# sebhaan/geobo

Measured on AMD Instinct MI355X. Metric: voxels/sec posterior (mean+var) for 64^3 x 2-prop joint inversion; fp64 roofline %, higher is better.
Workload: dtype f64

## Files before the change

geobo_amd/_lib.py:

```python
import ctypes as C
import os

LIB_PATH = os.environ.get("GEOBO_HIP_LIB") or os.path.join(os.path.dirname(os.path.abspath(__file__)), "lib", "libgeobo_hip.so")

_dp = C.c_void_p
_i64 = C.c_int64
_f64 = C.c_double
_int = C.c_int
_sz = C.c_size_t

SIGNATURES = {
    "geobo_version": (_int, []),
    "geobo_pad_m": (_i64, [_i64]),
    "geobo_pad_n": (_i64, [_i64]),
    "geobo_k_block": (_int, [_int, _dp, _dp, _dp, _i64, _dp, _dp, _dp, _i64, _f64, _f64, _f64, _f64, _dp, _i64, _dp]),
    "geobo_k_block_f32": (_int, [_int, _dp, _dp, _dp, _i64, _dp, _dp, _dp, _i64, _f64, _f64, _f64, _f64, _dp, _i64, _dp]),
    "geobo_k_block_grid": (_int, [_int, _int, _int, _dp, _dp, _i64, _i64, _i64, _i64, _int, _dp, _i64, _dp]),
    "geobo_lattice_wbuild": (_int, [_i64, _int, _int, _int, _dp, _dp, _dp, _dp]),
    "geobo_lattice_wplanes": (_int, [_i64, _int, _int, _int, _dp, _dp, _dp, _dp]),
    "geobo_xz2d_fold_inv_strided": (_int, [_int, _i64, _int, _dp, _i64, _i64, _dp, _dp, _dp, _i64, _i64, _i64, _dp]),
    "geobo_xz2d_fold_inv_mul": (_int, [_int, _i64, _int, _dp, _i64, _dp, _i64, _dp, _dp, _dp, _i64, _i64, _i64, _dp]),
    "geobo_sumsq_accum": (_int, [_i64, _i64, _dp, _i64, _dp, _i64, _int, _dp, _i64, _dp]),
    "geobo_lamdot_z": (_int, [_i64, _int, _int, _int, _dp, _dp, _dp, _dp]),
    "geobo_centro_fill": (_int, [_dp, _i64, _i64, _i64, _dp]),
    "geobo_mirror_rows": (_int, [_dp, _i64, _i64, _i64, _i64, _int, _dp]),
    "geobo_mirror_dev_ws_bytes": (_sz, []),
    "geobo_mirror_dev": (_int, [_dp, _i64, _dp, _i64, _i64, _int, _int, _dp, _dp, _sz, _dp]),
    "geobo_colgemv_ws_bytes": (_sz, [_i64, _i64]),
    "geobo_colgemv": (_int, [_i64, _i64, _dp, _i64, _dp, _dp, _dp, _sz, _dp]),
    "geobo_rowgemv": (_int, [_i64, _i64, _dp, _i64, _dp, _dp, _dp]),
    "geobo_convert": (_int, [_int, _dp, _i64, _dp, _i64, _i64, _i64, _dp]),
    "geobo_round_f32": (_int, [_dp, _i64, _dp]),
    "geobo_k_eval": (_int, [_int, _dp, _i64, _f64, _f64, _f64, _f64, _dp, _dp]),
    "geobo_a_sens": (_int, [_int, C.POINTER(_f64), _dp, _i64, _int, _int, _int, _dp, _dp, _dp, _f64, _f64, _dp, _i64, _dp]),
    "geobo_a_sens_slab": (_int, [_int, C.POINTER(_f64), _dp, _i64, _int, _int, _int, _dp, _dp, _dp, _f64, _f64, _int, _int, _dp, _i64, _i64, _dp]),
    "geobo_potential": (_int, [_int, C.POINTER(_f64), _dp, _dp, _dp, _i64, _dp, _dp]),
    "geobo_ak_fused": (_int, [_int, _dp, _i64, _i64, _i64, _dp, _dp, _dp, _i64, _i64, _f64, _f64, _f64, _f64, _dp, _i64, _dp]),
    "geobo_ak_points": (_int, [_int, _dp, _i64, _i64, _i64, _dp, _dp, _dp, _dp, _dp, _dp, _i64, _f64, _f64, _f64, _f64, _dp, _i64, _dp]),
    "geobo_cov_table": (_int, [_int, _int, _int, _int, _f64, _f64, _f64, _f64, _f64, _f64, _f64, _dp, _dp]),
    "geobo_ak_fused_grid": (_int, [_dp, _i64, _i64, _i64, _int, _int, _int, _dp, _i64, _i64, _dp, _i64, _dp]),
    "geobo_gemm_nt": (_int, [_i64, _i64, _i64, _f64, _dp, _i64, _dp, _i64, _f64, _dp, _i64, _int, _i64, _dp]),
    "geobo_tile_order": (_i64, [_int, _int, _int, _int, _int, _int, _int, C.POINTER(_int), _i64]),
    "geobo_gemm_nt_splitk": (_int, [_i64, _i64, _i64, _int, _dp, _i64, _dp, _i64, _dp, _i64, _int, _i64, _dp, _sz, _dp]),
    "geobo_gemm_nn": (_int, [_i64, _i64, _i64, _f64, _dp, _i64, _dp, _i64, _f64, _dp, _i64, _int, _int, _dp]),
    "geobo_gemm_batched": (_int, [_int, _i64, _i64, _i64, _f64, _dp, _i64, _i64, _dp, _i64, _i64, _f64, _dp, _i64, _i64, _i64, _i64, _int, _dp]),
    "geobo_gemm_fold_lamdot": (_int, [_i64, _i64, _i64, _dp, _i64, _dp, _i64, _i64, _dp, _int, _i64, _dp, _i64, _dp]),
    "geobo_gemm_fold": (_int, [_int, _int, _i64, _i64, _i64, _dp, _i64, _i64, _dp, _i64, _i64, _dp, _i64, _i64, _i64, _i64, _i64, _dp]),
    "geobo_scale_broadcast": (_int, [_dp, _dp, _i64, _i64, _dp, _dp]),
    "geobo_scale_broadcast2": (_int, [_dp, _dp, _dp, _i64, _i64, _dp, _dp, _dp]),
    "geobo_a_sens_lattice_ws_bytes": (_sz, [_int, _int, _int]),
    "geobo_a_sens_lattice": (_int, [_int, C.POINTER(_f64), _i64, _int, _int, _int, _dp, _dp, _dp, _dp, _dp, _f64, _f64, _int, _int, _dp, _i64,
                                    _i64, _dp, _sz, _dp]),
    "geobo_xz2d": (_int, [_int, _int, _int, _i64, _int, _dp, _i64, _i64, _dp, _i64, _dp, _i64, _dp, _i64, _i64, _dp]),
    "geobo_xz2d_fold": (_int, [_int, _int, _i64, _int, _dp, _i64, _i64, _dp, _dp, _dp, _i64, _i64, _dp]),
    "geobo_xz2d_fold_quad": (_int, [_int, _int, _i64, _int, _dp, _i64, _i64, _dp, _dp, _dp, _i64, _i64, _dp]),
    "geobo_xcorr_reduce_fold": (_int, [_int, _i64, _int, _dp, _i64, _i64, _dp, _dp, _dp, _i64, _i64, _dp]),
    "geobo_xz2d_fold_lattice": (_int, [_int, _i64, _int, _dp, _dp, _i64, _dp, _i64, _dp, _dp, _dp, _i64, _i64, _dp]),
    "geobo_xz2d_fold_inv_ss_slots": (_int, [_int, _i64, _int]),
    "geobo_xz2d_fold_inv_ss": (_int, [_int, _i64, _int, _dp, _i64, _i64, _dp, _i64, _i64, _dp, _dp, _dp, _dp]),
    "geobo_ymul": (_int, [_int, _int, _i64, _i64, _dp, _i64, _dp, _i64, _dp, _i64, _dp]),
    "geobo_ymul_fold": (_int, [_int, _int, _i64, _i64, _dp, _i64, _dp, _i64, _dp, _i64, _dp]),
    "geobo_xcorr_reduce": (_int, [_int, _int, _i64, _int, _dp, _i64, _i64, _dp, _i64, _dp, _dp, _i64, _i64, _dp]),
    "geobo_toeplitz_y": (_int, [_int, _i64, _i64, _i64, _int, _dp, _dp, _dp, _dp, _dp, _int, _int, _dp]),
    "geobo_toeplitz_y2t": (_int, [_int, _i64, _i64, _i64, _dp, _dp, _dp, _dp, _dp, _dp, _dp, _dp, _dp]),
    "geobo_toeplitz_y2s": (_int, [_int, _i64, _i64, _i64, _dp, _dp, _dp, _dp, _dp, _dp, _dp, _dp]),
    "geobo_toeplitz_y3": (_int, [_int, _i64, _i64, _i64, _int, _dp, C.POINTER(_dp), C.POINTER(_dp), _int, _int, _dp]),
    "geobo_toeplitz_y3_add": (_int, [_int, _i64, _i64, _i64, _int, _dp, C.POINTER(_dp), C.POINTER(_dp), _int, _int, _dp]),
    "geobo_spectral_y_basis_doubles": (_i64, [_int]),
    "geobo_spectral_y_basis": (_int, [_int, _dp, _dp]),
    "geobo_spectral_y": (_int, [_int, _i64, _i64, _i64, _int, _dp, _dp, _dp, _dp, _dp, _int, _int, _dp, _dp]),
    "geobo_spectral_y_lattice": (_int, [_int, _i64, _i64, _i64, _int, _dp, _dp, _dp, _i64, _dp, _dp, _dp, _dp, _dp, _int, _int, _dp, _dp]),
    "geobo_spectral_y2s": (_int, [_int, _i64, _i64, _i64, _dp, _dp, _dp, _dp, _dp, _dp, _dp, _dp, _dp]),
    "geobo_spectral_y3": (_int, [_int, _i64, _i64, _i64, _int, _dp, C.POINTER(_dp), C.POINTER(_dp), _int, _int, _int, _dp, _dp]),
    "geobo_spectral_y3t": (_int, [_int, _i64, _i64, _i64, _int, _dp, _dp, C.POINTER(_dp), C.POINTER(_dp), C.POINTER(_dp), _dp, _dp]),
    "geobo_spectral_axis": (_int, [_int, _int, _i64, _i64, _i64, _i64, _i64, _i64, _dp, _dp, _dp, _int, _dp]),
    "geobo_potrf_ws_bytes": (_sz, [_i64]),
    "geobo_potrf_ctx_create": (_int, [C.POINTER(C.c_void_p)]),
    "geobo_potrf_ctx_destroy": (_int, [_dp]),
    "geobo_potrf_inv": (_int, [_i64, _dp, _i64, _dp, _i64, _dp, _dp, _sz, _dp, _dp]),
    "geobo_posterior_ws_bytes": (_sz, [_i64, _i64]),
    "geobo_posterior_reduce": (_int, [_i64, _i64, _dp, _i64, _dp, _i64, _dp, _f64, _dp, _dp, _i64, _dp, _sz, _dp]),
    "geobo_kinv_dot_ws_bytes": (_sz, [_i64, _int]),
    "geobo_kinv_dot": (_int, [_i64, _dp, _i64, _dp, _int, C.POINTER(_dp), _i64, C.POINTER(_i64), _dp, _dp, _sz, _dp]),
    "geobo_philox_fill": (_int, [_int, C.c_uint64, C.c_uint64, _i64, _i64, _i64, _i64, C.c_uint64, _dp, _dp]),
    "geobo_torus_table": (_int, [_int, _int, _int, _int, _f64, _f64, _f64, _f64, _f64, _f64, _f64, _dp, _dp]),
    "geobo_fft_lines": (_int, [_int, _i64]),
    "geobo_fft_axis": (_int, [_int, _i64, _int, _i64, _int, _int, _dp, _dp, _int, _i64, _i64, _dp]),
    "geobo_sample_factor_ws_bytes": (_sz, []),
    "geobo_sample_factor": (_int, [_int, _int, _int, _int, _dp, _dp, _dp, _dp, _sz, _dp, _dp]),
    "geobo_sample_zpass": (_int, [_int, _i64, _i64, _int, _int, _int, _int, _dp, _dp, C.c_uint64, _dp, _dp]),
    "geobo_spectral_mix": (_int, [_int, _i64, _int, _int, _int, _dp, _f64, _dp, _dp, _dp]),
    "geobo_set_gram": (_int, [_i64, _int, _dp, _i64, _dp, _i64, _i64, _int, _dp, _dp]),
    "geobo_set_logdet": (_int, [_i64, _int, _dp, _dp, _i64, _f64, _dp, _dp, _i64, _dp, _dp, _dp]),
    "geobo_kinv_diag_ws_bytes": (_sz, [_i64]),
    "geobo_kinv_diag": (_int, [_i64, _dp, _i64, _dp, _dp, _dp, _dp, _sz, _dp]),
    "geobo_set_loo": (_int, [_i64, _int, _dp, _dp, _dp, _i64, _dp, _dp, _dp, _dp, _dp, _dp]),
    "geobo_block_cov_ws_bytes": (_sz, [_i64, _int, _int, _int, _int, _int, _int]),
    "geobo_block_cov": (_int, [_i64, _dp, _dp, _dp, _i64, _int, _int, _int, _int, _int, _int, _int, _dp, _dp, _sz, _dp]),
    "geobo_box_means": (_int, [_i64, _dp, _i64, _i64, _int, _int, _int, _int, _int, _int, _dp, _dp, _dp]),
    "geobo_cutoff_stats_ws_bytes": (_sz, [_i64, _i64, _int]),
    "geobo_cutoff_stats": (_int, [_i64, _dp, _i64, _i64, _i64, _int, _int, C.POINTER(_f64), C.POINTER(_f64), _dp, _dp, _dp, _dp, _dp, _dp, _sz, _dp]),
    "geobo_bodies_ws_bytes": (_sz, [_i64, _int, _int, _int, _int]),
    "geobo_bodies": (_int, [_i64, _dp, _i64, _i64, _int, _int, _int, _int, _int, C.POINTER(_f64), C.POINTER(_f64), _dp, _dp, _int, _i64, _i64,
                            C.POINTER(C.c_int32), _dp, _dp, _dp, _dp, _dp, _dp, _int, _dp, _sz, _dp]),
    "geobo_trace_stats_ws_bytes": (_sz, [_i64, _i64, _int]),
    "geobo_trace_stats": (_int, [_i64, _dp, _i64, _i64, _int, _int, _int, _int, _int, C.POINTER(_f64), C.POINTER(_f64), _dp, _i64, _dp, _dp, _int,
                                 _int, _int, _dp, _dp, _dp, _dp, _dp, _dp, _dp, _dp, _dp, _dp, _dp, _sz, _dp]),
    "geobo_trmv_stats": (_int, [_i64, _dp, _i64, _dp, _dp, _i64, _dp, _dp, _dp]),
    "geobo_mfma_f64_peak": (_int, [_int, _int, _dp, _dp]),
    "geobo_mfma_mix": (_int, [_int, _int, _int, _int, _dp, _dp]),
}


class GeoboHipUnavailable(RuntimeError):
    pass


_lib = None


def load():
    global _lib
    if _lib is not None:
        return _lib
    if not os.path.exists(LIB_PATH):
        raise GeoboHipUnavailable(
            "%s not found. Build the HIP extension first: `python -m geobo_amd.build` "
            "(hipcc --offload-arch=gfx950). There is no CPU fallback for the inversion hot path." % LIB_PATH)
    import torch
    try:
        lib = C.CDLL(LIB_PATH)
    except OSError as e:
        raise GeoboHipUnavailable("cannot load %s: %s" % (LIB_PATH, e)) from e
    for name, (res, args) in SIGNATURES.items():
        try:
            fn = getattr(lib, name)
        except AttributeError as e:
            raise GeoboHipUnavailable("libgeobo_hip.so lacks symbol %s (stale build?)" % name) from e
        fn.restype = res
        fn.argtypes = args
    _lib = lib
    return lib


ERRORS = {-1: "GEOBO_E_ARG", -2: "GEOBO_E_ALIGN", -3: "GEOBO_E_LAUNCH", -4: "GEOBO_E_UNSUPPORTED"}


def check(rc, what):
    if rc != 0:
        raise RuntimeError("%s failed: %s (%d)" % (what, ERRORS.get(rc, "?"), rc))
```

geobo_amd/csrc/gemm_f64.hip:

```cpp
#include <hip/hip_runtime.h>
#include <atomic>
#include <type_traits>
#include <stdint.h>
#include "covfun.h"
#include "geobo_hip.h"

typedef double v4d __attribute__((ext_vector_type(4)));
typedef double v2d __attribute__((ext_vector_type(2)));

namespace {

constexpr int BK = 16;
constexpr int XS = 16;
constexpr int NST = 3;

__device__ __forceinline__ int swz(int row) {
  const int p = (row >> 1) & 7;
  return (p & 1) | (((p >> 2) & 1) * 6);
}

enum { Y_GEN = 0, Y_NT = 1, Y_NN = 2, Y_TAB = 3 };
enum { EPI_STORE = 0, EPI_REDUCE = 1 };
enum { TRI_LOWER_ONLY = 1, TRI_X_LOWER = 2, TRI_Y_LOWER = 4 };

struct GemmArgs {
  const double* X; int64_t ldx;
  const double* Y; int64_t ldy;
  double* C; int64_t ldc;
  int64_t k;
  double alpha, beta;
  int nbi, nbj, tri, xcd_map;
  int ntiles;
  int64_t sXb, sYb, sCb, m_valid, n_valid; int batch;
  const double *px, *py, *pz; int64_t gcol0;
  const double *qx, *qy, *qz;
  CovParams cov;
  const double* table; int gnx, gny, gnz; int64_t gN;
  const double* u; double* part_mu; double* part_ss; int64_t ncols;
  int64_t row_shift;
};

__host__ __device__ inline int lower_cols(int bi, int nbj, int tm, int tn) {
  const int64_t c = ((int64_t)(bi + 1) * tm + tn - 1) / tn;
  return c < nbj ? (int)c : nbj;
}
__host__ __device__ inline int64_t tile_items(int nbi, int nbj, int tm, int tn, int tri) {
  if (!(tri & TRI_LOWER_ONLY)) return (int64_t)nbi * nbj;
  int64_t n = 0;
  for (int bi = 0; bi < nbi; ++bi) n += lower_cols(bi, nbj, tm, tn);
  return n;
}
__host__ __device__ __forceinline__ void tile_of_item(int t, int nbi, int nbj, int tm, int tn, int tri, int& bi, int& bj) {
  if (tri & TRI_X_LOWER) { bi = nbi - 1 - t / nbj; bj = t % nbj; return; }
  if (tri & TRI_Y_LOWER) { bj = t / nbi; bi = t % nbi; return; }
  if (!(tri & TRI_LOWER_ONLY)) {
    const int band = t / (4 * nbj), r0 = 4 * band;
    const int rows = nbi - r0 < 4 ? nbi - r0 : 4;
    t -= band * 4 * nbj;
    bj = t / rows; bi = r0 + t % rows;
    return;
  }
  int r0 = 0;
  for (;; r0 += 4) {
    int cnt = 0;
    for (int i = r0; i < r0 + 4 && i < nbi; ++i) cnt += lower_cols(i, nbj, tm, tn);
    if (t < cnt || r0 + 4 >= nbi) break;
    t -= cnt;
  }
  const int r1 = r0 + 4 < nbi ? r0 + 4 : nbi;
  for (bj = 0; bj < nbj; ++bj) {
    const int first = (int)(((int64_t)bj * tn) / tm);
    const int lo = first > r0 ? first : r0;
    const int c = r1 - lo;
    if (c <= 0) continue;
    if (t < c) { bi = lo + t; return; }
    t -= c;
  }
  bi = nbi; bj = 0;
}

template <int WM, int WN>
constexpr int ring_depth() { return (WM * WN >= 8) ? NST : 2; }

template <int WM, int WN, int YMODE>
constexpr int lds_doubles() {
  constexpr int TM = 64 * WM, TN = 64 * WN;
  constexpr int ybuf = (YMODE == Y_NN) ? BK * (TN + 4) : TN * XS;
  return ring_depth<WM, WN>() * (TM * XS + ybuf);
}

template <int WM, int WN, int YMODE, int EPI, int KID>
__global__ void __launch_bounds__(64 * WM * WN, 2) gemm_f64_kernel(const GemmArgs a) {
  constexpr int TM = 64 * WM, TN = 64 * WN, NT = 64 * WM * WN;
  constexpr int YS_NN = TN + 4;
  constexpr int XBUF = TM * XS;
  constexpr int YBUF = (YMODE == Y_NN) ? BK * YS_NN : TN * XS;
  constexpr int XU = TM * 8 / NT;
  constexpr int YU = (YMODE == Y_NN) ? (8 * TN / NT) : (TN * 8 / NT);
  constexpr int EPT = BK * TN / NT;
  static_assert(NT % TN == 0 && EPT >= 2 && EPT % 2 == 0, "generator mapping");

  extern __shared__ __attribute__((aligned(16))) double smem[];
  double* const Xs = smem;
  constexpr int NSTG = ring_depth<WM, WN>();
  double* const Ys = smem + NSTG * XBUF;

  const int tid = threadIdx.x, lane = tid & 63;
  const int wave = __builtin_amdgcn_readfirstlane(tid >> 6);
  const int wrow = wave / WN, wn = wave % WN;
  const int wm = (WM == 4) ? (wrow < 2 ? wrow : 5 - wrow) : wrow;
  const int lr = lane & 15, lg = lane >> 4;

  int bi, bj;
  int batch_idx = blockIdx.y;
  {
    const int b = blockIdx.x;
    if (a.xcd_map == 1) {
      const int xcd = b & 7, s = b >> 3;
      bj = s % a.nbj;
      bi = xcd + 8 * (s / a.nbj);
    } else if (a.xcd_map == 2) {
      const int xcd = b & 7, s = b >> 3;
      const int within = s & 31, g = (s >> 5) * 8 + xcd;
      const int nsi = (a.nbi + 3) >> 2;
      if (a.tri & TRI_X_LOWER) {
        const int nsj = (a.nbj + 31) >> 5;
        bi = g / nsj;
        bj = 32 * (g % nsj) + within;
      } else {
        bi = 4 * (g % nsi) + (within & 3);
        bj = 8 * (g / nsi) + (within >> 2);
      }
      if (bj >= a.nbj) return;
    } else if (a.xcd_map == 3) {
      const int xcd = b & 7, s = b >> 3;
      const int64_t item = ((int64_t)((s >> 5) * 8 + xcd) << 5) + (s & 31);
      if (item >= (int64_t)a.ntiles * a.batch) return;
      batch_idx = (int)(item / a.ntiles);
      tile_of_item((int)(item - (int64_t)batch_idx * a.ntiles), a.nbi, a.nbj, TM, TN, a.tri, bi, bj);
    } else {
      bi = b % a.nbi;
      bj = b / a.nbi;
    }
  }
  if (bi >= a.nbi) return;
  const double* const Xp = a.X + (int64_t)batch_idx * a.sXb;
  const double* const Yp = a.Y + (int64_t)batch_idx * a.sYb;
  double* const Cp = a.C + (int64_t)batch_idx * a.sCb;
  if ((a.tri & TRI_X_LOWER) && a.xcd_map != 3) bi = a.nbi - 1 - bi;
  const int64_t row0 = (int64_t)bi * TM - a.row_shift, col0 = (int64_t)bj * TN;
  if ((a.tri & TRI_LOWER_ONLY) && col0 >= row0 + TM) return;
  int64_t kb = (a.tri & TRI_Y_LOWER) ? col0 : 0;
  int64_t ke = a.k;
  if ((a.tri & TRI_X_LOWER) && ke > row0 + TM) ke = row0 + TM;

  v4d acc[4][4];
#pragma unroll
  for (int m = 0; m < 4; ++m)
#pragma unroll
    for (int n = 0; n < 4; ++n) acc[m][n] = (v4d){0., 0., 0., 0.};
  bool c_in_acc = false;
  if constexpr (EPI == EPI_STORE && (YMODE == Y_NT || YMODE == Y_NN)) {
    c_in_acc = a.beta != 0.0 && (a.beta == a.alpha || a.beta == -a.alpha);
    if (c_in_acc) {
      const double sgn = (a.beta == a.alpha) ? 1.0 : -1.0;
#pragma unroll
      for (int m = 0; m < 4; ++m)
#pragma unroll
        for (int n = 0; n < 4; ++n)
#pragma unroll
          for (int r = 0; r < 4; ++r) {
            const int64_t row = row0 + wm * 64 + m * 16 + lg + 4 * r;
            const int64_t col = col0 + wn * 64 + n * 16 + lr;
            const bool ok = row < a.m_valid && col < a.n_valid;
            const double c = Cp[(row < a.m_valid ? row : a.m_valid - 1) * a.ldc + (col < a.n_valid ? col : a.n_valid - 1)];
            acc[m][n][r] = ok ? sgn * c : 0.0;
          }
    }
  }

  typedef __attribute__((address_space(3))) void* lds_ptr_t;
  typedef const __attribute__((address_space(1))) void* glb_ptr_t;
  auto dma16 = [&](const void* src, double* dst_wave_uniform) {
    __builtin_amdgcn_global_load_lds((glb_ptr_t)src, (lds_ptr_t)dst_wave_uniform, 16, 0, 0);
  };
  constexpr int RPI = NT / 8;
  const int srow = tid >> 3;
  const char* const Xgb = reinterpret_cast<const char*>(Xp);
  int64_t xsrc[XU];
#pragma unroll
  for (int i = 0; i < XU; ++i) {
    const int row = i * RPI + srow;
    const int64_t grow = row0 + row < 0 ? 0 : row0 + row;
    xsrc[i] = (grow * a.ldx + 2 * ((tid & 7) ^ swz(row))) * 8;
  }
  auto stage_x = [&](int64_t k0, int st) {
#pragma unroll
    for (int i = 0; i < XU; ++i) dma16(Xgb + xsrc[i] + k0 * 8, Xs + st * XBUF + (i * RPI + wave * 8) * XS);
  };

  int64_t ysrc[(YMODE == Y_NT) ? YU : 1];
  const char* const Ygb = (YMODE == Y_NT) ? reinterpret_cast<const char*>(Yp + col0 * a.ldy) : nullptr;
  if constexpr (YMODE == Y_NT) {
#pragma unroll
    for (int i = 0; i < YU; ++i) {
      const int row = i * RPI + srow;
      ysrc[i] = ((int64_t)row * a.ldy + 2 * ((tid & 7) ^ swz(row))) * 8;
    }
  }

  double qx = 0., qy = 0., qz = 0.;
  const int gq = tid % TN;
  const int gsub = __builtin_amdgcn_readfirstlane(tid / TN);
  v2d yr[EPT / 2];
  if constexpr (YMODE == Y_GEN) {
    const int64_t q = col0 + gq;
    qx = a.qx[q]; qy = a.qy[q]; qz = a.qz[q];
  }

  int tqy[YU], tqx[YU], tqz[YU], tsl[YU];
  int piy = 0, pix = 0, piz = 0;
  int64_t pk = kb;
  if constexpr (YMODE == Y_TAB) {
#pragma unroll
    for (int i = 0; i < YU; ++i) {
      const int row = i * RPI + srow;
      int64_t q = a.gcol0 + col0 + row;
      if (q >= a.gN) q = a.gN - 1;
      tqz[i] = (int)(q % a.gnz);
      const int64_t t = q / a.gnz;
      tqx[i] = (int)(t % a.gnx);
      tqy[i] = (int)(t / a.gnx);
      tsl[i] = (tid & 7) ^ swz(row);
    }
    piz = (int)(kb % a.gnz);
    const int64_t tp = kb / a.gnz;
    pix = (int)(tp % a.gnx);
    piy = (int)(tp / a.gnx);
  }

  auto stage_y = [&](int64_t k0, int st) {
    if constexpr (YMODE == Y_NT) {
#pragma unroll
      for (int i = 0; i < YU; ++i) dma16(Ygb + ysrc[i] + k0 * 8, Ys + st * YBUF + (i * RPI + wave * 8) * XS);
    } else if constexpr (YMODE == Y_NN) {
#pragma unroll
      for (int i = 0; i < YU; ++i) {
        const int kr = i * (NT / 64) + wave;
        dma16(Yp + (k0 + kr) * a.ldy + col0 + 2 * lane, Ys + st * YBUF + kr * YS_NN);
      }
    } else if constexpr (YMODE == Y_TAB) {
      const int adv = (int)(k0 - pk);
      pk = k0;
      piz += adv;
      int c = piz >= a.gnz ? 1 : 0;
      piz -= c ? a.gnz : 0;
      pix += c;
      c = pix >= a.gnx ? 1 : 0;
      pix -= c ? a.gnx : 0;
      piy += c;
      int bx = pix + 1, by = piy;
      if (bx >= a.gnx) { bx = 0; by += 1; }
      const int ay = piy < a.gny ? piy : a.gny - 1;
      by = by < a.gny ? by : a.gny - 1;
      const char* const tb = reinterpret_cast<const char*>(a.table);
      const unsigned nz2 = 2u * (unsigned)a.gnz;
#pragma unroll
      for (int i = 0; i < YU; ++i) {
        int pz = piz + 2 * tsl[i];
        const bool carry = pz >= a.gnz;
        pz -= carry ? a.gnz : 0;
        const unsigned cy = carry ? by : ay, cx = carry ? bx : pix;
        const unsigned rowb = __umul24(__usad((unsigned)tqx[i], cx, __umul24(__usad((unsigned)tqy[i], cy, 0u), (unsigned)a.gnx)), nz2);
        const unsigned idx = rowb + (unsigned)(pz - tqz[i] + a.gnz - 1);
        dma16(tb + (idx << 3), Ys + st * YBUF + (i * RPI + wave * 8) * XS);
      }
    }
  };
  auto gen_y = [&](int64_t k0) {
    const int64_t p0 = k0 + gsub * EPT;
#pragma unroll
    for (int e = 0; e < EPT; ++e) {
      const double d2 = sqdist3(a.px[p0 + e], a.py[p0 + e], a.pz[p0 + e], qx, qy, qz);
      yr[e >> 1][e & 1] = a.cov.scale * cov_eval<KID>(a.cov, d2);
    }
  };
  auto store_gen = [&](int st) {
    double* buf = Ys + st * YBUF;
#pragma unroll
    for (int e = 0; e < EPT / 2; ++e)
      *reinterpret_cast<v2d*>(buf + gq * XS + 2 * ((gsub * (EPT / 2) + e) ^ swz(gq))) = yr[e];
  };

  if (kb < ke) {
    const int xoff0 = 2 * ((2 * lg + 0) ^ swz(lr)), xoff1 = 2 * ((2 * lg + 1) ^ swz(lr));
    const double* const xfrag = Xs + (wm * 64 + lr) * XS;
    const double* const yfrag = (YMODE == Y_NN) ? (Ys + wn * 64 + lr) : (Ys + (wn * 64 + lr) * XS);
    auto read_half = [&](int stage, int h, v2d (&av)[4], v2d (&bv)[4]) {
      const double* xb = xfrag + stage * XBUF + (h ? xoff1 : xoff0);
#pragma unroll
      for (int m = 0; m < 4; ++m) av[m] = *reinterpret_cast<const v2d*>(xb + m * 16 * XS);
      if constexpr (YMODE == Y_NN) {
        const double* yb = yfrag + stage * YBUF + (4 * lg + 2 * h) * YS_NN;
#pragma unroll
        for (int n = 0; n < 4; ++n) { bv[n][0] = yb[n * 16]; bv[n][1] = yb[YS_NN + n * 16]; }
      } else {
        const double* yb = yfrag + stage * YBUF + (h ? xoff1 : xoff0);
#pragma unroll
        for (int n = 0; n < 4; ++n) bv[n] = *reinterpret_cast<const v2d*>(yb + n * 16 * XS);
      }
    };
    if constexpr (NSTG == 2) {
      stage_x(kb, 0);
      if constexpr (YMODE == Y_GEN) { gen_y(kb); store_gen(0); } else { stage_y(kb, 0); }
      __syncthreads();
      int cur = 0;
      for (int64_t k0 = kb; k0 < ke; k0 += BK) {
        int64_t kn = k0 + BK;
        if (kn >= ke) kn = ke - BK;
        stage_x(kn, cur ^ 1);
        if constexpr (YMODE != Y_GEN) stage_y(kn, cur ^ 1);
        v2d a0[4], b0[4], a1[4], b1[4];
        read_half(cur, 0, a0, b0);
        read_half(cur, 1, a1, b1);
        if constexpr (YMODE == Y_GEN) gen_y(kn);
#pragma unroll
        for (int t = 0; t < 4; ++t)
#pragma unroll
          for (int m = 0; m < 4; ++m)
#pragma unroll
            for (int n = 0; n < 4; ++n)
              acc[m][n] = __builtin_amdgcn_mfma_f64_16x16x4f64(t < 2 ? a0[m][t & 1] : a1[m][t & 1],
                                                               t < 2 ? b0[n][t & 1] : b1[n][t & 1], acc[m][n], 0, 0, 0);
        if constexpr (YMODE == Y_GEN) store_gen(cur ^ 1);
        __syncthreads();
        cur ^= 1;
      }
    } else {
    {
        const int64_t k1 = (kb + BK < ke) ? kb + BK : kb;
        stage_x(kb, 0);
        stage_x(k1, 1);
        if constexpr (YMODE == Y_GEN) {
          gen_y(kb); store_gen(0);
          gen_y(k1); store_gen(1);
        } else {
          stage_y(kb, 0);
          stage_y(k1, 1);
        }
      }
      __syncthreads();
      int s0 = 0, s1 = 1, s2 = 2;
      int64_t kw = ke;
      if constexpr (YMODE != Y_GEN) {
        if ((a.tri & TRI_X_LOWER) && kw > row0 + 64 * (wm + 1)) kw = row0 + 64 * (wm + 1);
        if (row0 + wm * 64 >= a.m_valid || row0 + wm * 64 < 0 || kw < kb) kw = kb;
      }
      int64_t kd = kw;
      if constexpr (YMODE != Y_GEN) {
        if ((a.tri & TRI_X_LOWER) && kw == row0 + 64 * (wm + 1) && kw - 64 >= kb) kd = kw - 64;
      }
      if (kw > kb) {
      v2d a0[4], b0[4], a1[4], b1[4];
      read_half(0, 0, a0, b0);
      for (int64_t k0 = kb; k0 < kd; k0 += BK) {
        int64_t kn = k0 + 2 * BK;
        if (kn >= ke) kn = ke - BK;
        stage_x(kn, s2);
        if constexpr (YMODE != Y_GEN) stage_y(kn, s2);
        const int64_t p0 = kn + gsub * EPT;
        read_half(s0, 1, a1, b1);
  #pragma unroll
        for (int t = 0; t < 4; ++t) {
          if (t == 2) read_half(s1, 0, a0, b0);
  #pragma unroll
          for (int m = 0; m < 4; ++m)
  #pragma unroll
            for (int n = 0; n < 4; ++n)
              acc[m][n] = __builtin_amdgcn_mfma_f64_16x16x4f64(t < 2 ? a0[m][t & 1] : a1[m][t & 1],
                                                               t < 2 ? b0[n][t & 1] : b1[n][t & 1], acc[m][n], 0, 0, 0);
          if constexpr (YMODE == Y_GEN) {
  #pragma unroll
            for (int e = t * (EPT / 4); e < (t + 1) * (EPT / 4); ++e) {
              const double d2 = sqdist3(a.px[p0 + e], a.py[p0 + e], a.pz[p0 + e], qx, qy, qz);
              yr[e >> 1][e & 1] = a.cov.scale * cov_eval<KID>(a.cov, d2);
            }
          }
        }
        if constexpr (YMODE != Y_GEN) {
  #pragma unroll
          for (int i = 0; i < 64; ++i) {
            __builtin_amdgcn_sched_group_barrier(0x008, 1, 0);
            __builtin_amdgcn_sched_group_barrier(0x126, 4, 0);
          }
        }
        if constexpr (YMODE == Y_GEN && (KID <= COV_MATERN32_X)) {
          constexpr int GEN_VALU = (KID == COV_MATERN32_X) ? 7 : ((KID == COV_D2) ? 1 : 5);
  #pragma unroll
          for (int i = 0; i < 64; ++i) {
            __builtin_amdgcn_sched_group_barrier(0x008, 1, 0);
            __builtin_amdgcn_sched_group_barrier(0x002, GEN_VALU * (EPT / 4), 0);
          }
        }
        if constexpr (YMODE == Y_GEN) store_gen(s2);
        __syncthreads();
        const int ts = s0; s0 = s1; s1 = s2; s2 = ts;
      }
      if constexpr (YMODE != Y_GEN) {
        if (kd < kw) {
          auto diag_chunk = [&](auto mlo, int64_t k0) {
            constexpr int MLO = decltype(mlo)::value;
            int64_t kn = k0 + 2 * BK;
            if (kn >= ke) kn = ke - BK;
            stage_x(kn, s2);
            stage_y(kn, s2);
            read_half(s0, 1, a1, b1);
  #pragma unroll
            for (int t = 0; t < 4; ++t) {
              if (t == 2) read_half(s1, 0, a0, b0);
  #pragma unroll
              for (int m = MLO; m < 4; ++m)
  #pragma unroll
                for (int n = 0; n < 4; ++n)
                  acc[m][n] = __builtin_amdgcn_mfma_f64_16x16x4f64(t < 2 ? a0[m][t & 1] : a1[m][t & 1],
                                                                   t < 2 ? b0[n][t & 1] : b1[n][t & 1], acc[m][n], 0, 0, 0);
            }
  #pragma unroll
            for (int i = 0; i < 16 * (4 - MLO); ++i) {
              __builtin_amdgcn_sched_group_barrier(0x008, 1, 0);
              __builtin_amdgcn_sched_group_barrier(0x126, 6, 0);
            }
            __syncthreads();
            const int ts = s0; s0 = s1; s1 = s2; s2 = ts;
          };
          diag_chunk(std::integral_constant<int, 0>{}, kd);
          diag_chunk(std::integral_constant<int, 1>{}, kd + BK);
          diag_chunk(std::integral_constant<int, 2>{}, kd + 2 * BK);
          diag_chunk(std::integral_constant<int, 3>{}, kd + 3 * BK);
        }
      }
      }
      if constexpr (YMODE != Y_GEN) {
        for (int64_t k0 = kw; k0 < ke; k0 += BK) {
          int64_t kn = k0 + 2 * BK;
          if (kn >= ke) kn = ke - BK;
          stage_x(kn, s2);
          stage_y(kn, s2);
          __syncthreads();
          const int ts = s0; s0 = s1; s1 = s2; s2 = ts;
        }
      }
    }
  }

  if constexpr (EPI == EPI_STORE) {
    if (row0 + TM <= a.m_valid && col0 + TN <= a.n_valid && (a.beta == 0.0 || c_in_acc)) {
      double* const cw = Cp + (row0 + wm * 64 + lg) * a.ldc + col0 + wn * 64 + lr;
#pragma unroll
      for (int m = 0; m < 4; ++m)
#pragma unroll
        for (int n = 0; n < 4; ++n)
#pragma unroll
          for (int r = 0; r < 4; ++r) cw[(int64_t)(m * 16 + 4 * r) * a.ldc + n * 16] = a.alpha * acc[m][n][r];
      return;
    }
#pragma unroll
    for (int m = 0; m < 4; ++m)
#pragma unroll
      for (int n = 0; n < 4; ++n)
#pragma unroll
        for (int r = 0; r < 4; ++r) {
          const int64_t row = row0 + wm * 64 + m * 16 + lg + 4 * r;
          const int64_t col = col0 + wn * 64 + n * 16 + lr;
          if (row < a.m_valid && col < a.n_valid) {
            double v = a.alpha * acc[m][n][r];
            double* dst = Cp + row * a.ldc + col;
            if (a.beta != 0.0 && !c_in_acc) v += a.beta * (*dst);
            *dst = v;
          }
        }
  } else {
    double smu[4], sss[4];
#pragma unroll
    for (int n = 0; n < 4; ++n) { smu[n] = 0.; sss[n] = 0.; }
#pragma unroll
    for (int m = 0; m < 4; ++m)
#pragma unroll
      for (int r = 0; r < 4; ++r) {
        const int64_t ri = row0 + wm * 64 + m * 16 + lg + 4 * r;
        const double ur = a.u[ri < 0 ? 0 : ri];
#pragma unroll
        for (int n = 0; n < 4; ++n) {
          const double v = acc[m][n][r];
          smu[n] = __builtin_fma(v, ur, smu[n]);
          sss[n] = __builtin_fma(v, v, sss[n]);
        }
      }
#pragma unroll
    for (int n = 0; n < 4; ++n) {
      smu[n] += __shfl_xor(smu[n], 16); smu[n] += __shfl_xor(smu[n], 32);
      sss[n] += __shfl_xor(sss[n], 16); sss[n] += __shfl_xor(sss[n], 32);
    }
    double* red = smem;
    if (lg == 0) {
#pragma unroll
      for (int n = 0; n < 4; ++n) {
        red[(0 * WM + wm) * TN + wn * 64 + n * 16 + lr] = smu[n];
        red[(1 * WM + wm) * TN + wn * 64 + n * 16 + lr] = sss[n];
      }
    }
    __syncthreads();
    if (tid < TN) {
      double m_ = 0., s_ = 0.;
#pragma unroll
      for (int w = 0; w < WM; ++w) { m_ += red[(0 * WM + w) * TN + tid]; s_ += red[(1 * WM + w) * TN + tid]; }
      a.part_mu[(int64_t)bi * a.ncols + col0 + tid] = m_;
      a.part_ss[(int64_t)bi * a.ncols + col0 + tid] = s_;
    }
  }
}

__global__ void __launch_bounds__(256) sum_slices_kernel(const double* __restrict__ part, int splits, int64_t m, int64_t n,
                                                         double* __restrict__ out, int64_t ldo) {
  const int64_t n2 = n >> 1, total = m * n2;
  for (int64_t i = (int64_t)blockIdx.x * 256 + threadIdx.x; i < total; i += (int64_t)gridDim.x * 256) {
    const int64_t r = i / n2, c = (i - r * n2) * 2;
    v2d acc = *reinterpret_cast<const v2d*>(part + r * n + c);
    for (int s = 1; s < splits; ++s) acc += *reinterpret_cast<const v2d*>(part + (int64_t)s * m * n + r * n + c);
    *reinterpret_cast<v2d*>(out + r * ldo + c) = acc;
  }
}

__global__ void posterior_finish_kernel(const double* part_mu, const double* part_ss, int nbi, int64_t ncols,
                                        double prior_var, double* mu, double* var) {
  const int64_t c = (int64_t)blockIdx.x * blockDim.x + threadIdx.x;
  if (c >= ncols) return;
  double m = 0., s = 0.;
  for (int b = 0; b < nbi; ++b) { m += part_mu[(int64_t)b * ncols + c]; s += part_ss[(int64_t)b * ncols + c]; }
  mu[c] = m;
  var[c] = prior_var - s;
}

template <int WM, int WN, int YMODE, int EPI, int KID>
int launch(GemmArgs& a, hipStream_t st) {
  constexpr int NT = 64 * WM * WN;
  constexpr size_t lds = sizeof(double) * lds_doubles<WM, WN, YMODE>();
  auto kern = gemm_f64_kernel<WM, WN, YMODE, EPI, KID>;
  static std::atomic<uint64_t> attr_done{0};
  int dev = 0;
  if (hipGetDevice(&dev) != hipSuccess || dev < 0 || dev >= 64) return GEOBO_E_LAUNCH;
  if (!((attr_done.load(std::memory_order_acquire) >> dev) & 1)) {
    if (hipFuncSetAttribute(reinterpret_cast<const void*>(kern), hipFuncAttributeMaxDynamicSharedMemorySize, (int)lds) != hipSuccess)
      return GEOBO_E_LAUNCH;
    attr_done.fetch_or((uint64_t)1 << dev, std::memory_order_release);
  }
  if (a.m_valid <= 0) a.m_valid = (int64_t)1 << 62;
  if (a.n_valid <= 0) a.n_valid = (int64_t)1 << 62;
  a.xcd_map = (a.nbi >= 8) ? 1 : 0;
  if ((YMODE == Y_NT || YMODE == Y_NN) && !(a.tri & TRI_LOWER_ONLY) && a.nbi >= 4 && a.nbj >= 8) a.xcd_map = 2;
  a.ntiles = 0;
  if (a.batch <= 0) a.batch = 1;
  const int64_t items = (int64_t)a.nbi * a.nbj * a.batch;
  if ((YMODE == Y_NT || YMODE == Y_NN) && EPI == EPI_STORE && a.batch <= 64 &&
      a.nbi * a.nbj >= ((a.tri & (TRI_X_LOWER | TRI_Y_LOWER)) ? 16 : 64) && items <= 65536 && a.nbi <= 4096 &&
      (a.tri & (TRI_X_LOWER | TRI_Y_LOWER)) != (TRI_X_LOWER | TRI_Y_LOWER)) {
    a.ntiles = (int)tile_items(a.nbi, a.nbj, 64 * WM, 64 * WN, a.tri);
    if (a.ntiles > 0) a.xcd_map = 3;
  }
  int nblocks = a.nbi * a.nbj;
  if (a.xcd_map == 3) {
    const int64_t groups = ((int64_t)a.ntiles * a.batch + 31) / 32;
    nblocks = (int)(8 * 32 * ((groups + 7) / 8));
    hipLaunchKernelGGL(kern, dim3(nblocks), dim3(NT), lds, st, a);
    return hipGetLastError() == hipSuccess ? GEOBO_OK : GEOBO_E_LAUNCH;
  }
  if (a.xcd_map == 1) nblocks = 8 * ((a.nbi + 7) / 8) * a.nbj;
  if (a.xcd_map == 2) {
    int nst = ((a.nbi + 3) / 4) * ((a.nbj + 7) / 8);
    if (a.tri & TRI_X_LOWER) nst = a.nbi * ((a.nbj + 31) / 32);
    nblocks = 8 * 32 * ((nst + 7) / 8);
  }
  hipLaunchKernelGGL(kern, dim3(nblocks, a.batch), dim3(NT), lds, st, a);
  return hipGetLastError() == hipSuccess ? GEOBO_OK : GEOBO_E_LAUNCH;
}

template <int YMODE, int EPI, int KID>
int launch_by_rows(GemmArgs& a, int64_t m, int64_t n, hipStream_t st, bool small_tiles = false) {
  if (n % 128) return GEOBO_E_ALIGN;
  a.nbj = (int)(n / 128);
  if (m % 256 == 0 && !small_tiles) { a.nbi = (int)(m / 256); return launch<4, 2, YMODE, EPI, KID>(a, st); }
  if (m % 128 == 0) { a.nbi = (int)(m / 128); return launch<2, 2, YMODE, EPI, KID>(a, st); }
  return GEOBO_E_ALIGN;
}

}

extern "C" int64_t geobo_tile_order(int nbi, int nbj, int tm, int tn, int lower_only, int x_lower, int y_lower, int* out_host,
                                    int64_t capacity) {
  if (nbi <= 0 || nbj <= 0 || tm <= 0 || tn <= 0 || (x_lower && y_lower)) return GEOBO_E_ARG;
  const int tri = (lower_only ? TRI_LOWER_ONLY : 0) | (x_lower ? TRI_X_LOWER : 0) | (y_lower ? TRI_Y_LOWER : 0);
  const int64_t n = tile_items(nbi, nbj, tm, tn, tri);
  if (out_host)
    for (int64_t t = 0; t < n && t < capacity; ++t) {
      int bi, bj;
      tile_of_item((int)t, nbi, nbj, tm, tn, tri, bi, bj);
      out_host[t] = bi << 16 | bj;
    }
  return n;
}

extern "C" int geobo_ak_fused(int kernel_id, const double* A, int64_t Ms_pad, int64_t N_pad, int64_t lda,
                              const double* x, const double* y, const double* z, int64_t col0, int64_t ncols,
                              double l1, double l2, double w, double amp, double* AK, int64_t ldak, void* stream) {
  if (!A || !x || !y || !z || !AK) return GEOBO_E_ARG;
  if (Ms_pad % 128 || N_pad % BK || ncols % 128 || (lda & 1) || col0 < 0 || col0 + ncols > N_pad) return GEOBO_E_ALIGN;
  GemmArgs a{};
  a.X = A; a.ldx = lda; a.Y = nullptr; a.ldy = 0; a.C = AK; a.ldc = ldak; a.k = N_pad;
  a.alpha = 1.0; a.beta = 0.0; a.tri = 0;
  a.px = x; a.py = y; a.pz = z; a.gcol0 = col0;
  a.qx = x + col0; a.qy = y + col0; a.qz = z + col0;
  a.cov = make_cov(kernel_id, l1, l2, w, amp);
  hipStream_t st = (hipStream_t)stream;
#define GEOBO_FUSED(ID) return launch_by_rows<Y_GEN, EPI_STORE, ID>(a, Ms_pad, ncols, st)
  COV_DISPATCH_ALL(kernel_id, GEOBO_FUSED);
#undef GEOBO_FUSED
  return GEOBO_E_ARG;
}

extern "C" int geobo_ak_points(int kernel_id, const double* A, int64_t R_pad, int64_t N_pad, int64_t lda,
                               const double* px, const double* py, const double* pz,
                               const double* qx, const double* qy, const double* qz, int64_t nq_pad,
                               double l1, double l2, double w, double amp, double* out, int64_t ldo, void* stream) {
  if (!A || !px || !py || !pz || !qx || !qy || !qz || !out) return GEOBO_E_ARG;
  if (R_pad <= 0 || N_pad <= 0 || nq_pad <= 0 || R_pad % 128 || N_pad % BK || nq_pad % 128 || (lda & 1) || lda < N_pad || ldo < nq_pad)
    return GEOBO_E_ALIGN;
  GemmArgs a{};
  a.X = A; a.ldx = lda; a.Y = nullptr; a.ldy = 0; a.C = out; a.ldc = ldo; a.k = N_pad;
  a.alpha = 1.0; a.beta = 0.0; a.tri = 0;
  a.px = px; a.py = py; a.pz = pz; a.gcol0 = 0;
  a.qx = qx; a.qy = qy; a.qz = qz;
  a.cov = make_cov(kernel_id, l1, l2, w, amp);
  hipStream_t st = (hipStream_t)stream;
#define GEOBO_POINTS(ID) return launch_by_rows<Y_GEN, EPI_STORE, ID>(a, R_pad, nq_pad, st)
  COV_DISPATCH_ALL(kernel_id, GEOBO_POINTS);
#undef GEOBO_POINTS
  return GEOBO_E_ARG;
}

extern "C" int geobo_ak_fused_grid(const double* A, int64_t Ms_pad, int64_t N_pad, int64_t lda, int nx, int ny, int nz,
                                   const double* table, int64_t col0, int64_t ncols, double* AK, int64_t ldak,
                                   void* stream) {
  if (!A || !table || !AK) return GEOBO_E_ARG;
  if (nx <= 0 || ny <= 0 || nz < BK || (nz & 1)) return GEOBO_E_UNSUPPORTED;
  if ((int64_t)nx * ny * nz * 16 >= (int64_t)1 << 32) return GEOBO_E_UNSUPPORTED;
  const int64_t N = (int64_t)nx * ny * nz;
  if (Ms_pad % 128 || N_pad % BK || ncols % 128 || (lda & 1) || col0 < 0 || col0 + ncols > N_pad || N_pad < N) return GEOBO_E_ALIGN;
  GemmArgs a{};
  a.X = A; a.ldx = lda; a.Y = nullptr; a.ldy = 0; a.C = AK; a.ldc = ldak; a.k = N_pad;
  a.alpha = 1.0; a.beta = 0.0; a.tri = 0;
  a.gcol0 = col0; a.table = table; a.gnx = nx; a.gny = ny; a.gnz = nz; a.gN = N;
  return launch_by_rows<Y_TAB, EPI_STORE, COV_D2>(a, Ms_pad, ncols, (hipStream_t)stream);
}

extern "C" int geobo_gemm_nt(int64_t m, int64_t n, int64_t k, double alpha, const double* X, int64_t ldx,
                             const double* Y, int64_t ldy, double beta, double* C, int64_t ldc, int lower_only,
                             int64_t m_valid, void* stream) {
  if (!X || !Y || !C) return GEOBO_E_ARG;
  if (k % BK || (ldx & 1) || (ldy & 1)) return GEOBO_E_ALIGN;
  GemmArgs a{};
  a.X = X; a.ldx = ldx; a.Y = Y; a.ldy = ldy; a.C = C; a.ldc = ldc; a.k = k;
  a.alpha = alpha; a.beta = beta; a.tri = (lower_only & GEOBO_GEMM_LOWER_ONLY) ? TRI_LOWER_ONLY : 0;
  a.m_valid = m_valid;
  return launch_by_rows<Y_NT, EPI_STORE, COV_D2>(a, m, n, (hipStream_t)stream, (lower_only & GEOBO_GEMM_SMALL_TILES) != 0);
}

extern "C" int geobo_gemm_nt_splitk(int64_t m, int64_t n, int64_t k, int splits, const double* X, int64_t ldx, const double* Y,
                                    int64_t ldy, double* C, int64_t ldc, int lower_only, int64_t m_valid, void* ws,
                                    size_t ws_bytes, void* stream) {
  if (!X || !Y || !C || !ws || splits < 1 || splits > 64) return GEOBO_E_ARG;
  if (k % (BK * splits) || (ldx & 1) || (ldy & 1) || (ldc & 1) || (n & 1)) return GEOBO_E_ALIGN;
  if (ws_bytes < (size_t)splits * m * n * sizeof(double)) return GEOBO_E_ARG;
  hipStream_t st = (hipStream_t)stream;
  if (hipMemsetAsync(ws, 0, (size_t)splits * m * n * sizeof(double), st) != hipSuccess) return GEOBO_E_LAUNCH;
  GemmArgs a{};
  a.X = X; a.ldx = ldx; a.Y = Y; a.ldy = ldy; a.C = (double*)ws; a.ldc = n; a.k = k / splits;
  a.alpha = 1.0; a.beta = 0.0; a.tri = lower_only ? TRI_LOWER_ONLY : 0;
  a.sXb = k / splits; a.sYb = k / splits; a.sCb = m * n; a.batch = splits;
  a.m_valid = m_valid;
  int rc = launch_by_rows<Y_NT, EPI_STORE, COV_D2>(a, m, n, st);
  if (rc) return rc;
  int64_t nblk = (m * (n / 2) + 255) / 256;
  if (nblk > 256 * 16) nblk = 256 * 16;
  hipLaunchKernelGGL(sum_slices_kernel, dim3((unsigned)nblk), dim3(256), 0, st, (const double*)ws, splits, m, n, C, ldc);
  return hipGetLastError() == hipSuccess ? GEOBO_OK : GEOBO_E_LAUNCH;
}

extern "C" int geobo_gemm_nn(int64_t m, int64_t n, int64_t k, double alpha, const double* X, int64_t ldx,
                             const double* Y, int64_t ldy, double beta, double* C, int64_t ldc, int x_lower,
                             int y_lower, void* stream) {
  if (!X || !Y || !C) return GEOBO_E_ARG;
  if (k % BK || (ldx & 1) || (ldy & 1)) return GEOBO_E_ALIGN;
  GemmArgs a{};
  a.X = X; a.ldx = ldx; a.Y = Y; a.ldy = ldy; a.C = C; a.ldc = ldc; a.k = k;
  a.alpha = alpha; a.beta = beta; a.tri = ((x_lower & 1) ? TRI_X_LOWER : 0) | ((y_lower & 1) ? TRI_Y_LOWER : 0);
  return launch_by_rows<Y_NN, EPI_STORE, COV_D2>(a, m, n, (hipStream_t)stream, ((x_lower | y_lower) & GEOBO_GEMM_SMALL_TILES) != 0);
}

extern "C" int geobo_gemm_batched(int y_is_kn, int64_t m, int64_t n, int64_t k, double alpha, const double* X, int64_t ldx,
                                  int64_t strideX, const double* Y, int64_t ldy, int64_t strideY, double beta, double* C,
                                  int64_t ldc, int64_t strideC, int64_t m_valid, int64_t n_valid, int batch, void* stream) {
  if (!X || !Y || !C || batch <= 0 || batch > 65535) return GEOBO_E_ARG;
  if (k % BK || (ldx & 1) || (ldy & 1) || (strideX & 1) || (strideY & 1)) return GEOBO_E_ALIGN;
  GemmArgs a{};
  a.X = X; a.ldx = ldx; a.Y = Y; a.ldy = ldy; a.C = C; a.ldc = ldc; a.k = k;
  a.alpha = alpha; a.beta = beta; a.tri = 0;
  a.sXb = strideX; a.sYb = strideY; a.sCb = strideC; a.m_valid = m_valid; a.n_valid = n_valid; a.batch = batch;
  if (y_is_kn) return launch_by_rows<Y_NN, EPI_STORE, COV_D2>(a, m, n, (hipStream_t)stream);
  return launch_by_rows<Y_NT, EPI_STORE, COV_D2>(a, m, n, (hipStream_t)stream);
}

extern "C" size_t geobo_posterior_ws_bytes(int64_t m, int64_t ncols) {
  return (size_t)2 * (size_t)((m + 127) / 128) * (size_t)ncols * sizeof(double);
}

extern "C" int geobo_posterior_reduce(int64_t m, int64_t ncols, const double* Linv, int64_t ldi, const double* AK,
                                      int64_t ldak, const double* u, double prior_var, double* mu, double* var,
                                      int64_t m_valid, void* ws, size_t ws_bytes, void* stream) {
  if (!Linv || !AK || !u || !mu || !var || !ws) return GEOBO_E_ARG;
  if (m % 128 || ncols % 128 || (ldi & 1) || (ldak & 1)) return GEOBO_E_ALIGN;
  if (ws_bytes < geobo_posterior_ws_bytes(m, ncols)) return GEOBO_E_ARG;
  hipStream_t st = (hipStream_t)stream;
  GemmArgs a{};
  a.X = Linv; a.ldx = ldi; a.Y = AK; a.ldy = ldak; a.C = nullptr; a.ldc = 0; a.k = m;
  a.alpha = 1.0; a.beta = 0.0; a.tri = TRI_X_LOWER;
  a.u = u; a.ncols = ncols;
  a.m_valid = (m_valid > 0 && m_valid < m) ? m_valid : m;
  const int nbi_max = (int)((m + 127) / 128);
  a.part_mu = (double*)ws;
  a.part_ss = (double*)ws + (size_t)nbi_max * ncols;
  const int64_t groups = (a.m_valid + 63) / 64;
  a.row_shift = 64 * ((4 - groups % 4) % 4);
  a.nbi = (int)((groups * 64 + a.row_shift) / 256);
  a.nbj = (int)(ncols / 128);
  int rc = launch<4, 2, Y_NN, EPI_REDUCE, COV_D2>(a, st);
  if (rc) return rc;
  hipLaunchKernelGGL(posterior_finish_kernel, dim3((unsigned)((ncols + 255) / 256)), dim3(256), 0, st, a.part_mu,
                     a.part_ss, a.nbi, ncols, prior_var, mu, var);
  return hipGetLastError() == hipSuccess ? GEOBO_OK : GEOBO_E_LAUNCH;
}
```

geobo_amd/csrc/reduce.hip:

```cpp
#include <hip/hip_runtime.h>
#include <stdint.h>
#include "geobo_hip.h"

namespace {

typedef double v2d __attribute__((ext_vector_type(2)));

__global__ void __launch_bounds__(256) sumsq_accum_kernel(int64_t rows, int64_t n2, const double* __restrict__ a, int64_t lda,
                                                          const double* __restrict__ b, int64_t ldb, int slots, double* __restrict__ ss,
                                                          int64_t ld_ss) {
  const int64_t c2 = (int64_t)blockIdx.x * 256 + threadIdx.x;
  if (c2 >= n2) return;
  const int slot = blockIdx.y;
  v2d acc = *reinterpret_cast<const v2d*>(ss + slot * ld_ss + 2 * c2);
  if (b) {
    for (int64_t r = slot; r < rows; r += slots) {
      const v2d x = *reinterpret_cast<const v2d*>(a + r * lda + 2 * c2) + *reinterpret_cast<const v2d*>(b + r * ldb + 2 * c2);
      acc.x = __builtin_fma(x.x, x.x, acc.x);
      acc.y = __builtin_fma(x.y, x.y, acc.y);
    }
  } else {
    for (int64_t r = slot; r < rows; r += slots) {
      const v2d x = *reinterpret_cast<const v2d*>(a + r * lda + 2 * c2);
      acc.x = __builtin_fma(x.x, x.x, acc.x);
      acc.y = __builtin_fma(x.y, x.y, acc.y);
    }
  }
  *reinterpret_cast<v2d*>(ss + slot * ld_ss + 2 * c2) = acc;
}

__global__ void __launch_bounds__(256) lamdot_z_kernel(int64_t nrows, int planes, int px, int nz, const double* __restrict__ D,
                                                       const double* __restrict__ lam, double* __restrict__ out) {
  const int sub = threadIdx.x & 7;
  for (int64_t row = (int64_t)blockIdx.x * 32 + (threadIdx.x >> 3); row < nrows; row += (int64_t)gridDim.x * 32) {
    const int64_t bp = row / px;
    const int o = (int)(row - bp * px);
    const double* d = D + row * nz;
    const double* l = lam + ((int64_t)(bp % planes) * px + o) * nz;
    double acc = 0.0;
    for (int z = 2 * sub; z < nz; z += 16) {
      const v2d x = *reinterpret_cast<const v2d*>(d + z), y = *reinterpret_cast<const v2d*>(l + z);
      acc = __builtin_fma(x.x, y.x, acc);
      acc = __builtin_fma(x.y, y.y, acc);
    }
    acc += __shfl_xor(acc, 1);
    acc += __shfl_xor(acc, 2);
    acc += __shfl_xor(acc, 4);
    if (sub == 0) out[row] = acc;
  }
}

__global__ void __launch_bounds__(256) rowgemv_kernel(int64_t m, int64_t n2, const double* __restrict__ X, int64_t ld,
                                                      const double* __restrict__ v, double* __restrict__ out) {
  __shared__ double part[4];
  for (int64_t r = blockIdx.x; r < m; r += gridDim.x) {
    const v2d* x = reinterpret_cast<const v2d*>(X + r * ld);
    const v2d* w = reinterpret_cast<const v2d*>(v);
    double acc = 0.0;
    for (int64_t c = threadIdx.x; c < n2; c += 256) {
      const v2d a = x[c], b = w[c];
      acc = __builtin_fma(a.x, b.x, acc);
      acc = __builtin_fma(a.y, b.y, acc);
    }
    for (int o = 32; o > 0; o >>= 1) acc += __shfl_xor(acc, o);
    if ((threadIdx.x & 63) == 0) part[threadIdx.x >> 6] = acc;
    __syncthreads();
    if (threadIdx.x == 0) out[r] = (part[0] + part[1]) + (part[2] + part[3]);
    __syncthreads();
  }
}

__global__ void __launch_bounds__(256) centro_fill_kernel(double* __restrict__ B, int64_t ld, int64_t n, int64_t r0) {
  const int64_t p = (int64_t)blockIdx.x * 256 + threadIdx.x;
  const int64_t c = 2 * p;
  if (c >= n) return;
  for (int64_t r = r0 + blockIdx.y; r < n; r += gridDim.y) {
    const double* src = B + (n - 1 - r) * ld;
    double* dst = B + r * ld;
    if (c + 1 < n) {
      const v2d v = *reinterpret_cast<const v2d*>(src + c);
      if ((n & 1) == 0) {
        v2d w;
        w.x = v.y;
        w.y = v.x;
        *reinterpret_cast<v2d*>(dst + (n - 2 - c)) = w;
      } else {
        dst[n - 2 - c] = v.y;
        dst[n - 1 - c] = v.x;
      }
    } else {
      dst[0] = src[c];
    }
  }
}

__global__ void __launch_bounds__(256) mirror_rows_kernel(double* __restrict__ X, int64_t ld, int64_t m, int64_t r0, int64_t nb, int nz2) {
  const int64_t e = (int64_t)blockIdx.x * 256 + threadIdx.x;
  if (e >= nb * nz2) return;
  const int64_t b = e / nz2;
  const int64_t se = (nb - 1 - b) * nz2 + (e - b * nz2);
  for (int64_t r = r0 + blockIdx.y; r < m; r += gridDim.y)
    reinterpret_cast<v2d*>(X + r * ld)[e] = reinterpret_cast<const v2d*>(X + (m - 1 - r) * ld)[se];
}

__device__ __forceinline__ double max_keep_nan(double m, double v) { return (v > m || v != v) ? v : m; }

constexpr int MIRROR_SLOTS_X = 4, MIRROR_SLOTS_Y = 256;

__global__ void __launch_bounds__(256) mirror_dev_kernel(const double* __restrict__ a, int64_t lda, const double* __restrict__ b, int64_t ldb,
                                                         int64_t rows, int nx, int nz2, double* __restrict__ part) {
  __shared__ double sh[2][4];
  double dev = 0.0, mx = 0.0;
  const int pairs = nx * nz2;
  for (int64_t r = blockIdx.y; r < rows; r += gridDim.y) {
    const v2d* pa = reinterpret_cast<const v2d*>(a + r * lda);
    const v2d* pb = reinterpret_cast<const v2d*>(b + (rows - 1 - r) * ldb);
    for (int e = blockIdx.x * 256 + threadIdx.x; e < pairs; e += gridDim.x * 256) {
      const int x = e / nz2;
      const v2d u = pa[e], w = pb[(nx - 1 - x) * nz2 + (e - x * nz2)];
      dev = max_keep_nan(max_keep_nan(dev, __builtin_fabs(u.x - w.x)), __builtin_fabs(u.y - w.y));
      mx = max_keep_nan(max_keep_nan(mx, __builtin_fabs(u.x)), __builtin_fabs(u.y));
      mx = max_keep_nan(max_keep_nan(mx, __builtin_fabs(w.x)), __builtin_fabs(w.y));
    }
  }
  for (int o = 32; o > 0; o >>= 1) {
    dev = max_keep_nan(dev, __shfl_xor(dev, o));
    mx = max_keep_nan(mx, __shfl_xor(mx, o));
  }
  if ((threadIdx.x & 63) == 0) {
    sh[0][threadIdx.x >> 6] = dev;
    sh[1][threadIdx.x >> 6] = mx;
  }
  __syncthreads();
  if (threadIdx.x < 2) {
    const double* s = sh[threadIdx.x];
    part[2 * ((int64_t)blockIdx.y * gridDim.x + blockIdx.x) + threadIdx.x] = max_keep_nan(max_keep_nan(s[0], s[1]), max_keep_nan(s[2], s[3]));
  }
}

__global__ void __launch_bounds__(256) mirror_dev_finish_kernel(const double* __restrict__ part, int slots, double* __restrict__ out) {
  __shared__ double sh[2][4];
  double dev = 0.0, mx = 0.0;
  for (int s = threadIdx.x; s < slots; s += 256) {
    dev = max_keep_nan(dev, part[2 * s]);
    mx = max_keep_nan(mx, part[2 * s + 1]);
  }
  for (int o = 32; o > 0; o >>= 1) {
    dev = max_keep_nan(dev, __shfl_xor(dev, o));
    mx = max_keep_nan(mx, __shfl_xor(mx, o));
  }
  if ((threadIdx.x & 63) == 0) {
    sh[0][threadIdx.x >> 6] = dev;
    sh[1][threadIdx.x >> 6] = mx;
  }
  __syncthreads();
  if (threadIdx.x < 2) {
    const double* s = sh[threadIdx.x];
    out[threadIdx.x] = max_keep_nan(max_keep_nan(s[0], s[1]), max_keep_nan(s[2], s[3]));
  }
}

}

extern "C" int geobo_centro_fill(double* B, int64_t ld, int64_t n, int64_t r0, void* stream) {
  if (!B || ((uintptr_t)B & 15) || n < 0 || r0 < 0 || r0 > n || 2 * r0 < n || ld < n) return GEOBO_E_ARG;
  if (ld & 1) return GEOBO_E_ALIGN;
  if (r0 == n) return GEOBO_OK;
  const int64_t gy = n - r0 < 65535 ? n - r0 : 65535;
  hipLaunchKernelGGL(centro_fill_kernel, dim3((unsigned)(((n + 1) / 2 + 255) / 256), (unsigned)gy), dim3(256), 0, (hipStream_t)stream, B, ld, n, r0);
  return hipGetLastError() == hipSuccess ? GEOBO_OK : GEOBO_E_LAUNCH;
}

extern "C" int geobo_mirror_rows(double* X, int64_t ld, int64_t m, int64_t r0, int64_t nb, int nz, void* stream) {
  if (!X || m < 0 || r0 < 0 || r0 > m || 2 * r0 < m || nb <= 0 || nz <= 0 || nb * nz > ld) return GEOBO_E_ARG;
  if ((nz & 1) || (ld & 1) || ((uintptr_t)X & 15)) return GEOBO_E_ALIGN;
  if (r0 == m) return GEOBO_OK;
  const int64_t pairs = nb * (nz / 2), gy = m - r0 < 65535 ? m - r0 : 65535;
  hipLaunchKernelGGL(mirror_rows_kernel, dim3((unsigned)((pairs + 255) / 256), (unsigned)gy), dim3(256), 0, (hipStream_t)stream, X, ld, m, r0, nb,
                     nz / 2);
  return hipGetLastError() == hipSuccess ? GEOBO_OK : GEOBO_E_LAUNCH;
}

extern "C" size_t geobo_mirror_dev_ws_bytes(void) { return sizeof(double) * 2 * MIRROR_SLOTS_X * MIRROR_SLOTS_Y; }

extern "C" int geobo_mirror_dev(const double* a, int64_t lda, const double* b, int64_t ldb, int64_t rows, int nx, int nz, double* out2, void* ws,
                                size_t ws_bytes, void* stream) {
  if (!a || !b || !out2 || !ws || rows <= 0 || nx <= 0 || nz <= 0 || ws_bytes < geobo_mirror_dev_ws_bytes()) return GEOBO_E_ARG;
  if ((int64_t)nx * nz > lda || (int64_t)nx * nz > ldb || (int64_t)nx * nz >= (1LL << 31)) return GEOBO_E_ARG;
  if ((nz & 1) || (lda & 1) || (ldb & 1) || ((uintptr_t)a & 15) || ((uintptr_t)b & 15) || ((uintptr_t)ws & 15)) return GEOBO_E_ALIGN;
  const int pairs = nx * (nz / 2);
  const int gx = (pairs + 255) / 256 < MIRROR_SLOTS_X ? (pairs + 255) / 256 : MIRROR_SLOTS_X;
  const int gy = rows < MIRROR_SLOTS_Y ? (int)rows : MIRROR_SLOTS_Y;
  hipLaunchKernelGGL(mirror_dev_kernel, dim3(gx, gy), dim3(256), 0, (hipStream_t)stream, a, lda, b, ldb, rows, nx, nz / 2, (double*)ws);
  hipLaunchKernelGGL(mirror_dev_finish_kernel, dim3(1), dim3(256), 0, (hipStream_t)stream, (const double*)ws, gx * gy, out2);
  return hipGetLastError() == hipSuccess ? GEOBO_OK : GEOBO_E_LAUNCH;
}

extern "C" int geobo_rowgemv(int64_t m, int64_t n, const double* X, int64_t ld, const double* v, double* out, void* stream) {
  if (!X || !v || !out) return GEOBO_E_ARG;
  if (m <= 0 || n <= 0) return GEOBO_OK;
  if ((n & 1) || (ld & 1) || ld < n || ((uintptr_t)X & 15) || ((uintptr_t)v & 15)) return GEOBO_E_ALIGN;
  const int64_t nb = m < 256 * 16 ? m : 256 * 16;
  hipLaunchKernelGGL(rowgemv_kernel, dim3((unsigned)nb), dim3(256), 0, (hipStream_t)stream, m, n / 2, X, ld, v, out);
  return hipGetLastError() == hipSuccess ? GEOBO_OK : GEOBO_E_LAUNCH;
}

extern "C" int geobo_sumsq_accum(int64_t rows, int64_t n, const double* a, int64_t lda, const double* b, int64_t ldb, int slots,
                                 double* ss, int64_t ld_ss, void* stream) {
  if (!a || !ss) return GEOBO_E_ARG;
  if (rows <= 0 || n <= 0) return GEOBO_OK;
  if (slots < 1 || slots > 65535) return GEOBO_E_ARG;
  if ((n & 1) || (lda & 1) || (ldb & 1) || (ld_ss & 1) || lda < n || (b && ldb < n) || ld_ss < n || ((uintptr_t)a & 15) || ((uintptr_t)b & 15) ||
      ((uintptr_t)ss & 15))
    return GEOBO_E_ALIGN;
  const int64_t n2 = n / 2;
  hipLaunchKernelGGL(sumsq_accum_kernel, dim3((unsigned)((n2 + 255) / 256), (unsigned)slots), dim3(256), 0, (hipStream_t)stream, rows, n2, a,
                     lda, b, ldb, slots, ss, ld_ss);
  return hipGetLastError() == hipSuccess ? GEOBO_OK : GEOBO_E_LAUNCH;
}

extern "C" int geobo_lamdot_z(int64_t batch, int planes, int px, int nz, const double* D, const double* lam, double* out, void* stream) {
  if (!D || !lam || !out) return GEOBO_E_ARG;
  if (batch <= 0) return GEOBO_OK;
  if (planes <= 0 || px <= 0 || nz <= 0) return GEOBO_E_ARG;
  if ((nz & 15) || ((uintptr_t)D & 15) || ((uintptr_t)lam & 15)) return GEOBO_E_ALIGN;
  const int64_t nrows = batch * px;
  int64_t nb = (nrows + 31) / 32;
  if (nb > 256 * 64) nb = 256 * 64;
  hipLaunchKernelGGL(lamdot_z_kernel, dim3((unsigned)nb), dim3(256), 0, (hipStream_t)stream, nrows, planes, px, nz, D, lam, out);
  return hipGetLastError() == hipSuccess ? GEOBO_OK : GEOBO_E_LAUNCH;
}
```

geobo_amd/hip.py:

```python
import ctypes as C

import numpy as np
import torch

from . import _lib

F64 = torch.float64

KERNEL_IDS = {"d2": 0, "exp": 1, "exp_x": 2, "matern32": 3, "matern32_x": 4, "sparse": 5, "sparse_x": 6,
              "exp_dl": 7, "exp_x_dl1": 8, "exp_x_dl2": 9, "matern32_dl": 10, "matern32_x_dl1": 11, "matern32_x_dl2": 12,
              "sparse_dl": 13, "sparse_x_dl1": 14, "sparse_x_dl2": 15}
FUNC_IDS = {"grav": 0, "magn": 1}
from .plan import (PAD_M, PAD_N, SPECTRAL_AXIS_N, SPECTRAL_Y3T_NY, SPECTRAL_Y_NY, TOEPLITZ_ADD_NY, TOEPLITZ_NY, TOEPLITZ_Y2T_NY,
                   XZ2D_FOLD_N, XZ2D_SHAPES, YMUL_SHAPES)


def kernel_id(name, cross, deriv=None):
    if name not in ("exp", "matern32", "sparse"):
        raise ValueError("unknown kernelfunc %r (expected 'sparse', 'exp' or 'matern32')" % (name,))
    if deriv is None:
        return KERNEL_IDS[name + ("_x" if cross else "")]
    if isinstance(deriv, bool) or deriv not in (1, 2):
        raise ValueError("deriv must be None, 1 or 2, got %r" % (deriv,))
    if not cross:
        if deriv != 1:
            raise ValueError("the self family %r has one length: deriv must be 1" % (name,))
        return KERNEL_IDS[name + "_dl"]
    return KERNEL_IDS["%s_x_dl%d" % (name, deriv)]


def pad_m(m):
    return (int(m) + PAD_M - 1) // PAD_M * PAD_M


def pad_n(n):
    return (int(n) + PAD_N - 1) // PAD_N * PAD_N


def require_gpu():
    if not torch.cuda.is_available():
        raise _lib.GeoboHipUnavailable("no MI355X / ROCm device visible: the GeoBO hot path has no CPU fallback")
    return _lib.load()


def _stream():
    return C.c_void_p(torch.cuda.current_stream().cuda_stream)


def _p(t):
    return C.c_void_p(t.data_ptr())


def _chk(t, name, dtype=F64):
    if not (isinstance(t, torch.Tensor) and t.is_cuda and t.dtype == dtype):
        raise TypeError("%s must be a CUDA %s tensor" % (name, dtype))
    return t


def _rowmajor(t, name):
    _chk(t, name)
    if t.dim() != 2 or t.stride(1) != 1:
        raise ValueError("%s must be 2-D with unit column stride" % name)
    return t.stride(0)


def version():
    return _lib.load().geobo_version()


F32 = torch.float32


def k_block(kid, rows_xyz, cols_xyz, l1, l2, w, amp, out):
    lib = require_gpu()
    rx, ry, rz = (_chk(t, "rows") for t in rows_xyz)
    cx, cy, cz = (_chk(t, "cols") for t in cols_xyz)
    if not (isinstance(out, torch.Tensor) and out.is_cuda and out.dtype in (F64, F32) and out.dim() == 2 and out.stride(1) == 1):
        raise TypeError("out must be a 2-D CUDA float64 / float32 tensor with unit column stride")
    ld = out.stride(0)
    nr, nc = rx.numel(), cx.numel()
    assert out.shape[0] >= nr and out.shape[1] >= nc
    fn, name = (lib.geobo_k_block, "geobo_k_block") if out.dtype == F64 else (lib.geobo_k_block_f32, "geobo_k_block_f32")
    _lib.check(fn(kid, _p(rx), _p(ry), _p(rz), nr, _p(cx), _p(cy), _p(cz), nc, float(l1), float(l2), float(w), float(amp),
                  _p(out), ld, _stream()), name)
    return out


def k_block_grid(table, nx, ny, nz, rows, col0, out, row0=0, nr=None):
    lib = require_gpu()
    if not (isinstance(out, torch.Tensor) and out.is_cuda and out.dtype in (F64, F32) and out.dim() == 2 and out.stride(1) == 1):
        raise TypeError("out must be a 2-D CUDA float64 / float32 tensor with unit column stride")
    if rows is not None:
        assert rows.dtype == torch.int64 and rows.is_cuda and rows.is_contiguous()
        nr = rows.numel()
    nr = out.shape[0] if nr is None else int(nr)
    assert out.shape[0] >= nr and _chk(table, "table").numel() >= 2 * nx * ny * nz
    _lib.check(lib.geobo_k_block_grid(int(nx), int(ny), int(nz), _p(table), C.c_void_p(rows.data_ptr()) if rows is not None else None,
                                      int(row0), nr, int(col0), out.shape[1], 1 if out.dtype == F32 else 0, _p(out), out.stride(0),
                                      _stream()), "geobo_k_block_grid")
    return out


def lattice_wbuild(rows, Py, Px, nz, lamW, lhat, W):
    lib = require_gpu()
    done = 0
    while done < rows:
        nb = min(rows - done, 65535)
        _lib.check(lib.geobo_lattice_wbuild(nb, int(Py), int(Px), int(nz), _p(_chk(lamW, "lamW")),
                                            C.c_void_p(_chk(lhat, "lhat").data_ptr() + done * Py * Px * 8),
                                            C.c_void_p(_chk(W, "W").data_ptr() + done * Px * nz * Py * 8), _stream()), "geobo_lattice_wbuild")
        done += nb


def lattice_wplanes(rows, Py, Px, nz, lam3, lhat, W):
    lib = require_gpu()
    done = 0
    while done < rows:
        nb = min(rows - done, 65535)
        _lib.check(lib.geobo_lattice_wplanes(nb, int(Py), int(Px), int(nz), _p(_chk(lam3, "lam3")),
                                             C.c_void_p(_chk(lhat, "lhat").data_ptr() + done * Py * Px * 8),
                                             C.c_void_p(_chk(W, "W").data_ptr() + done * nz * Py * Px * 8), _stream()), "geobo_lattice_wplanes")
        done += nb


def xz2d_fold_inv_strided(n, rows, ppr, src, in_row, in_plane, Fx, Fz, out, out_row, out_plane, out_rowstride):
    lib = require_gpu()
    _lib.check(lib.geobo_xz2d_fold_inv_strided(int(n), int(rows), int(ppr), _p(_chk(src, "src")), int(in_row), int(in_plane), _p(_chk(Fx, "Fx")),
                                               _p(_chk(Fz, "Fz")), _p(_chk(out, "out")), int(out_row), int(out_plane), int(out_rowstride),
                                               _stream()), "geobo_xz2d_fold_inv_strided")


def xz2d_fold_inv_mul(n, rows, ppr, a, a_plane, b, b_row, Fx, Fz, out, out_row, out_plane, out_rowstride):
    lib = require_gpu()
    _lib.check(lib.geobo_xz2d_fold_inv_mul(int(n), int(rows), int(ppr), _p(_chk(a, "a")), int(a_plane), _p(_chk(b, "b")), int(b_row),
                                           _p(_chk(Fx, "Fx")), _p(_chk(Fz, "Fz")), _p(_chk(out, "out")), int(out_row), int(out_plane),
                                           int(out_rowstride), _stream()), "geobo_xz2d_fold_inv_mul")


def colgemv(X, v, out=None, ws=None):
    lib = require_gpu()
    ld = _rowmajor(X, "X")
    m, n = X.shape
    assert _chk(v, "v").numel() >= m
    if out is None:
        out = torch.empty(n, dtype=F64, device=X.device)
    nbytes = lib.geobo_colgemv_ws_bytes(m, n)
    if ws is None or ws.numel() * 8 < nbytes:
        ws = torch.empty(max(nbytes // 8, 1), dtype=F64, device=X.device)
    _lib.check(lib.geobo_colgemv(m, n, _p(X), ld, _p(v), _p(_chk(out, "out")), _p(ws), ws.numel() * 8, _stream()), "geobo_colgemv")
    return out


def rowgemv(X, v, out=None):
    lib = require_gpu()
    ld = _rowmajor(X, "X")
    m, n = X.shape
    assert v.numel() >= n and v.dtype == F64 and v.is_cuda
    if out is None:
        out = torch.empty(m, dtype=F64, device=X.device)
    _lib.check(lib.geobo_rowgemv(int(m), int(n), _p(X), int(ld), _p(v), _p(out), _stream()), "geobo_rowgemv")
    return out


def sumsq_accum(a, b, rows, ss):
    lib = require_gpu()
    lda = _rowmajor(a, "a")
    n = ss.shape[1]
    assert a.shape[1] >= n and a.shape[0] >= rows and _rowmajor(ss, "ss") >= n
    _lib.check(lib.geobo_sumsq_accum(int(rows), int(n), _p(a), lda, _p(b) if b is not None else None,
                                     _rowmajor(b, "b") if b is not None else 0, ss.shape[0], _p(ss), ss.stride(0), _stream()),
               "geobo_sumsq_accum")
    return ss


def lamdot_z(batch, planes, px, nz, D, lam, out):
    lib = require_gpu()
    _lib.check(lib.geobo_lamdot_z(int(batch), int(planes), int(px), int(nz), _p(_chk(D, "D")), _p(_chk(lam, "lam")), _p(_chk(out, "out")),
                                  _stream()), "geobo_lamdot_z")
    return out


def centro_fill(B, n, r0):
    lib = require_gpu()
    ld = _rowmajor(B, "B")
    assert B.shape[0] >= n and B.shape[1] >= n
    _lib.check(lib.geobo_centro_fill(_p(B), int(ld), int(n), int(r0), _stream()), "geobo_centro_fill")
    return B


def mirror_rows(X, m, r0, nb, nz):
    lib = require_gpu()
    ld = _rowmajor(X, "X")
    assert X.shape[0] >= m and X.shape[1] >= nb * nz
    _lib.check(lib.geobo_mirror_rows(_p(X), int(ld), int(m), int(r0), int(nb), int(nz), _stream()), "geobo_mirror_rows")
    return X


def mirror_dev_ws_doubles():
    return require_gpu().geobo_mirror_dev_ws_bytes() // 8


def mirror_dev(a, b, rows, nx, nz, out=None, ws=None):
    lib = require_gpu()
    lda, ldb = _rowmajor(a, "a"), _rowmajor(b, "b")
    assert a.shape[0] >= rows and b.shape[0] >= rows
    nws = lib.geobo_mirror_dev_ws_bytes() // 8
    if ws is None:
        ws = torch.empty(nws, dtype=F64, device=a.device)
    if out is None:
        out = torch.empty(2, dtype=F64, device=a.device)
    _lib.check(lib.geobo_mirror_dev(_p(a), int(lda), _p(b), int(ldb), int(rows), int(nx), int(nz), _p(_chk(out, "out")), _p(_chk(ws, "ws")),
                                    ws.numel() * 8, _stream()), "geobo_mirror_dev")
    return out


def convert(src, dst):
    lib = require_gpu()
    assert src.shape == dst.shape and src.dim() == 2 and src.stride(1) == 1 and dst.stride(1) == 1
    assert {src.dtype, dst.dtype} == {F64, F32}, "one side float64, the other float32"
    _lib.check(lib.geobo_convert(1 if dst.dtype == F32 else 0, _p(src), src.stride(0), _p(dst), dst.stride(0), src.shape[0],
                                 src.shape[1], _stream()), "geobo_convert")
    return dst


def round_f32_(x):
    lib = require_gpu()
    assert _chk(x, "x").is_contiguous()
    _lib.check(lib.geobo_round_f32(_p(x), x.numel(), _stream()), "geobo_round_f32")
    return x


def k_eval(kid, d2, l1, l2, w=1.0, amp=1.0):
    lib = require_gpu()
    d2 = _chk(d2, "d2").contiguous()
    out = torch.empty_like(d2)
    _lib.check(lib.geobo_k_eval(kid, _p(d2), d2.numel(), float(l1), float(l2), float(w), float(amp), _p(out), _stream()),
               "geobo_k_eval")
    return out


def lattice_plan(loc, xe, ye, ze, nx, ny, nz, device="cuda"):
    loc = np.asarray(loc, dtype=np.float64)
    xe, ye, ze = (np.asarray(v, dtype=np.float64) for v in (xe, ye, ze))
    if ny < 3 or nz % 2 or loc.shape != (nx * ny, 3) or np.unique(loc[:, 2]).size != 1:
        return None
    ux, uy = np.unique(loc[:, 0]), np.unique(loc[:, 1])
    if ux.size != nx or uy.size != ny:
        return None
    jx, jy = np.searchsorted(ux, loc[:, 0]), np.searchsorted(uy, loc[:, 1])
    if np.unique(jy * nx + jx).size != nx * ny:
        return None
    X = xe[:, None] - ux[None, :]
    Y = ye[1:ny, None] - uy[None, :]
    dix = np.arange(nx + 1)[:, None] - np.arange(nx)[None, :] + nx - 1
    diy = np.arange(1, ny)[:, None] - np.arange(ny)[None, :] + ny - 2
    dxv, dyv = np.empty(2 * nx), np.empty(2 * ny - 2)
    dxv[dix.ravel()] = X.ravel()
    dyv[diy.ravel()] = Y.ravel()
    if not ((dxv[dix] == X).all() and (dyv[diy] == Y).all()):
        return None
    dev = lambda a, dt: torch.as_tensor(np.ascontiguousarray(a, dtype=dt)).to(device)
    return dict(dxv=dev(dxv, np.float64), dyv=dev(dyv, np.float64), dzv=dev(ze - loc[0, 2], np.float64),
                jx=dev(jx, np.int32), jy=dev(jy, np.int32), rowmajor=bool((jy * nx + jx == np.arange(nx * ny)).all()))


def a_sens(func, B, loc, nx, ny, nz, xe, ye, ze, scale_mul, scale_div, out, iy0=0, iy1=None, plan=None, rows=None, ws=None,
           col_origin=0):
    lib = require_gpu()
    ld = _rowmajor(out, "A")
    col_origin = int(col_origin)
    base = _p(out)
    loc = _chk(loc, "loc").contiguous()
    Bh = (C.c_double * 3)(*[float(b) for b in B])
    iy1 = int(ny if iy1 is None else iy1)

    def direct(a, b):
        _lib.check(lib.geobo_a_sens_slab(FUNC_IDS[func], Bh, _p(loc), loc.shape[0], int(nx), int(ny), int(nz), _p(_chk(xe, "xe")),
                                         _p(_chk(ye, "ye")), _p(_chk(ze, "ze")), float(scale_mul), float(scale_div), int(a),
                                         int(b), base, ld, col_origin, _stream()), "geobo_a_sens_slab")
    if plan is None:
        direct(iy0, iy1)
        return out
    rows = slice(0, loc.shape[0]) if rows is None else rows
    jx, jy = plan["jx"][rows].contiguous(), plan["jy"][rows].contiguous()
    assert jx.numel() == loc.shape[0]
    nbytes = lib.geobo_a_sens_lattice_ws_bytes(int(nx), int(ny), int(nz))
    if ws is None or ws.numel() * 8 < nbytes:
        ws = torch.empty(nbytes // 8, dtype=F64, device=out.device)
    _lib.check(lib.geobo_a_sens_lattice(FUNC_IDS[func], Bh, loc.shape[0], int(nx), int(ny), int(nz), _p(plan["dxv"]), _p(plan["dyv"]),
                                        _p(plan["dzv"]), C.c_void_p(jx.data_ptr()), C.c_void_p(jy.data_ptr()), float(scale_mul),
                                        float(scale_div), int(iy0), iy1, base, ld, col_origin, _p(ws), nbytes, _stream()),
               "geobo_a_sens_lattice")
    if iy0 == 0:
        direct(0, 1)
    if iy1 == ny:
        direct(ny - 1, ny)
    return out


def potential(func, B, x, y, z):
    lib = require_gpu()
    x, y, z = (_chk(t, "xyz").contiguous() for t in (x, y, z))
    out = torch.empty_like(x)
    Bh = (C.c_double * 3)(*[float(b) for b in B])
    _lib.check(lib.geobo_potential(FUNC_IDS[func], Bh, _p(x), _p(y), _p(z), x.numel(), _p(out), _stream()), "geobo_potential")
    return out


def ak_fused(kid, A, xyz, col0, ncols, l1, l2, w, amp, out):
    lib = require_gpu()
    lda = _rowmajor(A, "A")
    ldo = _rowmajor(out, "AK")
    x, y, z = (_chk(t, "xyz") for t in xyz)
    Ms_pad, N_pad = A.shape
    assert x.numel() >= N_pad and out.shape[0] >= Ms_pad and out.shape[1] >= ncols
    _lib.check(lib.geobo_ak_fused(kid, _p(A), Ms_pad, N_pad, lda, _p(x), _p(y), _p(z), int(col0), int(ncols), float(l1),
                                  float(l2), float(w), float(amp), _p(out), ldo, _stream()), "geobo_ak_fused")
    return out


def ak_points(kid, A, grid_xyz, q_xyz, l1, l2, w, amp, out):
    lib = require_gpu()
    lda = _rowmajor(A, "A")
    ldo = _rowmajor(out, "out")
    x, y, z = (_chk(t, "grid_xyz") for t in grid_xyz)
    qx, qy, qz = (_chk(t, "q_xyz") for t in q_xyz)
    R_pad, N_pad = A.shape
    nq = qx.numel()
    assert min(x.numel(), y.numel(), z.numel()) >= N_pad and qy.numel() == nq and qz.numel() == nq
    assert all(t.is_contiguous() for t in (x, y, z, qx, qy, qz)) and out.shape[0] >= R_pad and out.shape[1] >= nq
    _lib.check(lib.geobo_ak_points(kid, _p(A), R_pad, N_pad, lda, _p(x), _p(y), _p(z), _p(qx), _p(qy), _p(qz), nq, float(l1),
                                   float(l2), float(w), float(amp), _p(out), ldo, _stream()), "geobo_ak_points")
    return out


def cov_table(kid, nx, ny, nz, sx, sy, sz, l1, l2, w, amp, device="cuda"):
    lib = require_gpu()
    tab = torch.empty(2 * int(nx) * int(ny) * int(nz), dtype=F64, device=device)
    _lib.check(lib.geobo_cov_table(kid, int(nx), int(ny), int(nz), float(sx), float(sy), float(sz), float(l1), float(l2),
                                   float(w), float(amp), _p(tab), _stream()), "geobo_cov_table")
    return tab


def ak_fused_grid(A, nx, ny, nz, table, col0, ncols, out):
    lib = require_gpu()
    lda = _rowmajor(A, "A")
    ldo = _rowmajor(out, "AK")
    Ms_pad, N_pad = A.shape
    assert out.shape[0] >= Ms_pad and out.shape[1] >= ncols and _chk(table, "table").numel() >= 2 * nx * ny * nz
    _lib.check(lib.geobo_ak_fused_grid(_p(A), Ms_pad, N_pad, lda, int(nx), int(ny), int(nz), _p(table), int(col0), int(ncols),
                                       _p(out), ldo, _stream()), "geobo_ak_fused_grid")
    return out


def gemm_nt(X, Y, C_, alpha=1.0, beta=0.0, lower_only=False, m_valid=0, small_tiles=False):
    lib = require_gpu()
    ldx, ldy, ldc = _rowmajor(X, "X"), _rowmajor(Y, "Y"), _rowmajor(C_, "C")
    m, k = X.shape
    n = Y.shape[0]
    assert Y.shape[1] == k and C_.shape[0] >= m and C_.shape[1] >= n
    _lib.check(lib.geobo_gemm_nt(m, n, k, float(alpha), _p(X), ldx, _p(Y), ldy, float(beta), _p(C_), ldc,
                                 (1 if lower_only else 0) | (2 if small_tiles else 0), int(m_valid), _stream()), "geobo_gemm_nt")
    return C_


def gemm_nt_splitk(X, Y, C_, splits, ws, lower_only=False, m_valid=0):
    lib = require_gpu()
    ldx, ldy, ldc = _rowmajor(X, "X"), _rowmajor(Y, "Y"), _rowmajor(C_, "C")
    m, k = X.shape
    n = Y.shape[0]
    assert Y.shape[1] == k and C_.shape[0] >= m and C_.shape[1] >= n and ws.numel() >= splits * m * n
    _lib.check(lib.geobo_gemm_nt_splitk(m, n, k, int(splits), _p(X), ldx, _p(Y), ldy, _p(C_), ldc, 1 if lower_only else 0,
                                        int(m_valid), _p(ws), ws.numel() * 8, _stream()), "geobo_gemm_nt_splitk")
    return C_


def gemm_nn(X, Y, C_, alpha=1.0, beta=0.0, x_lower=False, y_lower=False):
    lib = require_gpu()
    ldx, ldy, ldc = _rowmajor(X, "X"), _rowmajor(Y, "Y"), _rowmajor(C_, "C")
    m, k = X.shape
    n = Y.shape[1]
    assert Y.shape[0] == k and C_.shape[0] >= m and C_.shape[1] >= n
    _lib.check(lib.geobo_gemm_nn(m, n, k, float(alpha), _p(X), ldx, _p(Y), ldy, float(beta), _p(C_), ldc,
                                 1 if x_lower else 0, 1 if y_lower else 0, _stream()), "geobo_gemm_nn")
    return C_


def _check_extents(fn, ops, batch):
    for T, lead, stride, rows, cols, what in ops:
        last = (batch - 1) * int(stride) + (int(rows) - 1) * int(lead) + int(cols)
        room = T.untyped_storage().nbytes() // T.element_size() - T.storage_offset()
        if last > room:
            raise ValueError("%s: operand %s (%d x %d, ld %d, batch %d x stride %d) reads %d elements past its allocation"
                             % (fn, what, rows, cols, lead, batch, stride, last - room))


def axis_pass(fold, y_is_kn, inverse, *args):
    even = (4, 5, 7, 8) + ((10, 11) if not (y_is_kn or inverse) else ())
    if fold and all(int(args[i]) % 2 == 0 for i in even):
        return gemm_fold(y_is_kn, inverse, *args)
    return gemm_batched(y_is_kn, *args)


def gemm_fold_lamdot(px, nz, k, G, ldg, Y, ldy, strideY, lam, planes, out, batch):
    lib = require_gpu()
    _check_extents("geobo_gemm_fold_lamdot", ((G, ldg, 0, pad_n(px), k, "G"), (Y, ldy, strideY, k, pad_n(nz), "Y")), batch)
    done = 0
    while done < batch:
        nb = min(batch - done, 65535)
        _lib.check(lib.geobo_gemm_fold_lamdot(int(px), int(nz), int(k), _p(G), int(ldg), C.c_void_p(Y.data_ptr() + done * strideY * 8),
                                              int(ldy), int(strideY), _p(_chk(lam, "lam")), int(planes), int(done),
                                              C.c_void_p(out.data_ptr() + done * px * 8), int(nb), _stream()), "geobo_gemm_fold_lamdot")
        done += nb
    return out


def gemm_fold(y_is_kn, inverse, m, n, k, X, ldx, strideX, Y, ldy, strideY, C_, ldc, strideC, m_valid, n_valid, batch):
    lib = require_gpu()
    _check_extents("geobo_gemm_fold", ((X, ldx, strideX, m, k, "X"), (Y, ldy, strideY, k if y_is_kn else n, n if y_is_kn else k, "Y")), batch)
    done = 0
    while done < batch:
        nb = min(batch - done, 65535)
        _lib.check(lib.geobo_gemm_fold(1 if y_is_kn else 0, int(inverse), int(m), int(n), int(k),
                                       C.c_void_p(X.data_ptr() + done * strideX * 8), int(ldx), int(strideX),
                                       C.c_void_p(Y.data_ptr() + done * strideY * 8), int(ldy), int(strideY),
                                       C.c_void_p(C_.data_ptr() + done * strideC * 8), int(ldc), int(strideC), int(m_valid), int(n_valid),
                                       int(nb), _stream()), "geobo_gemm_fold")
        done += nb
    return C_


def gemm_batched(y_is_kn, m, n, k, X, ldx, strideX, Y, ldy, strideY, C_, ldc, strideC, m_valid, n_valid, batch, alpha=1.0,
                 beta=0.0):
    lib = require_gpu()
    done = 0
    esz = 8
    _check_extents("geobo_gemm_batched", ((X, ldx, strideX, m, k, "X"), (Y, ldy, strideY, k if y_is_kn else n, n if y_is_kn else k, "Y")), batch)
    while done < batch:
        nb = min(batch - done, 65535)
        _lib.check(lib.geobo_gemm_batched(1 if y_is_kn else 0, int(m), int(n), int(k), float(alpha),
                                          C.c_void_p(X.data_ptr() + done * strideX * esz), int(ldx), int(strideX),
                                          C.c_void_p(Y.data_ptr() + done * strideY * esz), int(ldy), int(strideY), float(beta),
                                          C.c_void_p(C_.data_ptr() + done * strideC * esz), int(ldc), int(strideC),
                                          int(m_valid), int(n_valid), int(nb), _stream()), "geobo_gemm_batched")
        done += nb
    return C_


def scale_broadcast(a, b, out):
    lib = require_gpu()
    _lib.check(lib.geobo_scale_broadcast(_p(_chk(a, "a")), _p(_chk(b, "b")), a.numel(), b.numel(), _p(out), _stream()),
               "geobo_scale_broadcast")
    return out


def scale_broadcast2(a, b0, b1, out0, out1):
    lib = require_gpu()
    _lib.check(lib.geobo_scale_broadcast2(_p(_chk(a, "a")), _p(_chk(b0, "b0")), _p(_chk(b1, "b1")), a.numel(), b0.numel(),
                                          _p(out0), _p(out1), _stream()), "geobo_scale_broadcast2")




def xz2d(inverse, nx, nz, rows, ppr, src, in_row, in_plane, Mx, Mz, out, out_row, out_plane):
    lib = require_gpu()
    _lib.check(lib.geobo_xz2d(1 if inverse else 0, int(nx), int(nz), int(rows), int(ppr), _p(_chk(src, "src")), int(in_row),
                              int(in_plane), _p(_chk(Mx, "Mx")), int(Mx.stride(0)), _p(_chk(Mz, "Mz")), int(Mz.stride(0)),
                              _p(_chk(out, "out")), int(out_row), int(out_plane), _stream()), "geobo_xz2d")




def xz2d_fold(inverse, n, rows, ppr, src, in_row, in_plane, Fx, Fz, out, out_row, out_plane):
    lib = require_gpu()
    _lib.check(lib.geobo_xz2d_fold(1 if inverse else 0, int(n), int(rows), int(ppr), _p(_chk(src, "src")), int(in_row), int(in_plane),
                                   _p(_chk(Fx, "Fx")), _p(_chk(Fz, "Fz")), _p(_chk(out, "out")), int(out_row), int(out_plane), _stream()),
               "geobo_xz2d_fold")


def xz2d_fold_quad(inverse, n, rows, groups, src, in_row, in_plane, Fx, Fz, out, out_row, out_plane):
    lib = require_gpu()
    _lib.check(lib.geobo_xz2d_fold_quad(1 if inverse else 0, int(n), int(rows), int(groups), _p(_chk(src, "src")), int(in_row), int(in_plane),
                                        _p(_chk(Fx, "Fx")), _p(_chk(Fz, "Fz")), _p(_chk(out, "out")), int(out_row), int(out_plane), _stream()),
               "geobo_xz2d_fold_quad")


def xz2d_fold_inv_ss_slots(n, rows, ppr):
    return _lib.load().geobo_xz2d_fold_inv_ss_slots(int(n), int(rows), int(ppr))


def xz2d_fold_inv_ss(n, rows, ppr, src, in_row, in_plane, Fx, Fz, ss, src2=None, in2_row=0, r2_first=0):
    lib = require_gpu()
    assert _chk(ss, "ss").numel() >= xz2d_fold_inv_ss_slots(n, rows, ppr) * ppr * n * n
    _lib.check(lib.geobo_xz2d_fold_inv_ss(int(n), int(rows), int(ppr), _p(_chk(src, "src")), int(in_row), int(in_plane),
                                          _p(_chk(src2, "src2")) if src2 is not None else None, int(in2_row), int(r2_first),
                                          _p(_chk(Fx, "Fx")), _p(_chk(Fz, "Fz")), _p(ss), _stream()), "geobo_xz2d_fold_inv_ss")


def tile_rows(m, m_valid, tile=256, group=64):
    m_valid = m if not m_valid or m_valid > m else m_valid
    out = []
    for r0 in range(0, m, tile):
        v = min(max(m_valid - r0, 0), tile)
        out.append((v + group - 1) // group * group)
    return out


def xz2d_fold_lattice(n, rows, ppr, Q, row_off, q_plane, edge, edge_row, Fx, Fz, out, out_row, out_plane):
    lib = require_gpu()
    assert row_off.dtype == torch.int64 and row_off.is_contiguous() and row_off.numel() >= rows
    _lib.check(lib.geobo_xz2d_fold_lattice(int(n), int(rows), int(ppr), _p(_chk(Q, "Q")), row_off.data_ptr(), int(q_plane),
                                           _p(_chk(edge, "edge")), int(edge_row), _p(_chk(Fx, "Fx")), _p(_chk(Fz, "Fz")),
                                           _p(_chk(out, "out")), int(out_row), int(out_plane), _stream()), "geobo_xz2d_fold_lattice")




def ymul(m, k, C, rows, G, src, in_row, out, out_row, fold=False):
    lib = require_gpu()
    fn, name = (lib.geobo_ymul_fold, "geobo_ymul_fold") if fold else (lib.geobo_ymul, "geobo_ymul")
    _lib.check(fn(int(m), int(k), int(C), int(rows), _p(_chk(G, "G")), int(G.stride(0)), _p(_chk(src, "src")), int(in_row),
                  _p(_chk(out, "out")), int(out_row), _stream()), name)


def xcorr_reduce(nx, nz, rows, planes, src, in_row, in_plane, Mx, lam, out, out_row, out_plane):
    lib = require_gpu()
    _lib.check(lib.geobo_xcorr_reduce(int(nx), int(nz), int(rows), int(planes), _p(_chk(src, "src")), int(in_row), int(in_plane),
                                      _p(_chk(Mx, "Mx")), int(Mx.stride(0)), _p(_chk(lam, "lam")), _p(_chk(out, "out")),
                                      int(out_row), int(out_plane), _stream()), "geobo_xcorr_reduce")


def xcorr_reduce_fold(n, rows, planes, src, in_row, in_plane, F, lam, out, out_row, out_plane):
    lib = require_gpu()
    _lib.check(lib.geobo_xcorr_reduce_fold(int(n), int(rows), int(planes), _p(_chk(src, "src")), int(in_row), int(in_plane),
                                           _p(_chk(F, "F")), _p(_chk(lam, "lam")), _p(_chk(out, "out")), int(out_row), int(out_plane),
                                           _stream()), "geobo_xcorr_reduce_fold")


def a_sens_lattice_stencil(ws, nx, ny, nz):
    np_ = (2 * ny - 2) * (2 * nx) * (nz + 1)
    return ws[np_:np_ + (2 * ny - 3) * (2 * nx - 1) * nz].view(2 * ny - 3, 2 * nx - 1, nz)






def toeplitz_y(ny, C, R, src, tabs, outs, y0=0, y1=None, plane=None, accumulate=False):
    lib = require_gpu()
    y1 = ny if y1 is None else y1
    n = len(tabs)
    assert 1 <= n <= 3 and len(outs) == n
    import ctypes
    tp = (ctypes.c_void_p * n)(*[t.data_ptr() for t in (_chk(t, "tab") for t in tabs)])
    op = (ctypes.c_void_p * n)(*[o.data_ptr() for o in (_chk(o, "out") for o in outs)])
    fn, name = (lib.geobo_toeplitz_y3_add, "geobo_toeplitz_y3_add") if accumulate else (lib.geobo_toeplitz_y3, "geobo_toeplitz_y3")
    _lib.check(fn(int(ny), int(C), int(C if plane is None else plane), int(R), n, _p(_chk(src, "src")), tp, op, int(y0), int(y1), _stream()), name)




def toeplitz_y2t(ny, C, R, src_g, src_m, tabs_g, tabs_m, outs, plane=None):
    lib = require_gpu()
    assert len(tabs_g) == 2 and len(tabs_m) == 2 and len(outs) == 2
    _lib.check(lib.geobo_toeplitz_y2t(int(ny), int(C), int(C if plane is None else plane), int(R), _p(_chk(src_g, "src_g")), _p(_chk(src_m, "src_m")),
                                      _p(_chk(tabs_g[0], "tab")), _p(_chk(tabs_g[1], "tab")), _p(_chk(tabs_m[0], "tab")), _p(_chk(tabs_m[1], "tab")),
                                      _p(_chk(outs[0], "out")), _p(_chk(outs[1], "out")), _stream()), "geobo_toeplitz_y2t")


def toeplitz_y2s(ny, C, R, src_g, src_m, tab_d0, tab_x, tab_d1, outs, plane=None):
    lib = require_gpu()
    assert len(outs) == 2
    _lib.check(lib.geobo_toeplitz_y2s(int(ny), int(C), int(C if plane is None else plane), int(R), _p(_chk(src_g, "src_g")), _p(_chk(src_m, "src_m")),
                                      _p(_chk(tab_d0, "tab")), _p(_chk(tab_x, "tab")), _p(_chk(tab_d1, "tab")),
                                      _p(_chk(outs[0], "out")), _p(_chk(outs[1], "out")), _stream()), "geobo_toeplitz_y2s")


_spectral_y_basis = {}


def spectral_y_basis(ny, device=None):
    lib = require_gpu()
    dev = torch.cuda.current_device() if device is None else torch.device(device).index
    b = _spectral_y_basis.get((ny, dev))
    if b is None:
        n = int(lib.geobo_spectral_y_basis_doubles(int(ny)))
        if n <= 0:
            raise RuntimeError("geobo_spectral_y: ny = %d is not instantiated" % ny)
        b = torch.empty(n, dtype=F64, device="cuda:%d" % dev)
        _lib.check(lib.geobo_spectral_y_basis(int(ny), _p(b), _stream()), "geobo_spectral_y_basis")
        _spectral_y_basis[(ny, dev)] = b
    return b


def spectral_y(ny, C, R, src, tabs, outs, y0=0, y1=None, plane=None, accumulate=False):
    lib = require_gpu()
    y1 = ny if y1 is None else y1
    n = len(tabs)
    assert 1 <= n <= 3 and len(outs) == n
    import ctypes
    tp = (ctypes.c_void_p * n)(*[t.data_ptr() for t in (_chk(t, "tab") for t in tabs)])
    op = (ctypes.c_void_p * n)(*[o.data_ptr() for o in (_chk(o, "out") for o in outs)])
    _lib.check(lib.geobo_spectral_y3(int(ny), int(C), int(C if plane is None else plane), int(R), n, _p(_chk(src, "src")), tp, op, int(y0), int(y1),
                                     1 if accumulate else 0, _p(spectral_y_basis(ny, src.device)), _stream()), "geobo_spectral_y3")


def spectral_y_lattice(ny, C, R, pool, row_off, edge, edge_row, order, tabs, outs, y0=0, y1=None, plane=None):
    lib = require_gpu()
    y1 = ny if y1 is None else y1
    n = len(tabs)
    assert 1 <= n <= 3 and len(outs) == n
    assert row_off.is_cuda and row_off.dtype == torch.int64 and row_off.is_contiguous() and row_off.numel() >= R
    assert order is None or (order.is_cuda and order.dtype == torch.int32 and order.is_contiguous() and order.numel() == R)
    basis = spectral_y_basis(ny, pool.device)
    for j in range(0, n, 2):
        two = j + 1 < n
        _lib.check(lib.geobo_spectral_y_lattice(int(ny), int(C), int(C if plane is None else plane), int(R), 2 if two else 1, _p(_chk(pool, "pool")),
                                                row_off.data_ptr(), _p(_chk(edge, "edge")), int(edge_row), order.data_ptr() if order is not None else None,
                                                _p(_chk(tabs[j], "tab")), _p(_chk(tabs[j + 1], "tab")) if two else None,
                                                _p(_chk(outs[j], "out")), _p(_chk(outs[j + 1], "out")) if two else None,
                                                int(y0), int(y1), _p(basis), _stream()), "geobo_spectral_y_lattice")




def spectral_y3t(ny, C, R, src_g, src_m, tabs_g, tabs_m, outs, plane=None):
    lib = require_gpu()
    n = len(outs)
    assert 1 <= n <= 3 and len(tabs_g) == n and len(tabs_m) == n
    import ctypes
    arr = lambda ts, what: (ctypes.c_void_p * n)(*[t.data_ptr() for t in (_chk(t, what) for t in ts)])
    _lib.check(lib.geobo_spectral_y3t(int(ny), int(C), int(C if plane is None else plane), int(R), n, _p(_chk(src_g, "src_g")), _p(_chk(src_m, "src_m")),
                                      arr(tabs_g, "tab"), arr(tabs_m, "tab"), arr(outs, "out"), _p(spectral_y_basis(ny, src_g.device)), _stream()),
               "geobo_spectral_y3t")




def spectral_axis(inverse, n, C, plane_in, plane_out, item_in, item_out, items, src, dst, mask_ends=False):
    lib = require_gpu()
    _lib.check(lib.geobo_spectral_axis(1 if inverse else 0, int(n), int(C), int(plane_in), int(plane_out), int(item_in), int(item_out), int(items),
                                       _p(_chk(src, "src")), _p(_chk(dst, "dst")), _p(spectral_y_basis(n, src.device)), 1 if mask_ends else 0, _stream()),
               "geobo_spectral_axis")
    return dst


def spectral_y2s(ny, C, R, src_g, src_m, tab_d0, tab_x, tab_d1, outs, plane=None):
    lib = require_gpu()
    assert len(outs) == 2
    _lib.check(lib.geobo_spectral_y2s(int(ny), int(C), int(C if plane is None else plane), int(R), _p(_chk(src_g, "src_g")), _p(_chk(src_m, "src_m")),
                                      _p(_chk(tab_d0, "tab")), _p(_chk(tab_x, "tab")), _p(_chk(tab_d1, "tab")),
                                      _p(_chk(outs[0], "out")), _p(_chk(outs[1], "out")), _p(spectral_y_basis(ny, src_g.device)), _stream()),
               "geobo_spectral_y2s")


class PotrfContext:

    def __init__(self):
        lib = require_gpu()
        self._h = C.c_void_p()
        _lib.check(lib.geobo_potrf_ctx_create(C.byref(self._h)), "geobo_potrf_ctx_create")

    @property
    def handle(self):
        return self._h

    def close(self):
        if getattr(self, "_h", None) is not None and self._h.value:
            _lib.load().geobo_potrf_ctx_destroy(self._h)
            self._h = C.c_void_p()

    def __del__(self):
        try:
            self.close()
        except Exception:
            pass


def potrf_inv(A, Linv=None, ws=None, ctx=None):
    lib = require_gpu()
    ld = _rowmajor(A, "A")
    m = A.shape[0]
    if Linv is None:
        Linv = torch.empty((m, m), dtype=F64, device=A.device)
    info = torch.zeros(1, dtype=torch.int32, device=A.device)
    nbytes = lib.geobo_potrf_ws_bytes(m)
    if ws is None or ws.numel() * 8 < nbytes:
        ws = torch.empty(max(nbytes // 8, 1), dtype=F64, device=A.device)
    _lib.check(lib.geobo_potrf_inv(m, _p(A), ld, _p(Linv), Linv.stride(0), _p(info), _p(ws), nbytes,
                                   ctx.handle if ctx is not None else None, _stream()), "geobo_potrf_inv")
    return Linv, info


def trmv_stats(Linv, y, L):
    lib = require_gpu()
    m = Linv.shape[0]
    u = torch.empty(m, dtype=F64, device=Linv.device)
    stats = torch.empty(2, dtype=F64, device=Linv.device)
    _lib.check(lib.geobo_trmv_stats(m, _p(Linv), _rowmajor(Linv, "Linv"), _p(_chk(y, "y")), _p(L), _rowmajor(L, "L"),
                                    _p(u), _p(stats), _stream()), "geobo_trmv_stats")
    return u, stats


def a_sens_lattice_ws_doubles(nx, ny, nz):
    return max(_lib.load().geobo_a_sens_lattice_ws_bytes(int(nx), int(ny), int(nz)) // 8, 1)


def potrf_ws_doubles(m):
    return max(_lib.load().geobo_potrf_ws_bytes(int(m)) // 8, 1)


def colgemv_ws_doubles(m, n):
    return max(_lib.load().geobo_colgemv_ws_bytes(int(m), int(n)) // 8, 1)


def posterior_ws_doubles(m, ncols):
    return max(_lib.load().geobo_posterior_ws_bytes(int(m), int(ncols)) // 8, 1)


def posterior_reduce(Linv, AK, u, prior_var, ws=None, m_valid=0):
    lib = require_gpu()
    m, ncols = AK.shape
    mu = torch.empty(ncols, dtype=F64, device=AK.device)
    var = torch.empty(ncols, dtype=F64, device=AK.device)
    nbytes = lib.geobo_posterior_ws_bytes(m, ncols)
    if ws is None or ws.numel() * 8 < nbytes:
        ws = torch.empty(max(nbytes // 8, 1), dtype=F64, device=AK.device)
    _lib.check(lib.geobo_posterior_reduce(m, ncols, _p(Linv), _rowmajor(Linv, "Linv"), _p(AK), _rowmajor(AK, "AK"),
                                          _p(_chk(u, "u")), float(prior_var), _p(mu), _p(var), int(m_valid), _p(ws), nbytes,
                                          _stream()),
               "geobo_posterior_reduce")
    return mu, var


def kinv_dot_ws_doubles(m, T):
    return max(_lib.load().geobo_kinv_dot_ws_bytes(int(m), int(T)) // 8, 1)


def kinv_dot(Linv, alpha, Gs, segs, ws=None, out=None):
    lib = require_gpu()
    m = Linv.shape[0]
    ldl = _rowmajor(Linv, "Linv")
    T = len(Gs)
# ... 457 lines not shown
```

geobo_amd/lattice_gram.py:

```python
import numpy as np

import torch

from . import hip

F64 = hip.F64


class LatticeGram:
    def __init__(self, sp, device):
        self.sp, self.device = sp, device
        self.nx, self.ny, self.nz = sp.nx, sp.ny, sp.nz
        self.Px, self.Py = sp.Px, sp.Py
        gy0 = sp.G["y"].clone()
        gy0[:, 0] = 0.0
        gy0[:, self.ny - 1] = 0.0
        self.Gy0 = gy0
        per_row = self.Py * self.Px * self.nz * 8
        self.R = self.Rz = 256 if self.fast(self.nx, self.ny, self.nz) else max(8, min(256, (2 << 30) // per_row))
        self.J = (self.ny + 63) // 64 * 64
        self._lam_oz = {}

    EDGE_ROWS = 1024

    def _edge_consts(self):
        if getattr(self, "_edge_c", None) is None:
            nx = self.nx
            P = 2 * nx
            i = np.arange(nx)
            F2 = np.zeros((hip.pad_n(2 * nx) // 2, 2, nx))
            F2[0, 0], F2[0, 1] = 1.0, (-1.0) ** i
            Fi = np.zeros((hip.pad_n(nx), nx, 2))
            Fi[:nx, 0, 0], Fi[:nx, 0, 1] = 1.0 / P, ((-1.0) ** i) / P
            for w in range(1, nx):
                ang = 2.0 * np.pi * ((w * i) % P) / P
                F2[w, 0], F2[w, 1] = np.cos(ang), np.sin(ang)
                Fi[:nx, w, 0], Fi[:nx, w, 1] = 2.0 / P * np.cos(ang), 2.0 / P * np.sin(ang)
            self._edge_c = (hip.to_dev(F2.reshape(-1, nx), self.device), hip.to_dev(Fi.reshape(-1, 2 * nx), self.device))
        return self._edge_c

    def edge_supported(self):
        return True

    def edge_eigen(self, E):
        nx, ny, nz, J = self.nx, self.ny, self.nz, self.J
        Kc_s, Ks_s, K64 = self._edge_spectra(E)
        V = torch.zeros((nx, 2, J, 2, nz), dtype=F64, device=self.device)
        V[1:, 0, :ny, 0], V[1:, 0, :ny, 1] = Kc_s[1:], Ks_s[1:]
        V[1:, 1, :ny, 0], V[1:, 1, :ny, 1] = -Ks_s[1:], Kc_s[1:]
        V[0, 0, :ny, 0] = Kc_s[0]
        V[0, 1, :ny, 1] = K64
        return V.view(nx, 2 * J, 2 * nz)

    def _edge_spectra(self, E):
        nx, ny, nz = self.nx, self.ny, self.nz
        F2, _ = self._edge_consts()
        Ev = E[:ny * nx]
        nzp = hip.pad_n(nz)
        kap = torch.zeros((2, ny, nx, nzp), dtype=F64, device=self.device)
        kap[0, :, :, :nz] = Ev[0::nx].reshape(ny, nx, nz)
        kap[1, :, 1:, :nz] = Ev[:, :nz].reshape(ny, nx, nz)[:, 1:]
        T = torch.empty((2 * ny * 2 * nx * nz + 4096,), dtype=F64, device=self.device)[:2 * ny * 2 * nx * nz].view(2, ny, 2 * nx, nz)
        hip.gemm_batched(True, hip.pad_n(2 * nx), nzp, nx, F2, nx, 0, kap, nzp, nx * nzp, T, nz, 2 * nx * nz, 2 * nx, nz, 2 * ny)
        T = T.view(2, ny, nx, 2, nz)
        even = T[0] + T[1]
        Ks = (T[0] - T[1])[:, :, 1]
        Kc = even[:, :, 0]
        return Kc.permute(1, 0, 2).contiguous(), Ks.permute(1, 0, 2).contiguous(), even[:, 0, 1].contiguous()

    def edge_rows(self, X, nrows, V, out):
        nx, ny, nz, sp, J = self.nx, self.ny, self.nz, self.sp, self.J
        pl, RB = nx * nz, self.EDGE_ROWS
        F2, FiT = self._edge_consts()
        assert X.stride(1) == 1 and X.stride(0) % 2 == 0 and out.stride(1) == 1
        nzp, nxp = hip.pad_n(nz), hip.pad_n(nx)
        end = X.storage_offset() + (nrows - 1) * X.stride(0) + pl + nzp
        if end > X.untyped_storage().nbytes() // 8:
            Xc = sp.buf("LG_EX", nrows * pl + nzp)[:nrows * pl].view(nrows, pl)
            Xc.copy_(X[:nrows, :pl])
            X = Xc
        for r0 in range(0, nrows, RB):
            R = min(RB, nrows - r0)
            Rp = (R + 127) // 128 * 128
            Xh = sp.buf("LG_EXh", RB * 2 * nx * max(nz, J))
            hip.gemm_batched(True, hip.pad_n(2 * nx), nzp, nx, F2, nx, 0, X[r0:], nz, X.stride(0), Xh, nz, 2 * nx * nz, 2 * nx, nz, R)
            o2 = sp.buf("LG_EO2", nx * 2 * max(J, nz) * RB)
            hip.gemm_batched(False, 2 * J, Rp, 2 * nz, V, 2 * nz, 2 * J * 2 * nz, Xh, 2 * nx * nz, 2 * nz, o2, Rp, 2 * J * Rp, 2 * J, R, nx)
            oT = sp.buf("LG_EOT", max(J, nz) * nx * RB)
            hip.gemm_batched(True, nxp, Rp, 2 * nx, FiT, 2 * nx, 0, o2, J * Rp, Rp, oT, Rp, nx * Rp, nx, R, ny)
            out[r0:r0 + R, :ny * nx] += oT[:ny * nx * Rp].view(ny * nx, Rp)[:, :R].t()

    def transpose_tables(self, lam):
        return lam.view(self.Py, self.nz, self.Px).permute(2, 1, 0).contiguous().view(-1)

    def _plane_yx(self, inverse, R, src, ld_src, dst, ld_dst):
        nx, ny, Px, Py, sp = self.nx, self.ny, self.Px, self.Py, self.sp
        form, fold = sp.forms.plane_yx, sp.forms.fold
        p_src, p_dst = (Py * Px, ny * nx) if inverse else (ny * nx, Py * Px)
        if form == "fold":
            hip.xz2d_fold(inverse, ny, R, 1, src, ld_src, p_src, sp.F["y"], sp.F["x"], dst, ld_dst, p_dst)
        elif form == "fused":
            M = sp.GT if inverse else sp.G
            hip.xz2d(inverse, ny, nx, R, 1, src, ld_src, p_src, M["y"], M["x"], dst, ld_dst, p_dst)
        elif inverse:
            t1 = sp.buf("LG_Bt", R * ny * Px + hip.pad_n(ny) * Px)
            hip.axis_pass(fold, True, True, hip.pad_n(ny), hip.pad_n(Px), Py, sp.GT["y"], Py, 0, src, Px, ld_src, t1, Px, ny * Px, ny, Px, R)
            hip.gemm_batched(True, hip.pad_n(ny), hip.pad_n(nx), Px, t1, Px, ny * Px, sp.G["x"], nx, 0, dst, nx, ld_dst, ny, nx, R)
        else:
            nyp = hip.pad_n(ny)
            end = src.storage_offset() + (R - 1) * ld_src + nyp * nx
            if end > src.untyped_storage().nbytes() // 8:
                Lc = sp.buf("LG_LX", R * ny * nx + nyp * nx)[:R * ny * nx].view(R, ny * nx)
                Lc.copy_(src[:R, :ny * nx])
                src, ld_src = Lc, ny * nx
            t1 = sp.buf("LG_Lt", R * ny * Px + nyp * Px)
            hip.axis_pass(fold, False, False, nyp, hip.pad_n(Px), nx, src, nx, ld_src, sp.G["x"], nx, 0, t1, Px, ny * Px, ny, Px, R)
            hip.axis_pass(fold, True, False, hip.pad_n(Py), hip.pad_n(Px), ny, sp.G["y"], ny, 0, t1, Px, ny * Px, dst, Px, ld_dst, Py, Px, R)

    def apply_transpose(self, Lrows, nrows, lamW, out):
        nx, ny, nz, Px, Py, sp = self.nx, self.ny, self.nz, self.Px, self.Py, self.sp
        assert Lrows.stride(1) == 1 and Lrows.stride(0) % 2 == 0 and out.stride(1) == 1
        if getattr(self, "_GyT0", None) is None:
            g = sp.GT["y"].clone()
            g[0] = 0.0
            g[ny - 1] = 0.0
            self._GyT0 = g
        R = self.Rz
        for r0 in range(0, nrows, R):
            Rb = min(R, nrows - r0)
            lh = sp.buf("LG_Lh", R * Py * Px)
            self._plane_yx(False, Rb, Lrows[r0:], Lrows.stride(0), lh, Py * Px)
            W = sp.buf("LG_W", R * Px * nz * Py)
            hip.lattice_wbuild(Rb, Py, Px, nz, lamW, lh, W)
            U = sp.buf("LG_U", R * nx * nz * Py)
            if sp.forms.x_axis4 and (nz * Py) % 16 == 0 and 2 * nx * nz * Py * 8 < (1 << 31):
                hip.spectral_axis(True, nx, nz * Py, nz * Py, nz * Py, Px * nz * Py, nx * nz * Py, Rb, W, U)
            else:
                hip.axis_pass(sp.forms.fold, True, True, hip.pad_n(nx), nz * Py, Px, sp.GT["x"], Px, 0, W, nz * Py, Px * nz * Py, U, nz * Py, nx * nz * Py, nx, nz * Py, Rb)
            hip.axis_pass(sp.forms.fold and 2, False, 2, hip.pad_n(ny), nx * nz, Py, self._GyT0, Py, 0, U, Py, nx * nz * Py, out[r0:], nx * nz, out.stride(0), ny, nx * nz, Rb)

    def transpose_tables3(self, lam):
        return lam.view(self.Py, self.nz, self.Px).permute(1, 0, 2).contiguous().view(-1)

    def zx_supported(self):
        return self.sp.forms.zx

    def apply_transpose_zx(self, Lrows, nrows, lam3, out):
        nx, ny, nz, Px, Py, sp = self.nx, self.ny, self.nz, self.Px, self.Py, self.sp
        assert self.zx_supported() and Lrows.stride(1) == 1 and Lrows.stride(0) % 2 == 0 and out.stride(1) == 1
        R = self.R
        for r0 in range(0, nrows, R):
            Rb = min(R, nrows - r0)
            lh = sp.buf("LG_Lh", R * Py * Px)
            self._plane_yx(False, Rb, Lrows[r0:], Lrows.stride(0), lh, Py * Px)
            if sp.forms.z_mul:
                hip.xz2d_fold_inv_mul(ny, Rb, nz, lam3, Py * Px, lh, Py * Px, sp.F["y"], sp.F["x"], out[r0:], out.stride(0), nx, nz * nx)
                continue
            W = sp.buf("LG_W", R * nz * Py * Px)
            hip.lattice_wplanes(Rb, Py, Px, nz, lam3, lh, W)
            hip.xz2d_fold_inv_strided(ny, Rb, nz, W, nz * Py * Px, Py * Px, sp.F["y"], sp.F["x"], out[r0:], out.stride(0), nx, nz * nx)

    def edge_eigen_t(self, E):
        nx, ny, nz, J = self.nx, self.ny, self.nz, self.J
        Kc_s, Ks_s, K64 = self._edge_spectra(E)
        spare = (hip.pad_n(2 * nz) - 2 * nz + 2 * nz - 1) // (2 * nz)
        Vt = torch.zeros((nx + max(spare, 1), 2, nz, 2, J), dtype=F64, device=self.device)
        Kc_t, Ks_t = Kc_s.transpose(1, 2), Ks_s.transpose(1, 2)
        Vt[1:nx, 0, :, 0, :ny], Vt[1:nx, 0, :, 1, :ny] = Kc_t[1:], -Ks_t[1:]
        Vt[1:nx, 1, :, 0, :ny], Vt[1:nx, 1, :, 1, :ny] = Ks_t[1:], Kc_t[1:]
        Vt[0, 0, :, 0, :ny] = Kc_t[0]
        Vt[0, 1, :, 1, :ny] = K64.t()
        return Vt.view(-1, 2 * nz, 2 * J)

    def edge_apply_transpose(self, Lrows, nrows, Vt, out, zx=False):
        nx, ny, nz, sp, J = self.nx, self.ny, self.nz, self.sp, self.J
        RB = self.EDGE_ROWS
        F2, FiT = self._edge_consts()
        nyp, nxp = hip.pad_n(ny), hip.pad_n(nx)
        end = Lrows.storage_offset() + (nrows - 1) * Lrows.stride(0) + nyp * nx
        if end > Lrows.untyped_storage().nbytes() // 8:
            Lc = sp.buf("LG_EX", nrows * ny * nx + nyp * nx)[:nrows * ny * nx].view(nrows, ny * nx)
            Lc.copy_(Lrows[:nrows, :ny * nx])
            Lrows = Lc
        for r0 in range(0, nrows, RB):
            R = min(RB, nrows - r0)
            Rp = (R + 127) // 128 * 128
            Lh = sp.buf("LG_EXh", RB * 2 * nx * max(nz, J))
            if ny < J:
                Lh.zero_()
            hip.gemm_batched(False, hip.pad_n(2 * nx), nyp, nx, F2, nx, 0, Lrows[r0:], nx, Lrows.stride(0), Lh, J, 2 * nx * J, 2 * nx, ny, R)
            o2 = sp.buf("LG_EO2", nx * 2 * max(J, nz) * RB)
            hip.gemm_batched(False, hip.pad_n(2 * nz), Rp, 2 * J, Vt, 2 * J, 2 * nz * 2 * J, Lh, 2 * nx * J, 2 * J, o2, Rp, 2 * nz * Rp, 2 * nz, R, nx)
            oT = sp.buf("LG_EOT", max(J, nz) * nx * RB)
            hip.gemm_batched(True, nxp, Rp, 2 * nx, FiT, 2 * nx, 0, o2, nz * Rp, Rp, oT, Rp, nx * Rp, nx, R, nz)
            res = oT[:nz * nx * Rp].view(nz, nx, Rp)[:, :, :R]
            if zx:
                out[r0:r0 + R, :nx * nz].view(R, nz, nx).copy_(res.permute(2, 0, 1))
            else:
                out[r0:r0 + R, :nx * nz].view(R, nx, nz).copy_(res.permute(2, 1, 0))

    @staticmethod
    def fast(nx, ny, nz):
        from .plan import lattice_gram_fast
        return lattice_gram_fast(nx, ny, nz)

    @staticmethod
    def supported(nx, ny, nz):
        from .plan import lattice_gram_supported
        return lattice_gram_supported(nx, ny, nz)

    def eigen(self, Q, tol=1e-11, extra=None):
        nx, ny, nz, Px, Py = self.nx, self.ny, self.nz, self.Px, self.Py
        cy, cx = ny - 2, nx - 1
        sp = self.sp
        Qh = sp.buf("LG_Qh", ny * nx * nz)[:ny * nx * nz].view(ny, nx, nz)
        Qh.zero_()
        Qh[:ny - 1] = Q[cy:cy + ny - 1, cx:cx + nx]
        dev = [Q.abs().max()]
        for sy, sx in ((-1, 1), (1, -1), (-1, -1)):
            ys = torch.arange(0, ny - 1, device=self.device) * sy + cy
            xs = torch.arange(0, nx, device=self.device) * sx + cx
            dev.append((Q[ys][:, xs] - Qh[:ny - 1]).abs().max())
        dev = torch.stack(dev)
        dev = (dev if extra is None else torch.cat([dev, extra.reshape(-1)])).tolist()
        dev, self.extra_host = dev[:4], dev[4:]
        if max(dev[1:]) > tol * dev[0]:
            return None
        T = sp.buf("LG_T", ny * Px * nz)
        hip.gemm_batched(True, hip.pad_n(Px), hip.pad_n(nz), nx, sp.E["x"], nx, 0, Qh, nz, nx * nz, T, nz, Px * nz, Px, nz, ny)
        lam = torch.empty(Py * Px * nz + 4096, dtype=F64, device=self.device)
        hip.gemm_batched(True, hip.pad_n(Py), hip.pad_n(Px * nz), ny, sp.E["y"], ny, 0, T, Px * nz, 0, lam, Px * nz, 0, Py, Px * nz, 1)
        lam[:Py * Px * nz].mul_(1.0 / float(Py * Px))
        return lam[:Py * Px * nz].view(Py, Px, nz).transpose(1, 2).contiguous().view(-1)

    def flops(self, rows, Ly=None):
        nx, ny, nz, Px, Py = self.nx, self.ny, self.nz, self.Px, self.Py
        Ly = ny if Ly is None else Ly
        f = self.sp.forms.gram_x == "fold"
        h = hb = 0.25 if f else 1.0
        zsum = 0.0 if self.fast(nx, ny, nz) else 2.0 * Py * Px * nz
        hy = 0.5 if (f and Ly in self.sp.forms.ymul_slabs) else 1.0
        return rows * (2.0 * (hy * hip.pad_n(Py) * nx * nz * Ly + h * Py * Px * nx * nz + hb * (ny * Py * Px + ny * nx * Px)) + zsum)

    def gram_rows(self, X, nrows, lam, out, y0=0, y1=None):
        nx, ny, nz, Px, Py = self.nx, self.ny, self.nz, self.Px, self.Py
        y1 = ny if y1 is None else y1
        Ly = y1 - y0
        assert Ly % 16 == 0
        sp, f = self.sp, self.sp.forms
        plane = nx * nz
        assert X.stride(1) == 1 and out.stride(1) == 1 and X.stride(0) % 2 == 0 and out.stride(0) % 2 == 0
        gy = self.Gy0[:, y0:]
        for r0 in range(0, nrows, self.R):
            R = min(self.R, nrows - r0)
            y1b = sp.buf("LG_Y1", R * Py * plane)
            if Ly in f.ymul_slabs and plane % 64 == 0:
                hip.ymul(Py, Ly, plane, R, gy, X[r0:], X.stride(0), y1b, Py * plane, fold=f.fold and y0 % 2 == 0)
            elif f.gram_y_axis4 and y0 == 0 and Ly == ny and plane % 16 == 0 and 2 * ny * plane * 8 < (1 << 31) and X.stride(0) >= ny * plane:
                hip.spectral_axis(False, ny, plane, plane, plane, X.stride(0), Py * plane, R, X[r0:], y1b, mask_ends=True)
            else:
                hip.axis_pass(f.fold and y0 % 2 == 0, True, False, hip.pad_n(Py), hip.pad_n(plane), Ly, gy, ny, 0, X[r0:], plane, X.stride(0),
                              y1b, plane, Py * plane, Py, plane, R)
            s = sp.buf("LG_S", R * Py * Px)
            if f.gram_x == "fold":
                hip.xcorr_reduce_fold(nx, R, Py, y1b, Py * plane, plane, sp.F["x"], lam, s, Py * Px, Px)
            elif f.gram_x == "plain":
                hip.xcorr_reduce(nx, nz, R, Py, y1b, Py * plane, plane, sp.G["x"], lam, s, Py * Px, Px)
            elif f.gram_x == "fold_lamdot":
                hip.gemm_fold_lamdot(Px, nz, nx, sp.G["x"], nx, y1b, nz, plane, self.lam_oz(lam), Py, s, R * Py)
            else:
                D = sp.buf("LG_D", R * Py * Px * nz)
                hip.axis_pass(f.fold, True, False, hip.pad_n(Px), hip.pad_n(nz), nx, sp.G["x"], nx, 0, y1b, nz, plane, D, nz, Px * nz, Px, nz, R * Py)
                hip.lamdot_z(R * Py, Py, Px, nz, D, self.lam_oz(lam), s)
            self._plane_yx(True, R, s, Py * Px, out[r0:], out.stride(0))

    def lam_oz(self, lam):
        hit = self._lam_oz.get(lam.data_ptr())
        if hit is None or hit[0] is not lam:
            self._lam_oz = {k: v for k, v in self._lam_oz.items() if v[0] is not lam}
            if len(self._lam_oz) > 4:
                self._lam_oz = {}
            hit = self._lam_oz[lam.data_ptr()] = (lam, lam.view(self.Py, self.nz, self.Px).transpose(1, 2).contiguous().view(-1))
        return hit[1]
```

geobo_amd/spectral.py:

```python
import math
import os

import numpy as np
import torch

from . import hip, plan
from .plan import INTEGER_BASIS_N, half_integer

F64 = hip.F64
SLACK = 4096


def base_modes(n):
    assert n % 4 == 0
    q = n // 4
    modes = [("cos", 0), ("mid", n // 2), ("cos", q), ("sin", q)]
    for om in range(1, q):
        modes += [("cos", om), ("sin", om), ("cos", n // 2 - om), ("sin", n // 2 - om)]
    return modes


def half_modes(n):
    assert n % 4 == 0
    modes = []
# ... 115 lines not shown
        return PooledRows(self.pool, self.row_off, self.edge, self.jy, self.jx, self.r0 + r0, self.geo)


class SpectralProduct:

    def __init__(self, nx, ny, nz, device, rows_per_batch=None, plane_pad=0, opts=None, forms=None):
        if nx % 16 or ny % 16 or nz % 16:
            raise ValueError("spectral path needs grid extents that are multiples of 16")
        self.nx, self.ny, self.nz = nx, ny, nz
        self.forms = f = forms or plan.stage_forms(nx, ny, nz, plan.switches(os.environ) if opts is None else opts)
        self.Px, self.Py, self.Pz = 2 * nx, 2 * ny, 2 * nz
        self.N, self.P3 = nx * ny * nz, self.Px * self.Py * self.Pz
        self.device = device
        dev = lambda a: hip.to_dev(a, device)
        axes = {"x": nx, "y": ny, "z": nz}
        self.G = {a: dev(_pad_rows(forward_matrix(n))) for a, n in axes.items()}
        self.GT = {a: dev(_pad_rows(forward_matrix(n).T.copy())) for a, n in axes.items()}
        self.E = {a: dev(_pad_rows(eigen_matrix(n))) for a, n in axes.items()}
        self.F = {a: dev(np.stack(folded_matrices(axes[a]), axis=2)) for a in f.folded_axes()}
        if f.xz == "quad":
            fe, fo = folded_matrices(32)
            fq = np.zeros((64, 32, 2))
            fq[:32, :16, 0], fq[:32, :16, 1] = fe, fo
            fq[32:, 16:, 0], fq[32:, 16:, 1] = fe, fo
            self.Fq = dev(fq)
        self._pairs = {}
        C, pad = self.Px * self.Pz, int(plane_pad)
        self.Cp = C + pad if (self.fused_xz and self.dense_y and C % 2048 == 0 and pad > 0) else C
        if rows_per_batch is None:
            per_row = (ny * self.Cp if self.dense_y else self.P3) * 8
            cap = 3 << 30
            rows_per_batch = max(1, min(256 if self.dense_y else 128, cap // per_row))
        g = 128 // math.gcd(nx * ny, 128)
        self.R = max(g, rows_per_batch // g * g)
        self._bufs = {}
        self._pool_tabs = {}
        self.kernel_timer = None

    pooled_feed = True

    def pool_applies(self):
        return bool(self.pooled_feed and self.forms.lattice_feed and self.forms.y == "mfma" and self.ny in (32, 48, 64))

    def pool_planes(self, Ms):
        return pool_layout(self.nx, self.ny, Ms, self.Cp)[3]

    def plane_pool(self, lattice, Ms, jy, jx):
        assert self.pool_applies()
        nx, ny, nz, Cp = self.nx, self.ny, self.nz, self.Cp
        nd = 2 * ny - 3
        n_int, edge_off, edge_row, planes = pool_layout(nx, ny, Ms, Cp)
        buf = self.buf("Pool", planes * Cp)
        hip.xz2d_fold(False, nx, nx, nd, lattice.Q, nz, lattice.q_plane, self.F["x"], self.F["z"], buf, nd * Cp, Cp)
        e0 = lattice.edge[lattice.r0:]
        edge = buf[edge_off:planes * Cp]
        hip.xz2d_fold(False, nx, Ms, 2, e0, lattice.edge.stride(0), nx * nz, self.F["x"], self.F["z"], edge, edge_row, Cp)
        jy, jx = np.ascontiguousarray(jy, dtype=np.int64)[:Ms], np.ascontiguousarray(jx, dtype=np.int64)[:Ms]
        rows = PooledRows(buf, None, edge, jy, jx)
        key = (rows.geo, Cp)
        row_off = self._pool_tabs.get(key)
        if row_off is None:
            row_off = self._pool_tabs[key] = torch.from_numpy(pool_row_off(nx, ny, Cp, jy, jx)).to(self.device)
        rows.row_off = row_off
        return rows

    def _pool_batch(self, A, r0, R):
        a = A.r0 + r0
        key = (A.geo, a, R)
        hit = self._pool_tabs.get(key)
        if hit is None:
            jy, jx = A.jy[a:a + R], A.jx[a:a + R]
            hit = self._pool_tabs[key] = (torch.from_numpy(pool_order(jy, jx)).to(self.device), pool_distinct_planes(self.ny, jy, jx))
        return hit

    def _ystage_pooled(self, A, r0, R, tabs, outs, y0, y1):
        ny, C, Cp = self.ny, self.Px * self.Pz, self.Cp
        order, distinct = self._pool_batch(A, r0, R)
        a = A.r0 + r0
        fn = lambda: hip.spectral_y_lattice(ny, C, R, A.pool, A.row_off[a:], A.edge[a * 2 * Cp:], 2 * Cp, order, tabs, outs, y0, y1, plane=Cp)
        name = "kernel:toeplitz_y" if len(tabs) >= 2 else "kernel:toeplitz_y_single"
        return self._launch(name, 8.0 * C * (distinct + R * len(tabs) * (y1 - y0)), R, self.y_stage_flop(1, len(tabs), y1 - y0), fn)

    dense_y = property(lambda self: self.forms.y != "spectrum")
    y_mfma = property(lambda self: self.forms.y == "mfma")
    fused_xz = property(lambda self: self.forms.xz in ("fold", "fused"))

    def _ystage(self, ny, C, R, src, tabs, outs, y0, y1, plane, accumulate=False):
        if self.y_mfma and (ny > 64 or not accumulate) and (ny <= 64 or 2 * (y1 - y0) >= ny):
            fn = lambda: hip.spectral_y(ny, C, R, src, tabs, outs, y0, y1, plane=plane, accumulate=accumulate)
        else:
            fn = lambda: hip.toeplitz_y(ny, C, R, src, tabs, outs, y0, y1, plane=plane, accumulate=accumulate)
        name = "kernel:toeplitz_y" if len(tabs) >= 2 or ny > 64 else "kernel:toeplitz_y_single"
        return self._launch(name, 8.0 * R * C * (ny + (2 if accumulate else 1) * len(tabs) * (y1 - y0)), R, self.y_stage_flop(1, len(tabs), y1 - y0), fn)

    def _launch(self, name, nbytes, rows, flop, fn):
        if self.kernel_timer is None:
            return fn()
        return self.kernel_timer(name, nbytes, fn, valu=rows * flop[1], flop=rows * flop[0])

    def buf(self, name, n):
        b = self._bufs.get(name)
        if b is None or b.numel() < n + SLACK:
            b = self._bufs[name] = _buf(n, self.device)
        return b

    def _paired(self, Mx, rows, cols):
        key = (Mx.data_ptr(), rows, cols)
        m2 = self._pairs.get(key)
        if m2 is None:
            m2 = torch.zeros((2 * rows, 2 * cols), dtype=Mx.dtype, device=Mx.device)
            m2[:rows, :cols] = Mx[:rows, :cols]
            m2[rows:, cols:] = Mx[:rows, :cols]
            self._pairs[key] = m2
        return m2

    def forward_zx(self, src, R, M, src_row_stride=None, out_name="T2"):
        nx, ny, nz, Px, Pz, Cp = self.nx, self.ny, self.nz, self.Px, self.Pz, self.Cp
        xz, analysis = self.forms.xz, M is self.G
        lds = self.N if src_row_stride is None else int(src_row_stride)
        t2 = self.buf(out_name, R * ny * Cp)
        if isinstance(src, LatticeRows):
            assert self.forms.lattice_feed and analysis
            hip.xz2d_fold_lattice(nx, R, ny, src.Q, src.row_off[src.r0:], src.q_plane, src.edge[src.r0:], src.edge.stride(0),
                                  self.F["x"], self.F["z"], t2, ny * Cp, Cp)
        elif xz == "fold" and analysis:
            hip.xz2d_fold(False, nx, R, ny, src, lds, nx * nz, self.F["x"], self.F["z"], t2, ny * Cp, Cp)
        elif xz in ("fold", "fused"):
            hip.xz2d(False, nx, nz, R, ny, src, lds, nx * nz, M["x"], M["z"], t2, ny * Cp, Cp)
        elif xz == "quad" and analysis:
            hip.xz2d_fold_quad(False, nx, R, ny // 4, src, lds, nx * nz, self.Fq, self.Fq, t2, ny * Cp, Cp)
        elif xz in ("quad", "pair"):
            hip.xz2d(False, 2 * nx, nz, R, ny // 2, src, lds, 2 * nx * nz, self._paired(M["x"], Px, nx), M["z"], t2, ny * Cp, 2 * Cp)
        else:
            fold = self.forms.fold and analysis
            t1 = self.buf("T1", R * ny * nx * Pz)
            hip.axis_pass(fold, False, False, hip.pad_n(ny * nx), hip.pad_n(Pz), nz, src, nz, lds, M["z"], nz, 0, t1, Pz, ny * nx * Pz, ny * nx, Pz, R)
            if self.forms.x_axis4 and analysis and Pz % 16 == 0:
                hip.spectral_axis(False, nx, Pz, Pz, Pz, nx * Pz, Px * Pz, R * ny, t1, t2)
            else:
                hip.axis_pass(fold, True, False, hip.pad_n(Px), hip.pad_n(Pz), nx, M["x"], nx, 0, t1, Pz, nx * Pz, t2, Pz, Px * Pz, Px, Pz, R * ny)
        return t2

    def forward(self, src, R, M, out_name="T3", src_row_stride=None):
        ny, Px, Py, Pz = self.ny, self.Px, self.Py, self.Pz
        t2 = self.forward_zx(src, R, M, src_row_stride)
        t3 = self.buf(out_name, R * self.P3)
        hip.gemm_batched(True, hip.pad_n(Py), hip.pad_n(Px * Pz), ny, M["y"], ny, 0, t2, Px * Pz, ny * Px * Pz, t3, Px * Pz,
                         self.P3, Py, Px * Pz, R)
        return t3

    def backward(self, spec, R, y0, y1, out, ldo):
        Px, Py, Pz = self.Px, self.Py, self.Pz
        slab = y1 - y0
        gyt = self.GT["y"][y0:]
        u2 = self.buf("U2", R * slab * Px * Pz)
        hip.gemm_batched(True, hip.pad_n(slab), hip.pad_n(Px * Pz), Py, gyt, Py, 0, spec, Px * Pz, self.P3, u2, Px * Pz,
                         slab * Px * Pz, slab, Px * Pz, R)
        self.backward_xz(u2, R, y0, y1, [(y0, y1, out, ldo)])

    def backward_xz(self, u2, R, ylo, yhi, targets):
        nx, nz, Px, Pz, Cp = self.nx, self.nz, self.Px, self.Pz, self.Cp
        Ly, xz = yhi - ylo, self.forms.xz
        whole = lambda k: all((yb - ya) % k == 0 for ya, yb, _, _ in targets)
        if xz == "fold":
            for ya, yb, out, ldo in targets:
                hip.xz2d_fold(True, nx, R, yb - ya, u2[(ya - ylo) * Cp:], Ly * Cp, Cp, self.F["x"], self.F["z"], out, ldo, nx * nz)
        elif xz == "fused":
            for ya, yb, out, ldo in targets:
                hip.xz2d(True, nx, nz, R, yb - ya, u2[(ya - ylo) * Cp:], Ly * Cp, Cp, self.GT["x"], self.GT["z"], out, ldo, nx * nz)
        elif xz == "quad" and whole(4):
            for ya, yb, out, ldo in targets:
                hip.xz2d_fold_quad(True, nx, R, (yb - ya) // 4, u2[(ya - ylo) * Cp:], Ly * Cp, Cp, self.Fq, self.Fq, out, ldo, nx * nz)
        elif xz in ("quad", "pair") and whole(2):
            for ya, yb, out, ldo in targets:
                hip.xz2d(True, 2 * nx, nz, R, (yb - ya) // 2, u2[(ya - ylo) * Cp:], Ly * Cp, 2 * Cp,
                         self._paired(self.GT["x"], nx, Px), self.GT["z"], out, ldo, 2 * nx * nz)
        else:
            fold = self.forms.fold
            u1 = self.buf("U1", R * Ly * nx * Pz)
            if self.forms.x_axis4 and Pz % 16 == 0:
                hip.spectral_axis(True, nx, Pz, Pz, Pz, Px * Pz, nx * Pz, R * Ly, u2, u1)
            else:
                hip.axis_pass(fold, True, True, hip.pad_n(nx), hip.pad_n(Pz), Px, self.GT["x"], Px, 0, u2, Pz, Px * Pz, u1, Pz, nx * Pz, nx, Pz, R * Ly)
            for ya, yb, out, ldo in targets:
                slab = yb - ya
                hip.axis_pass(fold, False, True, hip.pad_n(slab * nx), hip.pad_n(nz), Pz, u1[(ya - ylo) * nx * Pz:], Pz, Ly * nx * Pz,
                              self.GT["z"], Pz, 0, out, nz, ldo, slab * nx, nz, R)

    def flops(self, rows, nblocks, slab, fwd_planes=None):
        nx, ny, nz, Px, Py, Pz = self.nx, self.ny, self.nz, self.Px, self.Py, self.Pz
        pn = hip.pad_n
        fwd = 2.0 * (ny * nx * pn(Pz) * nz + ny * pn(Px) * pn(Pz) * nx)
        bwd = 2.0 * (slab * pn(nx) * pn(Pz) * Px + pn(slab * nx) * pn(nz) * Pz)
        xz = self.forms.xz
        if xz == "gemm" and self.forms.fold:
            fwd, bwd = 0.5 * fwd, 0.5 * bwd
        elif xz == "quad":
            fwd = 0.25 * ny * (64.0 * 64 * 128 + 128.0 * 64 * 128)
            bwd = 0.25 * slab * (128.0 * 128 * 64 + 64.0 * 128 * 64)
        elif xz == "pair":
            fwd += 2.0 * ny * Px * Pz * nx
            bwd += 2.0 * slab * nx * Pz * Px
        elif xz == "fold":
            fwd = 2.0 * ny * (0.5 * nx * pn(Pz) * nz + 0.25 * pn(Px) * pn(Pz) * nx)
            bwd = 0.25 * bwd
        if not self.dense_y:
            fwd += 2.0 * pn(Py) * Px * Pz * ny
            bwd += 2.0 * pn(slab) * Px * Pz * Py
        if fwd_planes is not None:
            fwd *= float(fwd_planes) / (rows * ny)
        return rows * (fwd + nblocks * bwd + (self.y_stage_flop(1, nblocks, slab)[0] if self.dense_y else 0.0))

    def y_stage_flop(self, terms, nblocks, slab=None, shared=False):
        ny, C = self.ny, self.Px * self.Pz
        if self.y_mfma and (ny <= 64 or slab is None or 2 * slab >= ny):
            valu = C * ny * (4.0 * terms + (7.0 * nblocks if terms == 1 else 10.0 * nblocks))
            return C * 1.0 * ny * ny * (terms + nblocks) + valu, valu
        outs = ny if (ny <= 64 or slab is None) else (slab + 15) // 16 * 16
        nprod = terms * nblocks * (0.75 if shared and terms == 2 and nblocks == 2 else 1.0)
        f = 2.0 * ny * outs * C * nprod
        return f, f

    def flops_valu(self, rows, nblocks, slab=None):
        return rows * self.y_stage_flop(1, nblocks, slab)[1] if self.dense_y else 0.0

    def eigenvalues(self, table_mirrored):
        nx, ny, nz = self.nx, self.ny, self.nz
        T = table_mirrored[:ny * nx * 2 * nz].view(ny, nx, 2 * nz)[:, :, nz - 1:2 * nz - 1].contiguous()
        src = self.buf("Tsrc", self.N)
        src[:self.N] = T.reshape(-1)
        if self.dense_y:
            C, Cp = self.Px * self.Pz, self.Cp
            gen = self.forward_zx(src, 1, self.E, out_name="Lam")[:ny * Cp].view(ny, Cp)[:, :C].clone().view(-1)
            gen.mul_(1.0 / float(C))
            return gen
        lam = self.forward(src, 1, self.E, out_name="Lam")[:self.P3].clone()
        lam.mul_(1.0 / float(self.P3))
        return lam

    def product(self, A, Ms, lam_list, outs, y0=0, y1=None, slabs=None):
        y1 = self.ny if y1 is None else y1
        if slabs is None:
            slabs = [(y0, y1, outs)]
        N = self.N
        if isinstance(A, PooledRows):
            assert self.pool_applies() and self.dense_y
        elif isinstance(A, LatticeRows):
            assert self.forms.lattice_feed
        else:
            assert A.stride(1) == 1 and A.stride(0) >= N and A.stride(0) % 2 == 0
        if self.dense_y:
            return self._product_dense_y(A, Ms, lam_list, slabs)
        for r0 in range(0, Ms, self.R):
            R = min(self.R, Ms - r0)
            spec = self.forward(A[r0:], R, self.G, src_row_stride=A.stride(0))
            n = R * self.P3
            j = 0
            while j < len(lam_list):
                if j + 1 < len(lam_list):
                    s0, s1 = self.buf("S", n), self.buf("S1", n)
                    hip.scale_broadcast2(spec[:n], lam_list[j], lam_list[j + 1], s0[:n], s1[:n])
                    for ya, yb, o in slabs:
                        self.backward(s0, R, ya, yb, o[j][r0:], o[j].stride(0))
                        self.backward(s1, R, ya, yb, o[j + 1][r0:], o[j + 1].stride(0))
                    j += 2
                else:
                    s0 = self.buf("S", n)
                    hip.scale_broadcast(spec[:n], lam_list[j], s0[:n])
                    for ya, yb, o in slabs:
                        self.backward(s0, R, ya, yb, o[j][r0:], o[j].stride(0))
                    j += 1

    def _product_dense_y(self, A, Ms, gens, slabs):
        ny, C, Cp = self.ny, self.Px * self.Pz, self.Cp
        ylo, yhi = min(s[0] for s in slabs), max(s[1] for s in slabs)
        n_out = (yhi - ylo) * Cp
        for r0 in range(0, Ms, self.R):
            R = min(self.R, Ms - r0)
            if isinstance(A, PooledRows):
                t2 = None
            elif isinstance(A, LatticeRows):
                t2 = self.forward_zx(A.rows(r0), R, self.G)
            else:
                t2 = self.forward_zx(A[r0:], R, self.G, src_row_stride=A.stride(0))
            for j in range(0, len(gens), 3):
                js = list(range(j, min(j + 3, len(gens))))
                u2 = [self.buf(("S", "S1", "S2")[i], R * n_out) for i in range(len(js))]
                if t2 is None:
                    for i in range(0, len(js), 2):
                        self._ystage_pooled(A, r0, R, [gens[jj] for jj in js[i:i + 2]], u2[i:i + 2], ylo, yhi)
                else:
                    self._ystage(ny, C, R, t2, [gens[jj] for jj in js], u2, ylo, yhi, Cp)
                for i, jj in enumerate(js):
                    self.backward_xz(u2[i], R, ylo, yhi, [(ya, yb, o[jj][r0:], o[jj].stride(0)) for ya, yb, o in slabs])

    def fused_ss(self):
        return self.forms.ss == "fused"

    GENERIC_SS_SLOTS = 8

    def ss_slots(self):
        return hip.xz2d_fold_inv_ss_slots(self.nx, self.R, self.ny) if self.fused_ss() else self.GENERIC_SS_SLOTS

    def y2s_tables(self, gens_g, gens_m, pair=(0, 1)):
        self.sym_residual = None
        a, b = pair
        if not (self.forms.y2s and b == a + 1 and a % 2 == 0 and b < len(gens_g)):
            return None
        x = gens_g[b]
        den = torch.maximum(x.abs().max(), gens_m[a].abs().max())
        self.sym_residual = (x - gens_m[a]).abs().max() / den.clamp_min(torch.finfo(x.dtype).tiny)
        return (a, gens_g[a] - x, x, gens_m[b] - x)

    def reduce_ss(self, Zg, Mg, gens_g, Zm, m_first, gens_m, ss, y2s=None):
        nx, ny, nz, C, Cp, R = self.nx, self.ny, self.nz, self.Px * self.Pz, self.Cp, self.R
        P_c, y2s_tabs, meet = len(gens_g), y2s, self.forms.y_two_term
        if Zm is None:
            m_first = Mg
        starts = list(range(0, min(m_first, Mg), R)) + list(range(m_first, Mg, R))
        if not self.fused_ss():
            N = self.N
            add_y = self.dense_y and meet == "add"
            for r0 in starts:
                two = r0 >= m_first
                Rb = min(R, (Mg if two else min(m_first, Mg)) - r0)
                vg = [self.buf("SSV%d" % jj, R * N)[:R * N].view(R, N) for jj in range(P_c)]
                if two and add_y:
                    t2g = self.forward_zx(Zg[r0:], Rb, self.G, src_row_stride=Zg.stride(0), out_name="T2")
                    t2m = self.forward_zx(Zm[r0 - m_first:], Rb, self.G, src_row_stride=Zm.stride(0), out_name="T2b")
                    for j in range(0, P_c, 3):
                        js = list(range(j, min(j + 3, P_c)))
                        u2 = [self.buf(("S", "S1", "S2")[i], Rb * ny * Cp) for i in range(len(js))]
                        if self.forms.y3t:
                            fn = lambda: hip.spectral_y3t(ny, C, Rb, t2g, t2m, [gens_g[jj] for jj in js], [gens_m[jj] for jj in js], u2, plane=Cp)
                            self._launch("kernel:toeplitz_y", 8.0 * Rb * C * ny * (2 + len(js)), Rb, self.y_stage_flop(2, len(js)), fn)
                        else:
                            self._ystage(ny, C, Rb, t2g, [gens_g[jj] for jj in js], u2, 0, ny, Cp)
                            self._ystage(ny, C, Rb, t2m, [gens_m[jj] for jj in js], u2, 0, ny, Cp, accumulate=True)
                        for i, jj in enumerate(js):
                            self.backward_xz(u2[i], Rb, 0, ny, [(0, ny, vg[jj], vg[jj].stride(0))])
                    for jj in range(P_c):
                        hip.sumsq_accum(vg[jj], None, Rb, ss[jj].view(ss[jj].shape[0], -1))
                    continue
                self.product(Zg[r0:], Rb, gens_g, vg)
                vm = None
                if two:
                    vm = [self.buf("SSW%d" % jj, R * N)[:R * N].view(R, N) for jj in range(P_c)]
                    self.product(Zm[r0 - m_first:], Rb, gens_m, vm)
                for jj in range(P_c):
                    hip.sumsq_accum(vg[jj], vm[jj] if two else None, Rb, ss[jj].view(ss[jj].shape[0], -1))
            return
        for r0 in starts:
            two = r0 >= m_first
            Rb = min(R, (Mg if two else min(m_first, Mg)) - r0)
            t2g = self.forward_zx(Zg[r0:], Rb, self.G, src_row_stride=Zg.stride(0), out_name="T2")
            t2m = self.forward_zx(Zm[r0 - m_first:], Rb, self.G, src_row_stride=Zm.stride(0), out_name="T2b") if two else None
            for j in range(0, P_c, 2):
                js = list(range(j, min(j + 2, P_c)))
                sg = [self.buf(("S", "S1")[i], Rb * ny * Cp) for i in range(len(js))]
                if two and len(js) == 2 and meet == "y2t":
                    if y2s_tabs is not None and y2s_tabs[0] == j:
                        y2s_fn = hip.spectral_y2s if self.y_mfma else hip.toeplitz_y2s
                        fn = lambda: y2s_fn(ny, C, Rb, t2g, t2m, y2s_tabs[1], y2s_tabs[2], y2s_tabs[3], sg, plane=Cp)
                        kname, nprod = "kernel:toeplitz_y2s", 3
                    else:
                        fn = lambda: hip.toeplitz_y2t(ny, C, Rb, t2g, t2m, [gens_g[jj] for jj in js], [gens_m[jj] for jj in js], sg, plane=Cp)
                        kname, nprod = "kernel:toeplitz_y2t", 4
                    self._launch(kname, 8.0 * Rb * C * (2 * ny + 2 * ny), Rb, self.y_stage_flop(2, 2, shared=nprod == 3), fn)
                    for i, jj in enumerate(js):
                        hip.xz2d_fold_inv_ss(nx, Rb, ny, sg[i], ny * Cp, Cp, self.F["x"], self.F["z"], ss[jj])
                    continue
                self._ystage(ny, C, Rb, t2g, [gens_g[jj] for jj in js], sg, 0, ny, Cp)
                sm = None
                if two and meet == "add":
                    self._ystage(ny, C, Rb, t2m, [gens_m[jj] for jj in js], sg, 0, ny, Cp, accumulate=True)
                elif two:
                    sm = [self.buf(("Sb", "S1b")[i], Rb * ny * Cp) for i in range(len(js))]
                    self._ystage(ny, C, Rb, t2m, [gens_m[jj] for jj in js], sm, 0, ny, Cp)
                for i, jj in enumerate(js):
                    hip.xz2d_fold_inv_ss(nx, Rb, ny, sg[i], ny * Cp, Cp, self.F["x"], self.F["z"], ss[jj],
                                         src2=sm[i] if sm is not None else None, in2_row=ny * Cp, r2_first=0)

    def flops_ss(self, rows_one, rows_two, nblocks, shared=False):
        nx, ny, nz, Px, Pz = self.nx, self.ny, self.nz, self.Px, self.Pz
        fwd = 1.0 * ny * (nx * nz * Pz + 0.5 * Px * nx * Pz)
        inv1, inv2 = 0.5 * ny * Px * Pz * nz, 0.5 * ny * nx * Px * nz
        terms = rows_one + 2 * rows_two
        y = rows_one * self.y_stage_flop(1, nblocks)[0] + rows_two * self.y_stage_flop(2, nblocks, shared=shared)[0]
        return terms * (fwd + nblocks * inv1) + (rows_one + rows_two) * nblocks * inv2 + y

    def valu_ss(self, rows_one, rows_two, nblocks, shared=False):
        return rows_one * self.y_stage_flop(1, nblocks)[1] + rows_two * self.y_stage_flop(2, nblocks, shared=shared)[1]
```

geobo_amd/transposed.py:

```python

import torch

from . import hip
from .operators import StreamedOperator

F64 = hip.F64


class TransposedPosteriorMixin:
    def _sym_ok(self, A_g, A_m):
        if not self._zpath_static_ok():
            return False
        return (self._gram is not None and self._gram.edge_supported() and self.Ms_pad == self.nx * self.ny
                and all(self._lam.get(f) is not None and self._lam[f][0] is A for f, A in (("grav", A_g), ("magn", A_m))))

    def _assemble_AkA_sym(self, step, AkA, AK, A_g, A_m):
        gram, pl, ny, Msp, nc = self._gram, self.nx * self.nz, self.ny, self.Ms_pad, self.nc
        Md, off_d, props = step.Md, 2 * self.Ms_pad, step.props
        lam = {0: self._lam["grav"][1], 1: self._lam["magn"][1]}
        ops = {0: A_g, 1: A_m}

        def edge_cols(sp_, k, iy):
            A = ops[sp_]
            if isinstance(A, StreamedOperator):
                return A.edge[:, k * pl:(k + 1) * pl] if A.lattice is not None else A.slab_into(self._workspace2d("op_slab", Msp, pl), iy, iy + 1)
            return A[:, iy * pl:(iy + 1) * pl]

        def rows_times_AT(X, nrows, sp_, out):
            gram.gram_rows(X, nrows, lam[sp_], out, 0, ny)
            for k, iy in enumerate((0, ny - 1)):
                gram.edge_rows(X[:, iy * pl:], nrows, self._edge_spectrum(("grav", "magn")[sp_], k, edge_cols(sp_, k, iy)), out)
        blk = lambda r0, j: AK[r0:, props.index(j) * nc:(props.index(j) + 1) * nc]

        Mm = step.mirror or self.Ms

        def run():
            rows_times_AT(blk(0, 0), self.Ms, 0, AkA[0:, 0:Msp])
            rows_times_AT(blk(0, 1), self.Ms, 1, AkA[0:, Msp:2 * Msp])
            rows_times_AT(blk(Msp, 1), Mm, 1, AkA[Msp:, Msp:2 * Msp])
            AkA[Msp:2 * Msp, :Msp] = AkA[:Msp, Msp:2 * Msp].t()
            if Md:
                rows_times_AT(blk(off_d, 0), Md, 0, AkA[off_d:, 0:Msp])
                rows_times_AT(blk(off_d, 1), Md, 1, AkA[off_d:, Msp:2 * Msp])
        self._timed("aka_lattice", gram.flops(2 * self.Ms + Mm + 2 * Md, ny), run)
        if step.mirror:
            self._timed("aka_centro_fill", 0.0, lambda: hip.centro_fill(AkA[Msp:Msp + self.Ms, Msp:Msp + self.Ms], self.Ms, (self.Ms + 1) // 2))
        return self._finish_AkA(step, AkA)

    def _zpath_static_ok(self):
        if not self.route.single or self.exchange:
            return False
        self._spectral_product()
        return True

    def _zpath_ok(self, step, AK):
        return (self._zpath_static_ok() and AK is not None and AK.dtype == F64
                and all((s_, j) in step.gens for s_ in (0, 1) for j in step.props))

    def _resident_operator(self, A, func):
        if not isinstance(A, StreamedOperator):
            return A
        R = self._workspace2d("A_" + func, self.Ms_pad, self.N_pad)
        xed, yed, zed = A.axes_dev
        hip.a_sens(A.func, A.Bv, A.locd, self.nx, self.ny, self.nz, xed, yed, zed, A.mul, A.div, R, plan=A.plan, ws=A.lws)
        return R

    def _lattice_Z(self, Lview, nrows, func, A, out, zx=False, edge=None):
        gram, pl, ny = self._gram, self.nx * self.nz, self.ny
        lam = self._lam[func][1]
        hit = self._lamW.get((func, zx))
        if hit is None or hit[0] is not lam:
            hit = self._lamW[(func, zx)] = (lam, gram.transpose_tables3(lam) if zx else gram.transpose_tables(lam))
        if zx:
            gram.apply_transpose_zx(Lview, nrows, hit[1], out)
        else:
            gram.apply_transpose(Lview, nrows, hit[1], out)
        for k, iy in enumerate((0, ny - 1)):
            if edge is not None:
                ycols = edge[k]
            elif isinstance(A, StreamedOperator) and A.lattice is not None:
                ycols = A.edge[:, k * pl:(k + 1) * pl]
            elif isinstance(A, StreamedOperator):
                ycols = A.slab_into(self._workspace2d("op_slab", self.Ms_pad, pl), iy, iy + 1)
            else:
                ycols = A[:, iy * pl:(iy + 1) * pl]
            key = (func, k)
            vt = self._edgeVt.get(key)
            if vt is None or vt[0] != ycols.data_ptr():
                vt = self._edgeVt[key] = (ycols.data_ptr(), gram.edge_eigen_t(ycols))
            gram.edge_apply_transpose(Lview, nrows, vt[1], out[:, iy * pl:(iy + 1) * pl], zx=zx)

    def _posterior_zpath(self, step, Linv, AK, u, A_g, A_m):
        props, Md, M_pad, amp = step.props, step.Md, step.M_pad, step.prior.amp
        sp, N, Msp, P_c = self._spectral, self.N, self.Ms_pad, len(props)
        nx, ny, nz = self.nx, self.ny, self.nz
        cws = self._workspace("colgemv_ws", (max(hip.colgemv_ws_doubles(M_pad, M_pad), hip.colgemv_ws_doubles(Msp, self.N_pad)),))
        w = self._timed("posterior_mean", 0.0, lambda: hip.colgemv(Linv, u, ws=cws))
        Zg, Zm = self._workspace2d("Zg", 2 * Msp, N), self._workspace2d("Zm", Msp, N)
        lat = (self._gram is not None and self._gram.edge_supported() and Msp == nx * ny and self.route.opt("z_lattice")
               and all(self._lam.get(f) is not None and self._lam[f][0] is A for f, A in (("grav", A_g), ("magn", A_m))))
        if lat:
            gram = self._gram
            fl = 3 * Msp * (gram.flops(1, ny) + 2 * 3 * 2.0 * 128 * 128 * 64)

            zx = gram.zx_supported()

            def zlattice():
                self._lattice_Z(Linv[:2 * Msp, :Msp], 2 * Msp, "grav", A_g, Zg, zx=zx)
                self._lattice_Z(Linv[Msp:2 * Msp, Msp:2 * Msp], Msp, "magn", A_m, Zm, zx=zx)
            self._timed("posterior_zlattice", fl, zlattice)
            Ag = Am = None
            vec_of = lambda func, wv, out: self._lattice_Z(wv.view(1, -1), 1, func, A_g if func == "grav" else A_m, out)
        else:
            Ag = self._timed("a_sens_grav", 0.0, lambda: self._resident_operator(A_g, "grav"))
            Am = self._timed("a_sens_magn", 0.0, lambda: self._resident_operator(A_m, "magn"))
            tri = sum(min(256 * (bi + 1), Msp) for bi in range(Msp // 256)) * 256.0
            fl = 2.0 * N * (2 * tri + 1.0 * Msp * Msp)
            alg = 2.0 * N * (2 * (Msp * (Msp + 1) / 2.0) + 1.0 * Msp * Msp)

            def zgemm():
                hip.gemm_nn(Linv[:2 * Msp, :Msp], Ag[:Msp, :N], Zg, x_lower=True)
                hip.gemm_nn(Linv[Msp:2 * Msp, Msp:2 * Msp], Am[:Msp, :N], Zm, x_lower=True)
            self._timed("posterior_zgemm", fl, zgemm, alg=alg)
            vec_of = lambda func, wv, out: hip.colgemv((Ag if func == "grav" else Am)[:Msp, :N], wv, out=out[0], ws=cws)
        mu_l = self._timed("posterior_mean", 0.0, lambda: self._mean_rows(step, w, vec_of)).reshape(-1)
        slots = hip.xz2d_fold_inv_ss_slots(nx, sp.R, ny)
        ss = [self._workspace("post_ss_%d" % jj, (slots, ny, nx * nz)) for jj in range(P_c)]
        for t in ss:
            t.zero_()
        gens_g, gens_m = [step.gens[(0, j)] for j in props], [step.gens[(1, j)] for j in props]
        zx = lat and zx
        swap = (lambda g: g.view(ny, sp.Px, sp.Pz).transpose(1, 2).contiguous().view(-1)) if zx else (lambda g: g)
        tg, tm = [swap(g) for g in gens_g], [swap(g) for g in gens_m]
        y2s = sp.y2s_tables(tg, tm) if tuple(props[:2]) == (0, 1) else None
        shared = y2s is not None and P_c == 2
        self._timed("posterior_spectral", sp.flops_ss(Msp, Msp, P_c, shared), lambda: sp.reduce_ss(Zg, 2 * Msp, tg, Zm, Msp, tm, ss, y2s=y2s),
                    valu=sp.valu_ss(Msp, Msp, P_c, shared))
        if zx:
            ssum = torch.stack([t.sum(0).view(ny, nz, nx).transpose(1, 2).reshape(-1) for t in ss])
        else:
            ssum = torch.stack([t.sum(0).reshape(-1) for t in ss])
        if Md:
            ssum = ssum + self._timed("posterior_drill_rows", 0.0, lambda: self._drill_rows_ss(
                step, Linv, 0, Md, (lambda Lv, n, func, out: self._lattice_Z(Lv, n, func, A_g if func == "grav" else A_m, out)) if lat else None, Ag, Am))
        return mu_l, (amp * 1.0 - ssum).reshape(-1)

    def _mean_rows(self, step, w, vec_of):
        props, sel_t, Md = step.props, step.sel_t, step.Md
        sp, N, Msp, P_c = self._spectral, self.N, self.Ms_pad, len(props)
        V = self._workspace2d("mean_rows", 4, N)
        vec_of("grav", w[:Msp], V[0:1])
        vec_of("magn", w[Msp:2 * Msp], V[1:2])
        terms = [(V[0:1], 0), (V[1:2], 1)]
        if Md:
            V[2].zero_()
            V[2][sel_t] = w[2 * Msp:2 * Msp + Md]
            terms.append((V[2:3], 2))
        mu = torch.zeros((P_c, N), dtype=F64, device=self.device)
        tmp = [self._workspace2d("mean_tmp_%d" % jj, 2, N) for jj in range(P_c)]
        for rows, s_ in terms:
            gens = [step.gens[(s_, j)] if s_ < 2 else sp.eigenvalues(step.prior.table(self, s_, j)) for j in props]
            sp.product(rows, 1, gens, tmp)
            for jj in range(P_c):
                mu[jj].add_(tmp[jj][0])
        return mu

    def _drill_rows_ss(self, step, Linv, d0, nd, lattice_Z, Ag, Am):
        props, sel_t, Md = step.props, step.sel_t, step.Md
        sp, N, Msp, P_c, T = self._spectral, self.N, self.Ms_pad, len(props), 128
        Zgd, Zmd, Zdd = (self._workspace2d(nm, T, N) for nm in ("Zg_d", "Zm_d", "Zd_d"))
        Vd = [self._workspace2d("Vd_%d" % jj, T, N) for jj in range(P_c)]
        tmp = [self._workspace2d("Vt_%d" % jj, T, N) for jj in range(P_c)]
        gens_g, gens_m = [step.gens[(0, j)] for j in props], [step.gens[(1, j)] for j in props]
        gens_d = [sp.eigenvalues(step.prior.table(self, 2, j)) for j in props]
        acc = torch.zeros((P_c, N), dtype=F64, device=self.device)
        for c0 in range(d0, d0 + nd, T):
            n = min(T, d0 + nd - c0)
            b0 = 2 * Msp + c0
            if lattice_Z is not None:
                lattice_Z(Linv[b0:b0 + n, :Msp], n, "grav", Zgd)
                lattice_Z(Linv[b0:b0 + n, Msp:2 * Msp], n, "magn", Zmd)
            else:
                nt = min(T, Linv.shape[0] - b0)
                hip.gemm_nn(Linv[b0:b0 + nt, :Msp], Ag[:Msp, :N], Zgd)
                hip.gemm_nn(Linv[b0:b0 + nt, Msp:2 * Msp], Am[:Msp, :N], Zmd)
            Zdd[:n].zero_()
            Zdd[:n, sel_t] = Linv[b0:b0 + n, 2 * Msp:2 * Msp + Md]
            sp.product(Zgd, n, gens_g, Vd)
            for Zx, gx in ((Zmd, gens_m), (Zdd, gens_d)):
                sp.product(Zx, n, gx, tmp)
                for jj in range(P_c):
                    Vd[jj][:n].add_(tmp[jj][:n])
            for jj in range(P_c):
                acc[jj].add_((Vd[jj][:n] ** 2).sum(0))
        return acc
```

include/geobo_hip.h:

```cpp
#ifndef GEOBO_HIP_H
#define GEOBO_HIP_H

#include <stddef.h>
#include <stdint.h>

#ifdef __cplusplus
extern "C" {
#endif

#define GEOBO_VERSION 212


#define GEOBO_PAD_M 256
#define GEOBO_PAD_N 128

enum { GEOBO_OK = 0, GEOBO_E_ARG = -1, GEOBO_E_ALIGN = -2, GEOBO_E_LAUNCH = -3, GEOBO_E_UNSUPPORTED = -4 };

enum {
  GEOBO_K_D2 = 0,
  GEOBO_K_EXP = 1,
  GEOBO_K_EXP_X = 2,
  GEOBO_K_MATERN32 = 3,
  GEOBO_K_MATERN32_X = 4,
  GEOBO_K_SPARSE = 5,
  GEOBO_K_SPARSE_X = 6
};

enum { GEOBO_F_GRAV = 0, GEOBO_F_MAGN = 1 };

int geobo_version(void);
int64_t geobo_pad_m(int64_t m);
int64_t geobo_pad_n(int64_t n);

int geobo_k_block(int kernel_id, const double* rx, const double* ry, const double* rz, int64_t nr,
                  const double* cx, const double* cy, const double* cz, int64_t nc,
                  double l1, double l2, double w, double amp, double* out, int64_t ld, void* stream);

int geobo_k_block_f32(int kernel_id, const double* rx, const double* ry, const double* rz, int64_t nr,
                      const double* cx, const double* cy, const double* cz, int64_t nc,
                      double l1, double l2, double w, double amp, float* out, int64_t ld, void* stream);

int geobo_k_block_grid(int nx, int ny, int nz, const double* table, const int64_t* rows, int64_t row0, int64_t nr, int64_t col0,
                       int64_t ncols, int out_f32, void* out, int64_t ld, void* stream);

size_t geobo_colgemv_ws_bytes(int64_t m, int64_t n);
int geobo_colgemv(int64_t m, int64_t n, const double* X, int64_t ld, const double* v, double* out, void* ws, size_t ws_bytes,
                  void* stream);

int geobo_lattice_wbuild(int64_t rows, int Py, int Px, int nz, const double* lamW, const double* lhat, double* W, void* stream);
int geobo_lattice_wplanes(int64_t rows, int Py, int Px, int nz, const double* lam3, const double* lhat, double* W, void* stream);

int geobo_convert(int to_f32, const void* src, int64_t ld_src, void* dst, int64_t ld_dst, int64_t rows, int64_t cols,
                  void* stream);
int geobo_round_f32(double* x, int64_t n, void* stream);

int geobo_k_eval(int kernel_id, const double* d2, int64_t n, double l1, double l2, double w, double amp,
                 double* out, void* stream);

int geobo_a_sens(int func_id, const double* B3_host, const double* loc, int64_t Ms, int nx, int ny, int nz,
                 const double* xe, const double* ye, const double* ze, double scale_mul, double scale_div,
                 double* A, int64_t ld, void* stream);

int geobo_a_sens_slab(int func_id, const double* B3_host, const double* loc, int64_t Ms, int nx, int ny, int nz,
                      const double* xe, const double* ye, const double* ze, double scale_mul, double scale_div,
                      int iy0, int iy1, double* A, int64_t ld, int64_t col_origin, void* stream);

size_t geobo_a_sens_lattice_ws_bytes(int nx, int ny, int nz);
int geobo_a_sens_lattice(int func_id, const double* B3_host, int64_t Ms, int nx, int ny, int nz, const double* dxv,
                         const double* dyv, const double* dzv, const int* jxs, const int* jys, double scale_mul,
                         double scale_div, int iy0, int iy1, double* A, int64_t ld, int64_t col_origin, void* ws, size_t ws_bytes,
                         void* stream);

int geobo_potential(int func_id, const double* B3_host, const double* x, const double* y, const double* z, int64_t n,
                    double* out, void* stream);

int geobo_ak_fused(int kernel_id, const double* A, int64_t Ms_pad, int64_t N_pad, int64_t lda,
                   const double* x, const double* y, const double* z, int64_t col0, int64_t ncols,
                   double l1, double l2, double w, double amp, double* AK, int64_t ldak, void* stream);

int geobo_ak_points(int kernel_id, const double* A, int64_t R_pad, int64_t N_pad, int64_t lda,
                    const double* px, const double* py, const double* pz,
                    const double* qx, const double* qy, const double* qz, int64_t nq_pad,
                    double l1, double l2, double w, double amp, double* out, int64_t ldo, void* stream);

int geobo_cov_table(int kernel_id, int nx, int ny, int nz, double sx, double sy, double sz, double l1, double l2,
                    double w, double amp, double* table, void* stream);
int geobo_ak_fused_grid(const double* A, int64_t Ms_pad, int64_t N_pad, int64_t lda, int nx, int ny, int nz,
                        const double* table, int64_t col0, int64_t ncols, double* AK, int64_t ldak, void* stream);

#define GEOBO_GEMM_LOWER_ONLY 1
#define GEOBO_GEMM_SMALL_TILES 2
int geobo_gemm_nt(int64_t m, int64_t n, int64_t k, double alpha, const double* X, int64_t ldx,
                  const double* Y, int64_t ldy, double beta, double* C, int64_t ldc, int lower_only, int64_t m_valid,
                  void* stream);

int64_t geobo_tile_order(int nbi, int nbj, int tm, int tn, int lower_only, int x_lower, int y_lower, int* out_host,
                         int64_t capacity);

int geobo_gemm_nt_splitk(int64_t m, int64_t n, int64_t k, int splits, const double* X, int64_t ldx, const double* Y,
                         int64_t ldy, double* C, int64_t ldc, int lower_only, int64_t m_valid, void* ws, size_t ws_bytes,
                         void* stream);

int geobo_gemm_nn(int64_t m, int64_t n, int64_t k, double alpha, const double* X, int64_t ldx,
                  const double* Y, int64_t ldy, double beta, double* C, int64_t ldc,
                  int x_lower, int y_lower, void* stream);

int geobo_gemm_batched(int y_is_kn, int64_t m, int64_t n, int64_t k, double alpha, const double* X, int64_t ldx,
                       int64_t strideX, const double* Y, int64_t ldy, int64_t strideY, double beta, double* C, int64_t ldc,
                       int64_t strideC, int64_t m_valid, int64_t n_valid, int batch, void* stream);

int geobo_gemm_fold(int y_is_kn, int inverse, int64_t m, int64_t n, int64_t k, const double* X, int64_t ldx, int64_t strideX,
                    const double* Y, int64_t ldy, int64_t strideY, double* C, int64_t ldc, int64_t strideC, int64_t m_valid,
                    int64_t n_valid, int64_t batch, void* stream);

int geobo_gemm_fold_lamdot(int64_t px, int64_t nz, int64_t k, const double* G, int64_t ldg, const double* Y, int64_t ldy, int64_t strideY,
                           const double* lam, int planes, int64_t batch0, double* out, int64_t batch, void* stream);

int geobo_scale_broadcast(const double* a, const double* b, int64_t n, int64_t nb, double* out, void* stream);
int geobo_scale_broadcast2(const double* a, const double* b0, const double* b1, int64_t n, int64_t nb, double* out0,
                           double* out1, void* stream);

int geobo_xz2d(int inverse, int nx, int nz, int64_t rows, int planes_per_row, const double* in, int64_t in_row,
               int64_t in_plane, const double* Mx, int64_t ldmx, const double* Mz, int64_t ldmz, double* out,
               int64_t out_row, int64_t out_plane, void* stream);

int geobo_xz2d_fold(int inverse, int n, int64_t rows, int planes_per_row, const double* in, int64_t in_row, int64_t in_plane,
                    const double* Fx, const double* Fz, double* out, int64_t out_row, int64_t out_plane, void* stream);

int geobo_xcorr_reduce(int nx, int nz, int64_t rows, int planes, const double* in, int64_t in_row, int64_t in_plane,
                       const double* Mx, int64_t ldmx, const double* lamT, double* out, int64_t out_row, int64_t out_plane,
                       void* stream);

int geobo_xz2d_fold_lattice(int n, int64_t rows, int planes_per_row, const double* Q, const int64_t* row_off, int64_t q_plane,
                            const double* edge, int64_t edge_row, const double* Fx, const double* Fz, double* out,
                            int64_t out_row, int64_t out_plane, void* stream);

int geobo_xz2d_fold_inv_strided(int n, int64_t rows, int planes_per_row, const double* in, int64_t in_row, int64_t in_plane,
                                const double* Fx, const double* Fz, double* out, int64_t out_row, int64_t out_plane,
                                int64_t out_rowstride, void* stream);

int geobo_xz2d_fold_inv_mul(int n, int64_t rows, int planes_per_row, const double* a, int64_t a_plane, const double* b, int64_t b_row,
                            const double* Fx, const double* Fz, double* out, int64_t out_row, int64_t out_plane,
                            int64_t out_rowstride, void* stream);

int geobo_xz2d_fold_quad(int inverse, int n, int64_t rows, int groups_per_row, const double* in, int64_t in_row, int64_t in_plane,
                         const double* Fx, const double* Fz, double* out, int64_t out_row, int64_t out_plane, void* stream);

int geobo_xz2d_fold_inv_ss_slots(int n, int64_t rows, int planes_per_row);
int geobo_xz2d_fold_inv_ss(int n, int64_t rows, int planes_per_row, const double* in, int64_t in_row, int64_t in_plane,
                           const double* in2, int64_t in2_row, int64_t r2_first, const double* Fx, const double* Fz, double* ss,
                           void* stream);

int geobo_ymul(int m, int k, int64_t C, int64_t rows, const double* G, int64_t ldg, const double* in, int64_t in_row,
               double* out, int64_t out_row, void* stream);
int geobo_ymul_fold(int m, int k, int64_t C, int64_t rows, const double* G, int64_t ldg, const double* in, int64_t in_row,
                    double* out, int64_t out_row, void* stream);

int geobo_xcorr_reduce_fold(int n, int64_t rows, int planes, const double* in, int64_t in_row, int64_t in_plane,
                            const double* F, const double* lamT, double* out, int64_t out_row, int64_t out_plane, void* stream);

int geobo_toeplitz_y(int ny, int64_t C, int64_t plane, int64_t R, int nprop, const double* in, const double* tab0, const double* tab1,
                     double* out0, double* out1, int y0, int y1, void* stream);

int geobo_toeplitz_y2t(int ny, int64_t C, int64_t plane, int64_t R, const double* in_g, const double* in_m, const double* tab_g0,
                       const double* tab_g1, const double* tab_m0, const double* tab_m1, double* out0, double* out1, void* stream);

int geobo_toeplitz_y2s(int ny, int64_t C, int64_t plane, int64_t R, const double* in_g, const double* in_m, const double* tab_d0,
                       const double* tab_x, const double* tab_d1, double* out0, double* out1, void* stream);

int geobo_toeplitz_y3(int ny, int64_t C, int64_t plane, int64_t R, int nprop, const double* in, const double* const* tabs,
                      double* const* outs, int y0, int y1, void* stream);
int geobo_toeplitz_y3_add(int ny, int64_t C, int64_t plane, int64_t R, int nprop, const double* in, const double* const* tabs,
                          double* const* outs, int y0, int y1, void* stream);

int64_t geobo_spectral_y_basis_doubles(int ny);
int geobo_spectral_y_basis(int ny, double* basis, void* stream);
int geobo_spectral_y(int ny, int64_t C, int64_t plane, int64_t R, int nprop, const double* in, const double* tab0, const double* tab1,
                     double* out0, double* out1, int y0, int y1, const double* basis, void* stream);
int geobo_spectral_y2s(int ny, int64_t C, int64_t plane, int64_t R, const double* in_g, const double* in_m, const double* tab_d0,
                       const double* tab_x, const double* tab_d1, double* out0, double* out1, const double* basis, void* stream);

int geobo_spectral_y_lattice(int ny, int64_t C, int64_t plane, int64_t R, int nprop, const double* pool, const int64_t* row_off,
                             const double* edge, int64_t edge_row, const int32_t* order, const double* tab0, const double* tab1,
                             double* out0, double* out1, int y0, int y1, const double* basis, void* stream);

int geobo_spectral_y3(int ny, int64_t C, int64_t plane, int64_t R, int nprop, const double* in, const double* const* tabs,
                      double* const* outs, int y0, int y1, int accumulate, const double* basis, void* stream);

int geobo_spectral_y3t(int ny, int64_t C, int64_t plane, int64_t R, int nprop, const double* in_g, const double* in_m,
                       const double* const* tabs_g, const double* const* tabs_m, double* const* outs, const double* basis, void* stream);

int geobo_spectral_axis(int inverse, int n, int64_t C, int64_t plane_in, int64_t plane_out, int64_t item_in, int64_t item_out, int64_t items,
                        const double* in, double* out, const double* basis, int mask_ends, void* stream);

size_t geobo_potrf_ws_bytes(int64_t m);
int geobo_potrf_ctx_create(void** ctx);
int geobo_potrf_ctx_destroy(void* ctx);
int geobo_potrf_inv(int64_t m, double* A, int64_t ld, double* Linv, int64_t ldi, int* info, void* ws,
                    size_t ws_bytes, void* ctx, void* stream);

int geobo_rowgemv(int64_t m, int64_t n, const double* X, int64_t ld, const double* v, double* out, void* stream);

int geobo_sumsq_accum(int64_t rows, int64_t n, const double* a, int64_t lda, const double* b, int64_t ldb, int slots, double* ss,
                      int64_t ld_ss, void* stream);

int geobo_lamdot_z(int64_t batch, int planes, int px, int nz, const double* D, const double* lam, double* out, void* stream);

int geobo_centro_fill(double* B, int64_t ld, int64_t n, int64_t r0, void* stream);
int geobo_mirror_rows(double* X, int64_t ld, int64_t m, int64_t r0, int64_t nb, int nz, void* stream);
size_t geobo_mirror_dev_ws_bytes(void);
int geobo_mirror_dev(const double* a, int64_t lda, const double* b, int64_t ldb, int64_t rows, int nx, int nz, double* out2, void* ws,
                     size_t ws_bytes, void* stream);

size_t geobo_posterior_ws_bytes(int64_t m, int64_t ncols);
int geobo_posterior_reduce(int64_t m, int64_t ncols, const double* Linv, int64_t ldi, const double* AK, int64_t ldak,
                           const double* u, double prior_var, double* mu, double* var, int64_t m_valid, void* ws,
                           size_t ws_bytes, void* stream);

size_t geobo_kinv_dot_ws_bytes(int64_t m, int T);
int geobo_kinv_dot(int64_t m, const double* Linv, int64_t ldl, const double* alpha, int T, const double* const* G, int64_t ldg,
                   const int64_t* seg, double* out, void* ws, size_t ws_bytes, void* stream);

int geobo_trmv_stats(int64_t m, const double* Linv, int64_t ldi, const double* y, const double* L, int64_t ld,
                     double* u, double* stats, void* stream);

int geobo_mfma_f64_peak(int blocks, int iters, double* out, void* stream);

int geobo_mfma_mix(int mode, int nv, int blocks, int iters, double* out, void* stream);

enum { GEOBO_RNG_PRIOR = 0, GEOBO_RNG_OBS = 1 };
#define GEOBO_FFT_INVERSE 1
#define GEOBO_FFT_IN_PAIRS 2
#define GEOBO_FFT_OUT_PAIRS 4
#define GEOBO_FFT_MAX 512

int geobo_philox_fill(int mode, uint64_t seed, uint64_t purpose, int64_t sample0, int64_t nsamples, int64_t elem0, int64_t nelem,
                      uint64_t sub, double* out, void* stream);

int geobo_torus_table(int kernel_id, int my, int mx, int mz, double sx, double sy, double sz, double l1, double l2, double w, double amp,
                      double* out, void* stream);

int geobo_fft_lines(int m, int64_t b1);

int geobo_fft_axis(int flags, int64_t b0, int m, int64_t b1, int n_in, int n_out, const double* in, double* out, int P, int64_t Q,
                   int64_t S, void* stream);

size_t geobo_sample_factor_ws_bytes(void);
int geobo_sample_factor(int P, int my, int mx, int mz, const double* spectra, double* F, double* lam, void* ws, size_t ws_bytes,
                        double* status, void* stream);

int geobo_sample_zpass(int P, int64_t pair0, int64_t npairs, int my, int mx, int mz, int nz, const double* F, const double* noise,
                       uint64_t seed, double* out, void* stream);

int geobo_spectral_mix(int P, int64_t npairs, int my, int mx, int mz, const double* lam, double scale, const double* in, double* out,
                       void* stream);

int geobo_set_gram(int64_t C, int k, const int32_t* idx, int64_t R, const double* V, int64_t ldv, int64_t ncols, int accumulate,
                   double* G, void* stream);

int geobo_set_logdet(int64_t C, int k, const double* G, const double* Kpp, int64_t kpp_stride, double sigma2, const int32_t* idx,
                     const uint8_t* observed, int64_t n_obs, double* out, int* status, void* stream);

size_t geobo_kinv_diag_ws_bytes(int64_t m);
int geobo_kinv_diag(int64_t m, const double* Linv, int64_t ldl, const double* u, double* d, double* alpha, void* ws, size_t ws_bytes,
                    void* stream);

int geobo_set_loo(int64_t C, int k, const double* G, const int32_t* idx, const double* alpha, int64_t n, double* out, double* resid,
                  double* var, double* white, int* status, void* stream);

size_t geobo_block_cov_ws_bytes(int64_t R, int ny, int nx, int nz, int by, int bx, int bz);
int geobo_block_cov(int64_t R, const double* V0, const double* V1, const double* V2, int64_t ldv, int ny, int nx, int nz, int by,
                    int bx, int bz, int accumulate, double* C6, void* ws, size_t ws_bytes, void* stream);

int geobo_box_means(int64_t S, const double* F, int64_t sstride, int64_t pstride, int ny, int nx, int nz, int by, int bx, int bz,
                    double* G, int32_t* count, void* stream);

size_t geobo_cutoff_stats_ws_bytes(int64_t S, int64_t n, int C);
int geobo_cutoff_stats(int64_t S, const double* F, int64_t sstride, int64_t pstride, int64_t n, int p, int C, const double* t,
                       const double* lo, const uint8_t* mask, const int32_t* weight, int64_t* cnt, double* sum, uint32_t* hits,
                       void* ws, size_t ws_bytes, void* stream);

enum { GEOBO_BODIES_INIT = 1, GEOBO_BODIES_MERGE = 2, GEOBO_BODIES_FLATTEN = 4, GEOBO_BODIES_STATS = 8, GEOBO_BODIES_ALL = 15, GEOBO_BODIES_TILED = 16 };
size_t geobo_bodies_ws_bytes(int64_t S, int ny, int nx, int nz, int C);
int geobo_bodies(int64_t S, const double* F, int64_t sstride, int64_t pstride, int ny, int nx, int nz, int p, int C, const double* t,
                 const double* lo, const uint8_t* mask, const int32_t* weight, int neighbours, int64_t min_count, int64_t K,
                 const int32_t* seeds, int64_t* stats, double* sums, uint32_t* hits_largest, uint32_t* hits_seeded, int32_t* labels,
                 int32_t* info, int phases, void* ws, size_t ws_bytes, void* stream);

size_t geobo_trace_stats_ws_bytes(int64_t S, int64_t K, int C);
int geobo_trace_stats(int64_t S, const double* F, int64_t sstride, int64_t pstride, int ny, int nx, int nz, int p, int C, const double* t,
                      const double* lo, const uint8_t* mask, int64_t K, const int32_t* offsets, const int32_t* voxels, int Lmax,
                      int min_len, int max_gap, int64_t* tab, uint32_t* hits_any, uint32_t* hits, int64_t* thick_sum, int64_t* top_sum,
                      double* acc_sum, uint32_t* hist_len, uint32_t* hist_thick, int32_t* detail, double* dsum, void* ws, size_t ws_bytes,
                      void* stream);

#ifdef __cplusplus
}
#endif
#endif
```

Measured before the change: 2.346 million.

## Add transposed-X GEMM mode, fuse lattice edge transposes, shorten drill-row variance path

Adds a Y_NT_XT GEMM mode that reads X stored k-major through a padded LDS tile. The lattice edge products now write straight into the output, accumulating with beta=1, instead of going through a temporary and a PyTorch transpose-add or permute-copy. A dedicated HIP transpose kernel replaces a strided torch .t() copy. Drill-row posterior variance gets a short path that reuses the two-term spectral product and a GEMM against existing AK columns, which saves memory traffic and extra kernels at the cost of more code paths and alignment constraints.

```diff
diff --git a/geobo_amd/_lib.py b/geobo_amd/_lib.py
--- a/geobo_amd/_lib.py
+++ b/geobo_amd/_lib.py
@@ -23,6 +23,7 @@
     "geobo_sumsq_accum": (_int, [_i64, _i64, _dp, _i64, _dp, _i64, _int, _dp, _i64, _dp]),
     "geobo_lamdot_z": (_int, [_i64, _int, _int, _int, _dp, _dp, _dp, _dp]),
     "geobo_centro_fill": (_int, [_dp, _i64, _i64, _i64, _dp]),
+    "geobo_transpose": (_int, [_i64, _i64, _dp, _i64, _dp, _i64, _dp]),
     "geobo_mirror_rows": (_int, [_dp, _i64, _i64, _i64, _i64, _int, _dp]),
     "geobo_mirror_dev_ws_bytes": (_sz, []),
     "geobo_mirror_dev": (_int, [_dp, _i64, _dp, _i64, _i64, _int, _int, _dp, _dp, _sz, _dp]),
diff --git a/geobo_amd/csrc/gemm_f64.hip b/geobo_amd/csrc/gemm_f64.hip
--- a/geobo_amd/csrc/gemm_f64.hip
+++ b/geobo_amd/csrc/gemm_f64.hip
@@ -19,7 +19,8 @@
   return (p & 1) | (((p >> 2) & 1) * 6);
 }
 
-enum { Y_GEN = 0, Y_NT = 1, Y_NN = 2, Y_TAB = 3 };
+enum { Y_GEN = 0, Y_NT = 1, Y_NN = 2, Y_TAB = 3, Y_NT_XT = 4 };
+constexpr bool mem_mode(int y) { return y == Y_NT || y == Y_NN || y == Y_NT_XT; }
 enum { EPI_STORE = 0, EPI_REDUCE = 1 };
 enum { TRI_LOWER_ONLY = 1, TRI_X_LOWER = 2, TRI_Y_LOWER = 4 };
 
@@ -85,15 +86,18 @@
 template <int WM, int WN, int YMODE>
 constexpr int lds_doubles() {
   constexpr int TM = 64 * WM, TN = 64 * WN;
+  constexpr int xbuf = (YMODE == Y_NT_XT) ? BK * (TM + 4) : TM * XS;
   constexpr int ybuf = (YMODE == Y_NN) ? BK * (TN + 4) : TN * XS;
-  return ring_depth<WM, WN>() * (TM * XS + ybuf);
+  return ring_depth<WM, WN>() * (xbuf + ybuf);
 }
 
 template <int WM, int WN, int YMODE, int EPI, int KID>
 __global__ void __launch_bounds__(64 * WM * WN, 2) gemm_f64_kernel(const GemmArgs a) {
   constexpr int TM = 64 * WM, TN = 64 * WN, NT = 64 * WM * WN;
-  constexpr int YS_NN = TN + 4;
-  constexpr int XBUF = TM * XS;
+  constexpr bool XT = (YMODE == Y_NT_XT), YNT = (YMODE == Y_NT || XT);
+  static_assert(!XT || TM == 128, "transposed X: 128-row tiles");
+  constexpr int YS_NN = TN + 4, XS_T = TM + 4;
+  constexpr int XBUF = XT ? BK * XS_T : TM * XS;
   constexpr int YBUF = (YMODE == Y_NN) ? BK * YS_NN : TN * XS;
   constexpr int XU = TM * 8 / NT;
   constexpr int YU = (YMODE == Y_NN) ? (8 * TN / NT) : (TN * 8 / NT);
@@ -160,7 +164,7 @@
 #pragma unroll
     for (int n = 0; n < 4; ++n) acc[m][n] = (v4d){0., 0., 0., 0.};
   bool c_in_acc = false;
-  if constexpr (EPI == EPI_STORE && (YMODE == Y_NT || YMODE == Y_NN)) {
+  if constexpr (EPI == EPI_STORE && mem_mode(YMODE)) {
     c_in_acc = a.beta != 0.0 && (a.beta == a.alpha || a.beta == -a.alpha);
     if (c_in_acc) {
       const double sgn = (a.beta == a.alpha) ? 1.0 : -1.0;
@@ -195,13 +199,20 @@
     xsrc[i] = (grow * a.ldx + 2 * ((tid & 7) ^ swz(row))) * 8;
   }
   auto stage_x = [&](int64_t k0, int st) {
+    if constexpr (XT) {
+#pragma unroll
+      for (int i = 0; i < BK * 64 / NT; ++i) {
+        const int kr = i * (NT / 64) + wave;
+        dma16(Xp + (k0 + kr) * a.ldx + row0 + 2 * lane, Xs + st * XBUF + kr * XS_T);
+      }
+    } else
 #pragma unroll
     for (int i = 0; i < XU; ++i) dma16(Xgb + xsrc[i] + k0 * 8, Xs + st * XBUF + (i * RPI + wave * 8) * XS);
   };
 
-  int64_t ysrc[(YMODE == Y_NT) ? YU : 1];
-  const char* const Ygb = (YMODE == Y_NT) ? reinterpret_cast<const char*>(Yp + col0 * a.ldy) : nullptr;
-  if constexpr (YMODE == Y_NT) {
+  int64_t ysrc[YNT ? YU : 1];
+  const char* const Ygb = YNT ? reinterpret_cast<const char*>(Yp + col0 * a.ldy) : nullptr;
+  if constexpr (YNT) {
 #pragma unroll
     for (int i = 0; i < YU; ++i) {
       const int row = i * RPI + srow;
@@ -240,7 +251,7 @@
   }
 
   auto stage_y = [&](int64_t k0, int st) {
-    if constexpr (YMODE == Y_NT) {
+    if constexpr (YNT) {
 #pragma unroll
       for (int i = 0; i < YU; ++i) dma16(Ygb + ysrc[i] + k0 * 8, Ys + st * YBUF + (i * RPI + wave * 8) * XS);
     } else if constexpr (YMODE == Y_NN) {
@@ -294,12 +305,18 @@
 
   if (kb < ke) {
     const int xoff0 = 2 * ((2 * lg + 0) ^ swz(lr)), xoff1 = 2 * ((2 * lg + 1) ^ swz(lr));
-    const double* const xfrag = Xs + (wm * 64 + lr) * XS;
+    const double* const xfrag = XT ? (Xs + wm * 64 + lr) : (Xs + (wm * 64 + lr) * XS);
     const double* const yfrag = (YMODE == Y_NN) ? (Ys + wn * 64 + lr) : (Ys + (wn * 64 + lr) * XS);
     auto read_half = [&](int stage, int h, v2d (&av)[4], v2d (&bv)[4]) {
-      const double* xb = xfrag + stage * XBUF + (h ? xoff1 : xoff0);
-#pragma unroll
-      for (int m = 0; m < 4; ++m) av[m] = *reinterpret_cast<const v2d*>(xb + m * 16 * XS);
+      if constexpr (XT) {
+        const double* xb = xfrag + stage * XBUF + (4 * lg + 2 * h) * XS_T;
+#pragma unroll
+        for (int m = 0; m < 4; ++m) { av[m][0] = xb[m * 16]; av[m][1] = xb[XS_T + m * 16]; }
+      } else {
+        const double* xb = xfrag + stage * XBUF + (h ? xoff1 : xoff0);
+#pragma unroll
+        for (int m = 0; m < 4; ++m) av[m] = *reinterpret_cast<const v2d*>(xb + m * 16 * XS);
+      }
       if constexpr (YMODE == Y_NN) {
         const double* yb = yfrag + stage * YBUF + (4 * lg + 2 * h) * YS_NN;
 #pragma unroll
@@ -557,11 +574,11 @@
   if (a.m_valid <= 0) a.m_valid = (int64_t)1 << 62;
   if (a.n_valid <= 0) a.n_valid = (int64_t)1 << 62;
   a.xcd_map = (a.nbi >= 8) ? 1 : 0;
-  if ((YMODE == Y_NT || YMODE == Y_NN) && !(a.tri & TRI_LOWER_ONLY) && a.nbi >= 4 && a.nbj >= 8) a.xcd_map = 2;
+  if (mem_mode(YMODE) && !(a.tri & TRI_LOWER_ONLY) && a.nbi >= 4 && a.nbj >= 8) a.xcd_map = 2;
   a.ntiles = 0;
   if (a.batch <= 0) a.batch = 1;
   const int64_t items = (int64_t)a.nbi * a.nbj * a.batch;
-  if ((YMODE == Y_NT || YMODE == Y_NN) && EPI == EPI_STORE && a.batch <= 64 &&
+  if (mem_mode(YMODE) && EPI == EPI_STORE && a.batch <= 64 &&
       a.nbi * a.nbj >= ((a.tri & (TRI_X_LOWER | TRI_Y_LOWER)) ? 16 : 64) && items <= 65536 && a.nbi <= 4096 &&
       (a.tri & (TRI_X_LOWER | TRI_Y_LOWER)) != (TRI_X_LOWER | TRI_Y_LOWER)) {
     a.ntiles = (int)tile_items(a.nbi, a.nbj, 64 * WM, 64 * WN, a.tri);
@@ -715,8 +732,16 @@
   a.X = X; a.ldx = ldx; a.Y = Y; a.ldy = ldy; a.C = C; a.ldc = ldc; a.k = k;
   a.alpha = alpha; a.beta = beta; a.tri = 0;
   a.sXb = strideX; a.sYb = strideY; a.sCb = strideC; a.m_valid = m_valid; a.n_valid = n_valid; a.batch = batch;
-  if (y_is_kn) return launch_by_rows<Y_NN, EPI_STORE, COV_D2>(a, m, n, (hipStream_t)stream);
-  return launch_by_rows<Y_NT, EPI_STORE, COV_D2>(a, m, n, (hipStream_t)stream);
+  hipStream_t st = (hipStream_t)stream;
+  if (y_is_kn & ~(1 | GEOBO_GEMM_X_KM)) return GEOBO_E_ARG;
+  if (y_is_kn & GEOBO_GEMM_X_KM) {
+    if (y_is_kn & 1) return GEOBO_E_UNSUPPORTED;
+    if (m <= 0 || n <= 0 || m % 128 || n % 128) return GEOBO_E_ALIGN;
+    a.nbi = (int)(m / 128); a.nbj = (int)(n / 128);
+    return launch<2, 2, Y_NT_XT, EPI_STORE, COV_D2>(a, st);
+  }
+  if (y_is_kn) return launch_by_rows<Y_NN, EPI_STORE, COV_D2>(a, m, n, st);
+  return launch_by_rows<Y_NT, EPI_STORE, COV_D2>(a, m, n, st);
 }
 
 extern "C" size_t geobo_posterior_ws_bytes(int64_t m, int64_t ncols) {
diff --git a/geobo_amd/csrc/reduce.hip b/geobo_amd/csrc/reduce.hip
--- a/geobo_amd/csrc/reduce.hip
+++ b/geobo_amd/csrc/reduce.hip
@@ -160,6 +160,28 @@
   }
 }
 
+__global__ void __launch_bounds__(256) transpose_kernel(int64_t rows, int64_t cols, const double* __restrict__ src, int64_t lds,
+                                                        double* __restrict__ dst, int64_t ldd) {
+  __shared__ double t[64][65];
+  const int tx = threadIdx.x & 63, ty = threadIdx.x >> 6;
+  const int64_t r0 = (int64_t)blockIdx.y * 64, c0 = (int64_t)blockIdx.x * 64;
+#pragma unroll 4
+  for (int i = ty; i < 64; i += 4)
+    if (r0 + i < rows && c0 + tx < cols) t[i][tx] = src[(r0 + i) * lds + c0 + tx];
+  __syncthreads();
+#pragma unroll 4
+  for (int i = ty; i < 64; i += 4)
+    if (c0 + i < cols && r0 + tx < rows) dst[(c0 + i) * ldd + r0 + tx] = t[tx][i];
+}
+
+}
+
+extern "C" int geobo_transpose(int64_t rows, int64_t cols, const double* src, int64_t lds, double* dst, int64_t ldd, void* stream) {
+  if (!src || !dst || rows < 0 || cols < 0 || lds < cols || ldd < rows || (rows + 63) / 64 > 65535) return GEOBO_E_ARG;
+  if (rows == 0 || cols == 0) return GEOBO_OK;
+  hipLaunchKernelGGL(transpose_kernel, dim3((unsigned)((cols + 63) / 64), (unsigned)((rows + 63) / 64)), dim3(256), 0, (hipStream_t)stream,
+                     rows, cols, src, lds, dst, ldd);
+  return hipGetLastError() == hipSuccess ? GEOBO_OK : GEOBO_E_LAUNCH;
 }
 
 extern "C" int geobo_centro_fill(double* B, int64_t ld, int64_t n, int64_t r0, void* stream) {
diff --git a/geobo_amd/hip.py b/geobo_amd/hip.py
--- a/geobo_amd/hip.py
+++ b/geobo_amd/hip.py
@@ -186,6 +186,15 @@
     assert B.shape[0] >= n and B.shape[1] >= n
     _lib.check(lib.geobo_centro_fill(_p(B), int(ld), int(n), int(r0), _stream()), "geobo_centro_fill")
     return B
+
+
+def transpose(src, dst):
+    lib = require_gpu()
+    lds, ldd = _rowmajor(src, "src"), _rowmajor(dst, "dst")
+    rows, cols = src.shape
+    assert dst.shape[0] >= cols and dst.shape[1] >= rows
+    _lib.check(lib.geobo_transpose(int(rows), int(cols), _p(src), int(lds), _p(dst), int(ldd), _stream()), "geobo_transpose")
+    return dst
 
 
 def mirror_rows(X, m, r0, nb, nz):
@@ -430,15 +439,19 @@
     return C_
 
 
+X_KM = 2
+
+
 def gemm_batched(y_is_kn, m, n, k, X, ldx, strideX, Y, ldy, strideY, C_, ldc, strideC, m_valid, n_valid, batch, alpha=1.0,
-                 beta=0.0):
+                 beta=0.0, x_km=False):
     lib = require_gpu()
     done = 0
     esz = 8
-    _check_extents("geobo_gemm_batched", ((X, ldx, strideX, m, k, "X"), (Y, ldy, strideY, k if y_is_kn else n, n if y_is_kn else k, "Y")), batch)
+    _check_extents("geobo_gemm_batched", ((X, ldx, strideX, k if x_km else m, m if x_km else k, "X"),
+                                          (Y, ldy, strideY, k if y_is_kn else n, n if y_is_kn else k, "Y")), batch)
     while done < batch:
         nb = min(batch - done, 65535)
-        _lib.check(lib.geobo_gemm_batched(1 if y_is_kn else 0, int(m), int(n), int(k), float(alpha),
+        _lib.check(lib.geobo_gemm_batched((1 if y_is_kn else 0) | (X_KM if x_km else 0), int(m), int(n), int(k), float(alpha),
                                           C.c_void_p(X.data_ptr() + done * strideX * esz), int(ldx), int(strideX),
                                           C.c_void_p(Y.data_ptr() + done * strideY * esz), int(ldy), int(strideY), float(beta),
                                           C.c_void_p(C_.data_ptr() + done * strideC * esz), int(ldc), int(strideC),
diff --git a/geobo_amd/lattice_gram.py b/geobo_amd/lattice_gram.py
--- a/geobo_amd/lattice_gram.py
+++ b/geobo_amd/lattice_gram.py
@@ -86,9 +86,7 @@
             hip.gemm_batched(True, hip.pad_n(2 * nx), nzp, nx, F2, nx, 0, X[r0:], nz, X.stride(0), Xh, nz, 2 * nx * nz, 2 * nx, nz, R)
             o2 = sp.buf("LG_EO2", nx * 2 * max(J, nz) * RB)
             hip.gemm_batched(False, 2 * J, Rp, 2 * nz, V, 2 * nz, 2 * J * 2 * nz, Xh, 2 * nx * nz, 2 * nz, o2, Rp, 2 * J * Rp, 2 * J, R, nx)
-            oT = sp.buf("LG_EOT", max(J, nz) * nx * RB)
-            hip.gemm_batched(True, nxp, Rp, 2 * nx, FiT, 2 * nx, 0, o2, J * Rp, Rp, oT, Rp, nx * Rp, nx, R, ny)
-            out[r0:r0 + R, :ny * nx] += oT[:ny * nx * Rp].view(ny * nx, Rp)[:, :R].t()
+            hip.gemm_batched(False, Rp, nxp, 2 * nx, o2, J * Rp, Rp, FiT, 2 * nx, 0, out[r0:], out.stride(0), nx, R, nx, ny, beta=1.0, x_km=True)
 
     def transpose_tables(self, lam):
         return lam.view(self.Py, self.nz, self.Px).permute(2, 1, 0).contiguous().view(-1)
@@ -176,7 +174,8 @@
         nx, ny, nz, sp, J = self.nx, self.ny, self.nz, self.sp, self.J
         RB = self.EDGE_ROWS
         F2, FiT = self._edge_consts()
-        nyp, nxp = hip.pad_n(ny), hip.pad_n(nx)
+        nyp, nxp, nzp = hip.pad_n(ny), hip.pad_n(nx), hip.pad_n(nz)
+        assert Lrows.stride(1) == 1 and Lrows.stride(0) % 2 == 0 and out.stride(1) == 1
         end = Lrows.storage_offset() + (nrows - 1) * Lrows.stride(0) + nyp * nx
         if end > Lrows.untyped_storage().nbytes() // 8:
             Lc = sp.buf("LG_EX", nrows * ny * nx + nyp * nx)[:nrows * ny * nx].view(nrows, ny * nx)
@@ -190,14 +189,12 @@
                 Lh.zero_()
             hip.gemm_batched(False, hip.pad_n(2 * nx), nyp, nx, F2, nx, 0, Lrows[r0:], nx, Lrows.stride(0), Lh, J, 2 * nx * J, 2 * nx, ny, R)
             o2 = sp.buf("LG_EO2", nx * 2 * max(J, nz) * RB)
-            hip.gemm_batched(False, hip.pad_n(2 * nz), Rp, 2 * J, Vt, 2 * J, 2 * nz * 2 * J, Lh, 2 * nx * J, 2 * J, o2, Rp, 2 * nz * Rp, 2 * nz, R, nx)
-            oT = sp.buf("LG_EOT", max(J, nz) * nx * RB)
-            hip.gemm_batched(True, nxp, Rp, 2 * nx, FiT, 2 * nx, 0, o2, nz * Rp, Rp, oT, Rp, nx * Rp, nx, R, nz)
-            res = oT[:nz * nx * Rp].view(nz, nx, Rp)[:, :, :R]
             if zx:
-                out[r0:r0 + R, :nx * nz].view(R, nz, nx).copy_(res.permute(2, 0, 1))
-            else:
-                out[r0:r0 + R, :nx * nz].view(R, nx, nz).copy_(res.permute(2, 1, 0))
+                hip.gemm_batched(False, hip.pad_n(2 * nz), Rp, 2 * J, Vt, 2 * J, 2 * nz * 2 * J, Lh, 2 * nx * J, 2 * J, o2, Rp, 2 * nz * Rp, 2 * nz, R, nx)
+                hip.gemm_batched(False, Rp, nxp, 2 * nx, o2, nz * Rp, Rp, FiT, 2 * nx, 0, out[r0:], out.stride(0), nx, R, nx, nz, x_km=True)
+            else:
+                hip.gemm_batched(False, Rp, hip.pad_n(2 * nz), 2 * J, Lh, 2 * nx * J, 2 * J, Vt, 2 * J, 2 * nz * 2 * J, o2, 2 * nx * nz, 2 * nz, R, 2 * nz, nx)
+                hip.gemm_batched(True, nxp, nzp, 2 * nx, FiT, 2 * nx, 0, o2, nz, 2 * nx * nz, out[r0:], nz, out.stride(0), nx, nz, R)
 
     @staticmethod
     def fast(nx, ny, nz):
diff --git a/geobo_amd/spectral.py b/geobo_amd/spectral.py
--- a/geobo_amd/spectral.py
+++ b/geobo_amd/spectral.py
@@ -441,10 +441,13 @@
     def ss_slots(self):
         return hip.xz2d_fold_inv_ss_slots(self.nx, self.R, self.ny) if self.fused_ss() else self.GENERIC_SS_SLOTS
 
-    def y2s_tables(self, gens_g, gens_m, pair=(0, 1)):
+    def y2s_tables(self, gens_g, gens_m, pair=(0, 1), check=True):
+        a, b = pair
+        applies = self.forms.y2s and b == a + 1 and a % 2 == 0 and b < len(gens_g)
+        if not check:
+            return (a, gens_g[a] - gens_g[b], gens_g[b], gens_m[b] - gens_g[b]) if applies else None
         self.sym_residual = None
-        a, b = pair
-        if not (self.forms.y2s and b == a + 1 and a % 2 == 0 and b < len(gens_g)):
+        if not applies:
             return None
         x = gens_g[b]
         den = torch.maximum(x.abs().max(), gens_m[a].abs().max())
@@ -520,6 +523,36 @@
                     hip.xz2d_fold_inv_ss(nx, Rb, ny, sg[i], ny * Cp, Cp, self.F["x"], self.F["z"], ss[jj],
                                          src2=sm[i] if sm is not None else None, in2_row=ny * Cp, r2_first=0)
 
+    def has_two_term_product(self, nblocks):
+        meet = self.forms.y_two_term
+        return self.dense_y and ((meet == "y2t" and nblocks % 2 == 0) or meet == "add")
+
+    def product_two_term(self, Zg, Zm, rows, gens_g, gens_m, outs, y2s=None):
+        ny, C, Cp = self.ny, self.Px * self.Pz, self.Cp
+        P_c, meet = len(gens_g), self.forms.y_two_term
+        assert self.has_two_term_product(P_c) and rows <= self.R
+        t2g = self.forward_zx(Zg, rows, self.G, src_row_stride=Zg.stride(0), out_name="T2")
+        t2m = self.forward_zx(Zm, rows, self.G, src_row_stride=Zm.stride(0), out_name="T2b")
+        for j in range(0, P_c, 2 if meet == "y2t" else 3):
+            js = list(range(j, min(j + (2 if meet == "y2t" else 3), P_c)))
+            u2 = [self.buf(("S", "S1", "S2")[i], rows * ny * Cp) for i in range(len(js))]
+            gg, gm = [gens_g[jj] for jj in js], [gens_m[jj] for jj in js]
+            if meet == "y2t" and y2s is not None and y2s[0] == j:
+                y2s_fn = hip.spectral_y2s if self.y_mfma else hip.toeplitz_y2s
+                fn = lambda: y2s_fn(ny, C, rows, t2g, t2m, y2s[1], y2s[2], y2s[3], u2, plane=Cp)
+                self._launch("kernel:toeplitz_y2s", 8.0 * rows * C * 4 * ny, rows, self.y_stage_flop(2, 2, shared=True), fn)
+            elif meet == "y2t":
+                fn = lambda: hip.toeplitz_y2t(ny, C, rows, t2g, t2m, gg, gm, u2, plane=Cp)
+                self._launch("kernel:toeplitz_y2t", 8.0 * rows * C * 4 * ny, rows, self.y_stage_flop(2, 2), fn)
+            elif self.forms.y3t:
+                fn = lambda: hip.spectral_y3t(ny, C, rows, t2g, t2m, gg, gm, u2, plane=Cp)
+                self._launch("kernel:toeplitz_y", 8.0 * rows * C * ny * (2 + len(js)), rows, self.y_stage_flop(2, len(js)), fn)
+            else:
+                self._ystage(ny, C, rows, t2g, gg, u2, 0, ny, Cp)
+                self._ystage(ny, C, rows, t2m, gm, u2, 0, ny, Cp, accumulate=True)
+            for i, jj in enumerate(js):
+                self.backward_xz(u2[i], rows, 0, ny, [(0, ny, outs[jj], outs[jj].stride(0))])
+
     def flops_ss(self, rows_one, rows_two, nblocks, shared=False):
         nx, ny, nz, Px, Pz = self.nx, self.ny, self.nz, self.Px, self.Pz
         fwd = 1.0 * ny * (nx * nz * Pz + 0.5 * Px * nx * Pz)
diff --git a/geobo_amd/transposed.py b/geobo_amd/transposed.py
--- a/geobo_amd/transposed.py
+++ b/geobo_amd/transposed.py
@@ -38,7 +38,7 @@
             rows_times_AT(blk(0, 0), self.Ms, 0, AkA[0:, 0:Msp])
             rows_times_AT(blk(0, 1), self.Ms, 1, AkA[0:, Msp:2 * Msp])
             rows_times_AT(blk(Msp, 1), Mm, 1, AkA[Msp:, Msp:2 * Msp])
-            AkA[Msp:2 * Msp, :Msp] = AkA[:Msp, Msp:2 * Msp].t()
+            hip.transpose(AkA[:Msp, Msp:2 * Msp], AkA[Msp:2 * Msp, :Msp])
             if Md:
                 rows_times_AT(blk(off_d, 0), Md, 0, AkA[off_d:, 0:Msp])
                 rows_times_AT(blk(off_d, 1), Md, 1, AkA[off_d:, Msp:2 * Msp])
@@ -141,8 +141,10 @@
         else:
             ssum = torch.stack([t.sum(0).reshape(-1) for t in ss])
         if Md:
+            Kd = [AK[2 * Msp:, jj * self.nc:(jj + 1) * self.nc] for jj in range(P_c)] if self.nc >= N and self.c0 == 0 else None
             ssum = ssum + self._timed("posterior_drill_rows", 0.0, lambda: self._drill_rows_ss(
-                step, Linv, 0, Md, (lambda Lv, n, func, out: self._lattice_Z(Lv, n, func, A_g if func == "grav" else A_m, out)) if lat else None, Ag, Am))
+                step, Linv, 0, Md, (lambda Lv, n, func, out: self._lattice_Z(Lv, n, func, A_g if func == "grav" else A_m, out)) if lat else None, Ag, Am,
+                Kd=Kd, y2s=None if zx else y2s))
         return mu_l, (amp * 1.0 - ssum).reshape(-1)
 
     def _mean_rows(self, step, w, vec_of):
@@ -165,15 +167,20 @@
                 mu[jj].add_(tmp[jj][0])
         return mu
 
-    def _drill_rows_ss(self, step, Linv, d0, nd, lattice_Z, Ag, Am):
+    DRILL_SS_SLOTS = 4
+
+    def _drill_rows_ss(self, step, Linv, d0, nd, lattice_Z, Ag, Am, Kd=None, y2s=None):
         props, sel_t, Md = step.props, step.sel_t, step.Md
         sp, N, Msp, P_c, T = self._spectral, self.N, self.Ms_pad, len(props), 128
-        Zgd, Zmd, Zdd = (self._workspace2d(nm, T, N) for nm in ("Zg_d", "Zm_d", "Zd_d"))
+        if Kd is not None and lattice_Z is not None and sp.has_two_term_product(P_c) and sp.R >= T:
+            return self._drill_rows_ss_short(step, Linv, d0, nd, lattice_Z, Kd, y2s)
+        Zgd, Zmd = (self._workspace2d(nm, T, N) for nm in ("Zg_d", "Zm_d"))
         Vd = [self._workspace2d("Vd_%d" % jj, T, N) for jj in range(P_c)]
         tmp = [self._workspace2d("Vt_%d" % jj, T, N) for jj in range(P_c)]
         gens_g, gens_m = [step.gens[(0, j)] for j in props], [step.gens[(1, j)] for j in props]
+        acc = torch.zeros((P_c, N), dtype=F64, device=self.device)
+        Zdd = self._workspace2d("Zd_d", T, N)
         gens_d = [sp.eigenvalues(step.prior.table(self, 2, j)) for j in props]
-        acc = torch.zeros((P_c, N), dtype=F64, device=self.device)
         for c0 in range(d0, d0 + nd, T):
             n = min(T, d0 + nd - c0)
             b0 = 2 * Msp + c0
@@ -194,3 +201,29 @@
             for jj in range(P_c):
                 acc[jj].add_((Vd[jj][:n] ** 2).sum(0))
         return acc
+
+    def _drill_rows_ss_short(self, step, Linv, d0, nd, lattice_Z, Kd, y2s=None):
+        props, Md = step.props, step.Md
+        sp, N, Msp, P_c, T = self._spectral, self.N, self.Ms_pad, len(props), 128
+        Zgd, Zmd = (self._workspace2d(nm, T, N) for nm in ("Zg_d", "Zm_d"))
+        Vd = [self._workspace2d("Vd_%d" % jj, T, N) for jj in range(P_c)]
+        tmp = [self._workspace2d("Vt_%d" % jj, T, N) for jj in range(P_c)]
+        gens_g, gens_m = [step.gens[(0, j)] for j in props], [step.gens[(1, j)] for j in props]
+        if y2s is None and tuple(props[:2]) == (0, 1):
+            y2s = sp.y2s_tables(gens_g, gens_m, check=False)
+        kd = (Md + 15) // 16 * 16
+        Ld = self._workspace2d("Ld_d", T, kd)
+        ss = self._workspace("drill_ss", (P_c, self.DRILL_SS_SLOTS, N))
+        ss.zero_()
+        for c0 in range(d0, d0 + nd, T):
+            n = min(T, d0 + nd - c0)
+            b0 = 2 * Msp + c0
+            lattice_Z(Linv[b0:b0 + n, :Msp], n, "grav", Zgd)
+            lattice_Z(Linv[b0:b0 + n, Msp:2 * Msp], n, "magn", Zmd)
+            sp.product_two_term(Zgd, Zmd, n, gens_g, gens_m, Vd, y2s=y2s)
+            Ld.zero_()
+            Ld[:n, :Md] = Linv[b0:b0 + n, 2 * Msp:2 * Msp + Md]
+            for jj in range(P_c):
+                hip.gemm_batched(True, T, N, kd, Ld, Ld.stride(0), 0, Kd[jj], Kd[jj].stride(0), 0, tmp[jj], tmp[jj].stride(0), 0, n, N, 1)
+                hip.sumsq_accum(Vd[jj], tmp[jj], n, ss[jj])
+        return ss.sum(1)
diff --git a/include/geobo_hip.h b/include/geobo_hip.h
--- a/include/geobo_hip.h
+++ b/include/geobo_hip.h
@@ -105,6 +105,7 @@
                   const double* Y, int64_t ldy, double beta, double* C, int64_t ldc,
                   int x_lower, int y_lower, void* stream);
 
+#define GEOBO_GEMM_X_KM 2
 int geobo_gemm_batched(int y_is_kn, int64_t m, int64_t n, int64_t k, double alpha, const double* X, int64_t ldx,
                        int64_t strideX, const double* Y, int64_t ldy, int64_t strideY, double beta, double* C, int64_t ldc,
                        int64_t strideC, int64_t m_valid, int64_t n_valid, int batch, void* stream);
@@ -207,6 +208,7 @@
 int geobo_lamdot_z(int64_t batch, int planes, int px, int nz, const double* D, const double* lam, double* out, void* stream);
 
 int geobo_centro_fill(double* B, int64_t ld, int64_t n, int64_t r0, void* stream);
+int geobo_transpose(int64_t rows, int64_t cols, const double* src, int64_t lds, double* dst, int64_t ldd, void* stream);
 int geobo_mirror_rows(double* X, int64_t ld, int64_t m, int64_t r0, int64_t nb, int nz, void* stream);
 size_t geobo_mirror_dev_ws_bytes(void);
 int geobo_mirror_dev(const double* a, int64_t lda, const double* b, int64_t ldb, int64_t rows, int nx, int nz, double* out2, void* ws,
```

Result: faster. 2.373 million (median of 6 runs) (+1.2%).
